# Atsuyo64/RayTracingC

Measured on AMD Instinct MI355X. Metric: Mrays/sec + frame time, 1920x1080x64spp ultracomplex.obj, 1/2/4/8 GPUs, higher is better.
Workload: dtype f32; 1 GPU; ultracomplex_1080p64; scene=ultracomplex.obj, width=1920, height=1080, spp=64, max_bounce=10, triangles=120, row_band=1, chain_wgs_per_cu=3, parallelism=rows mod 1; each rank SDMA-copies its rows into the shared host frame

## Files before the change

include/rtc.h:

```cpp
#ifndef RTC_H
#define RTC_H

#include <stddef.h>
#include <stdint.h>

#ifdef __cplusplus
extern "C" {
#endif

typedef unsigned char uint8;
typedef struct vec3 { float x, y, z; } vec3;
typedef struct Scene {
    vec3 normalizedSunDirection, skyColorHorizon, skyColorZenith, groundColor;
    float sunFocus, sunIntensity;
} Scene;
typedef struct Color { uint8 r, g, b; } Color;
typedef struct Material { vec3 color; float emissionStrength; float smoothness; } Material;
typedef struct Sphere { vec3 pos; float r; Material mat; } Sphere;
typedef struct Triangle { vec3 posA, posB, posC, normal; Material mat; } Triangle;
typedef struct Ray { vec3 pos; vec3 dir; } Ray;

typedef struct RtcCamera { vec3 origin, ex, ey, ez; float fov; } RtcCamera;

typedef struct RtcRenderDesc {
    int width, height;
    int spp;
    int maxBounce;
    int trianglesOnly;
    int rowStart, rowStride;
    int flags;
    int rowBand;
} RtcRenderDesc;

#define RTC_F_HOIST_PRIMARY 0x1
#define RTC_F_DEBUG_BOUNCES 0x2
#define RTC_F_NO_TILE_CULL  0x4
#define RTC_F_NO_REORDER    0x8
#define RTC_F_NO_COOP       0x10
#define RTC_F_NO_CLUSTER_CULL 0x20
#define RTC_F_COOP4         0x40
#define RTC_F_COOP8         0x80
#define RTC_F_PIPE          0x200
#define RTC_F_SPEC          0x100
#define RTC_F_CHAIN_INLINE  0x400
#define RTC_F_HOST_ROWS     0x1000
#define RTC_F_SPLIT_SPHERES 0x2000
#define RTC_F_NO_DRAW_CACHE 0x4000
#define RTC_F_WAVE_PER_RAY  0x20000
#define RTC_F_OVERLAP       0x800

typedef struct RtcStats {
    double renderMs;
    double totalMs;
    unsigned long long segments;
    unsigned long long samples;
    unsigned long long triTests;
    unsigned long long clusterTests;
    unsigned long long discardedTests;
    double frameMs;
} RtcStats;

#define RTC_OK 0
#define RTC_EINVAL (-10001)
#define RTC_ENODEV (-10002)
#define RTC_EIO (-10003)
#define RTC_ENOMEM (-10004)
#define RTC_EFORMAT (-10005)
#define RTC_ETIMEDOUT (-10006)
#define RTC_EBUSY (-10007)

const char *rtc_last_error(void);
const char *rtc_version(void);
int rtc_device_count(int *count);

int rtc_load_obj(const char *path, Triangle **outTris, int *outCount);
int rtc_parse_triangle_file(const char *path, Triangle **outTris, int *outCount);
void rtc_free(void *p);
int rtc_default_spheres(const Sphere **outSpheres, int *outCount);
int rtc_default_scene(Scene *outScene);
int rtc_scene_set_sun(Scene *scene, vec3 sunDirection);
int rtc_camera_basis(vec3 origin, vec3 lookingAt, float fov, RtcCamera *outCam);
int rtc_write_bmp(const char *path, int width, int height, const Color *image);
int rtc_quantize(const float *accum, size_t pixels, Color *out);

int rtc_render(const Triangle *tris, int triCount, const Sphere *spheres, int sphereCount,
               const Scene *scene, const RtcCamera *cam, const RtcRenderDesc *d, int device,
               Color *outImage, float *outAccum, RtcStats *stats);

int rtc_render_multi(const Triangle *tris, int triCount, const Sphere *spheres, int sphereCount,
                     const Scene *scene, const RtcCamera *cam, const RtcRenderDesc *d, int numDevices,
                     Color *outImage, float *outAccum, RtcStats *stats);
int rtc_last_multi_info(int *path, int *devices, int *commRanks, int maxComms);

typedef struct RtcDeviceScene RtcDeviceScene;
int rtc_scene_upload(const Triangle *tris, int triCount, const Sphere *spheres, int sphereCount,
                     int device, RtcDeviceScene **out);
int rtc_scene_release(RtcDeviceScene *s);
int rtc_scene_update_async(RtcDeviceScene *s, const Triangle *dTris, int triCount, const Sphere *dSpheres,
                           int sphereCount, void *stream);
int rtc_scene_update(RtcDeviceScene *s, const Triangle *tris, int triCount, const Sphere *spheres, int sphereCount);
size_t rtc_scene_regroup_scratch_bytes(const RtcDeviceScene *s);
int rtc_scene_regroup_max_tris(void);
int rtc_scene_regroup_async(RtcDeviceScene *s, const Triangle *dTris, int triCount, const Sphere *dSpheres,
                            int sphereCount, void *dScratch, size_t scratchBytes, void *stream);
int rtc_scene_regroup(RtcDeviceScene *s, const Triangle *tris, int triCount, const Sphere *spheres, int sphereCount);
int rtc_regroup_membership_host(const Triangle *tris, int triCount, int *idx);
int rtc_rows_selected(const RtcRenderDesc *d);
#define RTC_SEGMENT_COUNTERS 5
int rtc_scene_set_timing(RtcDeviceScene *s, int enable);
int rtc_scene_set_geometry_event(RtcDeviceScene *s, void *event);
int rtc_scene_set_frame_event(RtcDeviceScene *s, void *event);
int rtc_scene_kernel_times(const RtcDeviceScene *s, float out[2]);
int rtc_bounce_hit_share(const Triangle *tris, int triCount, float *share);
int rtc_scene_chain_wgs(const RtcDeviceScene *s);
typedef struct RtcChainReport {
    int multi, count, hits, general, spheres, resume;
    int chainPrimF, wgsPerCu, chainDyn, clusterCount, chunkCount, launches;
} RtcChainReport;
int rtc_scene_chain_report(const RtcDeviceScene *s, RtcChainReport *out);
int rtc_scene_set_draw_cache(RtcDeviceScene *s, long long blocks);
int rtc_scene_draw_cache_reset(RtcDeviceScene *s);
int rtc_scene_draw_cache_stats(const RtcDeviceScene *s, unsigned long long out[4]);
int rtc_probe_draw_cache(const RtcDeviceScene *s, unsigned int seed, float *out, int *block);
int rtc_bounce_hit_share_all(const Triangle *tris, int triCount, const Sphere *spheres, int sphereCount, float *share);
int rtc_scene_sphere_split(const RtcDeviceScene *s);
int rtc_render_rows_async(const RtcDeviceScene *s, const Scene *scene, const RtcCamera *cam,
                          const RtcRenderDesc *d, void *dColors, float *dAccum,
                          unsigned long long *dSegments, void *stream);
typedef struct RtcSampleRange { int first, count; } RtcSampleRange;
int rtc_render_samples_async(const RtcDeviceScene *s, const Scene *scene, const RtcCamera *cam,
                             const RtcRenderDesc *d, const RtcSampleRange *range,
                             void *dColors, float *dAccum, unsigned int *dRngState,
                             unsigned long long *dSegments, void *stream);
typedef struct RtcHitBuffers {
    int *prim;
    float *depth;
    float *normal;
    float *albedo;
} RtcHitBuffers;
int rtc_render_first_hit_async(const RtcDeviceScene *s, const RtcCamera *cam, const RtcRenderDesc *d,
                               const RtcHitBuffers *out, void *stream);
int rtc_trace_rays_async(const RtcDeviceScene *s, const Ray *dRays, size_t n, int trianglesOnly, int flags,
                         const RtcHitBuffers *out, void *stream);
int rtc_trace_rays(const RtcDeviceScene *s, const Ray *rays, size_t n, int trianglesOnly, int flags, int *prim,
                   float *depth, float *normal, float *albedo);
typedef struct RtcPathDesc {
    int spp;
    int maxBounce;
    int trianglesOnly;
    int flags;
    int sampleFirst, sampleCount;
} RtcPathDesc;
int rtc_trace_paths_async(const RtcDeviceScene *s, const Scene *scene, const Ray *dRays, const unsigned int *dSeeds,
                          size_t n, const RtcPathDesc *d, float *dRadiance, unsigned int *dSeedsOut,
                          unsigned long long *dSegments, void *stream);
int rtc_trace_paths(const RtcDeviceScene *s, const Scene *scene, const Ray *rays, const unsigned int *seeds, size_t n,
                    const RtcPathDesc *d, float *radiance, unsigned int *seedsOut, unsigned long long *segments);
int rtc_occluded_async(const RtcDeviceScene *s, const Ray *dRays, const float *dTMax , size_t n,
                       int trianglesOnly, int flags, unsigned char *dOccluded ,
                       unsigned long long *dCount , void *stream);
int rtc_occluded(const RtcDeviceScene *s, const Ray *rays, const float *tMax, size_t n, int trianglesOnly, int flags,
                 unsigned char *occluded, unsigned long long *count);
int rtc_render_pixels_async(const RtcDeviceScene *s, const Scene *scene, const RtcCamera *cam, const RtcRenderDesc *d,
                            const RtcSampleRange *range, const unsigned int *dPixels, size_t n, int flags,
                            void *dColors , float *dAccum, unsigned int *dRngState,
                            unsigned long long *dSegments , void *stream);
int rtc_render_pixels(const RtcDeviceScene *s, const Scene *scene, const RtcCamera *cam, const RtcRenderDesc *d,
                      const RtcSampleRange *range, const unsigned int *pixels, size_t n, int flags, void *colors,
                      float *accum, unsigned int *rngState, unsigned long long *segments);
int rtc_scene_bounds(const RtcDeviceScene *s, float lo[3], float hi[3]);
size_t rtc_ray_order_scratch_bytes(size_t n);
int rtc_ray_order_shape(int *keysPerGroup, int *scanGroups);
int rtc_ray_order_async(const RtcDeviceScene *s, const Ray *dRays, size_t n, const float *bounds,
                        unsigned *dOrder, unsigned *dKeys, void *dScratch, size_t scratchBytes, void *stream);
int rtc_ray_order(const RtcDeviceScene *s, const Ray *rays, size_t n, const float *bounds, unsigned *order,
                  unsigned *keys);
int rtc_ray_keys_host(const Ray *rays, size_t n, const float lo[3], const float hi[3], unsigned *keys);
int rtc_gather_async(void *dDst, const void *dSrc, const unsigned *dOrder, size_t n, size_t elemBytes, void *stream);
int rtc_scatter_async(void *dDst, const void *dSrc, const unsigned *dOrder, size_t n, size_t elemBytes, void *stream);
int rtc_copy_async(void *dst, const void *src, size_t bytes, int blocks, void *stream);
int rtc_copy_d2h_dma(void *hostDst, const void *devSrc, size_t bytes);
int rtc_dma_pending(const void *p, size_t bytes);
int rtc_dma_debug_inflight(void *p, size_t bytes, int pending);
int rtc_copy_rows_d2h_dma(void *hostDst, size_t hostPitch, const void *devSrc, size_t srcPitch, size_t rowBytes,
                          int rows);
int rtc_host_register(void *p, size_t bytes);
int rtc_host_unregister(void *p);

typedef struct RtcPlanSim RtcPlanSim;
int rtc_plan_sim_create(int triCount, int legacySlotLayout, RtcPlanSim **out);
int rtc_plan_sim_launch(RtcPlanSim *sim, const RtcRenderDesc *d, unsigned long long stream, unsigned long long colors,
                        unsigned long long accum, int segments, const float cam[13], const float env[14], int *ops,
                        int maxOps, unsigned long long *footprint, int maxFootprint);
int rtc_plan_sim_set_spheres(RtcPlanSim *sim, int sphereCount, int gateAllows);
int rtc_plan_sim_set_draw_cache(RtcPlanSim *sim, int on);
int rtc_plan_sim_set_sample_range(RtcPlanSim *sim, int first, int count, unsigned long long rngBuffer);
int rtc_plan_sim_set_first_hit(RtcPlanSim *sim, unsigned long long prim, unsigned long long depth,
                               unsigned long long normal, unsigned long long albedo);
int rtc_plan_sim_update(RtcPlanSim *sim, unsigned long long stream, int *ops, int maxOps, unsigned long long *footprint,
                        int maxFootprint);
int rtc_plan_sim_set_update_fault(RtcPlanSim *sim, int mode);
int rtc_plan_sim_regroup(RtcPlanSim *sim, unsigned long long stream, unsigned long long scratch, int *ops, int maxOps,
                         unsigned long long *footprint, int maxFootprint);
int rtc_plan_sim_trace_rays(RtcPlanSim *sim, unsigned long long stream, unsigned long long rays,
                            const unsigned long long hit[4], int flags, int *ops, int maxOps,
                            unsigned long long *footprint, int maxFootprint);
int rtc_plan_sim_trace_paths(RtcPlanSim *sim, unsigned long long stream, unsigned long long rays,
                             unsigned long long seeds, unsigned long long radiance, unsigned long long seedsOut,
                             unsigned long long segments, int sampleFirst, int flags, int *ops, int maxOps,
                             unsigned long long *footprint, int maxFootprint);
int rtc_plan_sim_occluded(RtcPlanSim *sim, unsigned long long stream, unsigned long long rays, unsigned long long tMax,
                          unsigned long long occluded, unsigned long long count, int flags, int *ops, int maxOps,
                          unsigned long long *footprint, int maxFootprint);
int rtc_plan_sim_render_pixels(RtcPlanSim *sim, unsigned long long stream, unsigned long long pixels,
                               unsigned long long colors, unsigned long long accum, unsigned long long rng,
                               unsigned long long segments, int first, int flags, int *ops, int maxOps,
                               unsigned long long *footprint, int maxFootprint);
int rtc_plan_sim_regions(const RtcPlanSim *sim, unsigned long long *rows, int maxRows);
int rtc_plan_sim_release(RtcPlanSim *sim);

typedef struct RtcLoopStats {
    double wallMs;
    int frames;
    double enqueueMs;
    double copyMsMedian;
    double copyMsMax;
} RtcLoopStats;
int rtc_frame_loop(RtcDeviceScene *s, const Scene *scene, const RtcCamera *cam, const RtcRenderDesc *d,
                   void *const *devRows, void *const *hostRows, size_t hostPitch, int nbuf, int frames, void *stream,
                   RtcLoopStats *stats);
int rtc_frame_loop_cameras(RtcDeviceScene *s, const Scene *scene, const RtcCamera *cams, int ncams,
                           const RtcRenderDesc *d, void *const *devRows, void *const *hostRows, size_t hostPitch,
                           int nbuf, int frames, void *stream, RtcLoopStats *stats);

int rtc_deinterleave_async(const void *dCompact, int parts, int rowsPerPart, int width, int height,
                           void *dOut, void *stream);
int rtc_deinterleave_bands_async(const void *dCompact, int parts, int rowsPerPart, int width, int height, int rowBand,
                                 void *dOut, void *stream);

int rtc_probe_ray_triangle(const Ray *rays, const Triangle *tris, size_t n, int *didHit, float *dst);
int rtc_probe_ray_sphere(const Ray *rays, const Sphere *spheres, size_t n, int *didHit, float *dst,
                         vec3 *normal);
int rtc_probe_environment(const Ray *rays, const Scene *scenes, size_t n, vec3 *out);
int rtc_probe_random(const unsigned int *seeds, size_t n, int draws, float *uniform, float *normal,
                     vec3 *direction);
int rtc_probe_sun_vanish(const Ray *rays, const Scene *scene, size_t n, int spp, int *vanish, vec3 *out, vec3 *sum);
int rtc_env_vanish_limit(const Scene *scene, double *limit);
int rtc_probe_cluster_bound(const Triangle *tris, int triCount, const Ray *rays, size_t n,
                            unsigned long long counts[7]);
int rtc_probe_item_records(const Triangle *tris, int triCount, const Sphere *spheres, int sphereCount, const Scene *scene,
                           const RtcCamera *cam, const RtcRenderDesc *d, int counts[16], int info[4],
                           unsigned int *records, size_t maxRecords, unsigned long long *pixMask, size_t maxTiles);
int rtc_probe_primary_cull(const Triangle *tris, int triCount, const Scene *scene, const RtcCamera *cam,
                           const RtcRenderDesc *d, unsigned char *kept, size_t maxKept, unsigned long long *tileBits,
                           size_t maxWords, unsigned long long *pixMask, size_t maxTiles, int info[4], float *primF,
                           double *cones, unsigned char *pruned);
int rtc_scene_records_host(const Triangle *tris, int triCount, const Triangle *newTris, const Sphere *spheres,
                           int sphereCount, void *outTris, void *outMats, void *outSpheres, void *outClTris,
                           void *outClusters, void *outChunks, size_t bytes[6]);
int rtc_probe_scene_records(const RtcDeviceScene *s, void *outTris, void *outMats, void *outSpheres, void *outClTris,
                            void *outClusters, void *outChunks, size_t bytes[6]);

#ifdef __cplusplus
}
#endif
#endif
```

raytracingc_amd/__init__.py:

```python
from __future__ import annotations

import contextlib
import ctypes as C
from dataclasses import dataclass

import numpy as np

from ._abi import (
    CLI_PATH,
    LIB_PATH,
    RAY_DT,
    RTC_F_DEBUG_BOUNCES,
    RTC_F_HOIST_PRIMARY,
    RTC_F_NO_CLUSTER_CULL,
    RTC_F_NO_COOP,
    RTC_F_CHAIN_INLINE,
    RTC_F_OVERLAP,
    RTC_F_HOST_ROWS,
    RTC_F_SPLIT_SPHERES,
    RTC_F_NO_DRAW_CACHE,
    RTC_F_NO_REORDER,
    RTC_F_NO_TILE_CULL,
    RTC_F_WAVE_PER_RAY,
    RTC_SEGMENT_COUNTERS,
    RTC_EBUSY,
    RTC_EINVAL,
    RTC_ETIMEDOUT,
    SCENE_DT,
    SPHERE_DT,
    TRIANGLE_DT,
    VEC3_DT,
    EXPORTS,
    Ray,
    RtcCamera,
    RtcChainReport,
    RtcError,
    RtcHitBuffers,
    RtcLoopStats,
    RtcPathDesc,
    RtcRenderDesc,
    RtcSampleRange,
    RtcStats,
    Scene,
    Vec3,
    check,
    lib,
)
from ._abi import _ptr

__all__ = [
    "loadOBJTriangles", "parseTriangleFile", "default_spheres", "default_scene", "camera_basis", "RenderConfig",
    "render", "render_multi", "DeviceScene", "vec3ToColor", "write_bmp", "rayTriangle", "raySphere",
    "getEnvironmentLight", "random_sequences", "device_count", "lib", "TRIANGLE_DT", "SPHERE_DT", "RAY_DT",
    "SCENE_DT", "RtcError", "ProgressState", "save_progress", "load_progress", "scene_records_host", "RECORD_ARRAYS",
    "ray_keys_host", "ray_order_scratch_bytes", "gather_async", "scatter_async",
    "regroup_membership_host", "regroup_max_tris", "adaptive_selection",
]

DEFAULT_ORIGIN = (-4.75, -1.5, -4.75)
DEFAULT_LOOKING_AT = (0.9, -1.2, 1.0)
DEFAULT_FOV = 1.0
DEFAULT_SUN = (-30.0, -85.0, 100.0)


def _take_tris(p: C.c_void_p, n: int) -> np.ndarray:
    out = np.empty(n, dtype=TRIANGLE_DT)
    if n:
        C.memmove(out.ctypes.data, p.value, n * TRIANGLE_DT.itemsize)
    lib().rtc_free(p)
    return out


def loadOBJTriangles(path: str) -> np.ndarray:
    p, n = C.c_void_p(), C.c_int()
    check(lib().rtc_load_obj(path.encode(), C.byref(p), C.byref(n)), "rtc_load_obj")
    return _take_tris(p, n.value)


def parseTriangleFile(path: str) -> np.ndarray:
    p, n = C.c_void_p(), C.c_int()
    check(lib().rtc_parse_triangle_file(path.encode(), C.byref(p), C.byref(n)), "rtc_parse_triangle_file")
    return _take_tris(p, n.value)


def default_spheres() -> np.ndarray:
    p, n = C.c_void_p(), C.c_int()
    check(lib().rtc_default_spheres(C.byref(p), C.byref(n)), "rtc_default_spheres")
    out = np.empty(n.value, dtype=SPHERE_DT)
    C.memmove(out.ctypes.data, p.value, n.value * SPHERE_DT.itemsize)
    return out


def default_scene(sun=DEFAULT_SUN, ground=None, horizon=None, zenith=None, focus=None, intensity=None) -> Scene:
    s = Scene()
    check(lib().rtc_default_scene(C.byref(s)), "rtc_default_scene")
    if ground is not None:
        s.groundColor = Vec3(*ground)
    if horizon is not None:
        s.skyColorHorizon = Vec3(*horizon)
    if zenith is not None:
        s.skyColorZenith = Vec3(*zenith)
    if focus is not None:
        s.sunFocus = focus
    if intensity is not None:
        s.sunIntensity = intensity
    check(lib().rtc_scene_set_sun(C.byref(s), Vec3(*sun)), "rtc_scene_set_sun")
    return s


def camera_basis(origin=DEFAULT_ORIGIN, looking_at=DEFAULT_LOOKING_AT, fov=DEFAULT_FOV) -> RtcCamera:
    cam = RtcCamera()
    check(lib().rtc_camera_basis(Vec3(*origin), Vec3(*looking_at), C.c_float(fov), C.byref(cam)), "rtc_camera_basis")
    return cam


@dataclass
class RenderConfig:
    width: int = 128
    height: int = 128
    spp: int = 4000
    max_bounce: int = 10
    triangles_only: bool = True
    hoist: bool = False
    row_start: int = 0
    row_stride: int = 1
    row_band: int = 0
    debug_bounces: bool = False
    tile_cull: bool = True
    reorder: bool = True
    coop: bool = True
    cluster_cull: bool = True
    chain_inline: bool = False
    host_rows: bool = False
    overlap: bool = False
    split_spheres: bool = False
    draw_cache: bool = True

    def flags(self) -> int:
        return ((RTC_F_HOIST_PRIMARY if self.hoist else 0) | (RTC_F_DEBUG_BOUNCES if self.debug_bounces else 0)
                | (0 if self.tile_cull else RTC_F_NO_TILE_CULL) | (0 if self.reorder else RTC_F_NO_REORDER)
                | (0 if self.coop else RTC_F_NO_COOP) | (0 if self.cluster_cull else RTC_F_NO_CLUSTER_CULL)
                | (RTC_F_CHAIN_INLINE if self.chain_inline else 0) | (RTC_F_OVERLAP if self.overlap else 0)
                | (RTC_F_HOST_ROWS if self.host_rows else 0) | (RTC_F_SPLIT_SPHERES if self.split_spheres else 0)
                | (0 if self.draw_cache else RTC_F_NO_DRAW_CACHE))

    def desc(self) -> RtcRenderDesc:
        return RtcRenderDesc(self.width, self.height, self.spp, self.max_bounce, int(self.triangles_only),
                             self.row_start, self.row_stride, self.flags(), self.row_band)

    def rows(self) -> int:
        d = self.desc()
        return lib().rtc_rows_selected(C.byref(d))


def _arr(a, dt):
    if a is None or len(a) == 0:
        return None, 0
    a = np.ascontiguousarray(a, dtype=dt)
    return a, len(a)


def _stats(st: RtcStats) -> dict:
    return {"render_ms": st.renderMs, "frame_ms": st.frameMs, "total_ms": st.totalMs, "segments": st.segments,
            "samples": st.samples, "tri_tests": st.triTests, "cluster_tests": st.clusterTests,
            "discarded_tests": st.discardedTests}


def _vp(p):
    return C.c_void_p(p) if p else None


def _query_rays(who: str, rays):
    if hasattr(rays, "data_ptr"):
        nbytes = rays.numel() * rays.element_size()
        if not rays.is_cuda or not rays.is_contiguous() or nbytes % RAY_DT.itemsize:
            raise ValueError(f"{who}: rays must be a contiguous device tensor of whole 24-byte Rays")
        return True, rays, nbytes // RAY_DT.itemsize
    a = np.asarray(rays)
    if a.dtype != RAY_DT:
        if a.ndim != 2 or a.shape[1] != 6:
            raise ValueError(f"{who}: rays must be RAY_DT [n] or float32 [n, 6]")
        a = np.ascontiguousarray(a, np.float32).view(RAY_DT).reshape(-1)
    a = np.ascontiguousarray(a.reshape(-1))
    return False, a, len(a)


@contextlib.contextmanager
def _current_stream_of(device):
    import torch

    with torch.cuda.device(device):
        st = torch.cuda.current_stream()
        yield st.cuda_stream
        st.synchronize()


def _host_order(who: str, order, n: int) -> np.ndarray:
    if hasattr(order, "data_ptr"):
        order = order.detach().cpu().numpy()
    idx = np.ascontiguousarray(np.asarray(order).reshape(-1)).astype(np.intp)
    if len(idx) != n or (n and (idx.min() < 0 or idx.max() >= n)):
        raise ValueError(f"{who}: order must hold {n} indices below {n}")
    return idx


def _device_order(who: str, order, n: int, device):
    import torch

    if not hasattr(order, "data_ptr"):
        order = torch.from_numpy(_host_order(who, order, n).astype(np.int32))
    order = order.reshape(-1).to(device=device, dtype=torch.int32).contiguous()
    if order.numel() != n or (n and (int(order.min()) < 0 or int(order.max()) >= n)):
        raise ValueError(f"{who}: order must hold {n} indices below {n}")
    return order


def _permuted(scatter: bool, src, order, n: int, elem_bytes: int, stream):
    import torch

    dst = torch.zeros_like(src) if scatter else torch.empty_like(src)
    if n:
        (scatter_async if scatter else gather_async)(dst.data_ptr(), src.data_ptr(), order.data_ptr(), n, elem_bytes,
                                                     stream)
    return dst


RECORD_ARRAYS = ("tris", "mats", "spheres", "clTris", "clusters", "chunks")
# ... 396 lines not shown
                    continue
                if not hasattr(t, "data_ptr") or not t.is_cuda or t.device != dev or not t.is_contiguous() or \
                        t.numel() * t.element_size() != nbytes:
                    raise ValueError(f"{who}: {name} must be a contiguous tensor of {nbytes} bytes on the list's device")
            if pixels.element_size() != 4 or rng.element_size() != 4 or accum.dtype != torch.float32:
                raise ValueError(f"{who}: pixels and rng are 4-byte integers, accum is float32")
            seg = torch.zeros(1, dtype=torch.int64, device=dev)
            if n and npix:
                with _current_stream_of(dev) as st:
                    self.render_pixels_async(scene, cam, cfg, first, count, pixels.data_ptr(), n, accum.data_ptr(),
                                             rng.data_ptr(), colors.data_ptr() if colors is not None else 0,
                                             seg.data_ptr() if segments else None, flags, st)
            res = {"accum": accum, "rng": rng}
            if colors is not None:
                res["colors"] = colors
            if segments:
                res["segments"] = int(seg.cpu().numpy()[0])
            return res
        px = np.asarray(pixels).reshape(-1)
        if px.size and (not np.issubdtype(px.dtype, np.integer) or px.min() < 0 or px.max() > 0xffffffff):
            raise ValueError(f"{who}: pixels must be integers in [0, 2^32)")
        px = np.ascontiguousarray(px, np.uint32)
        acc = np.array(accum, np.float32, order="C")
        state = np.array(rng, np.uint32, order="C")
        col = None if colors is None else np.array(colors, np.uint8, order="C")
        if acc.size != 3 * npix or state.size != npix or (col is not None and col.size != 3 * npix):
            raise ValueError(f"{who}: accum float32 [rows, W, 3], rng uint32 [rows, W] and colors uint8 [rows, W, 3] of "
                             f"the frame's {npix} pixels")
        seg = C.c_ulonglong(0)
        if len(px) and npix:
            d = cfg.desc()
            rg = RtcSampleRange(int(first), int(count))
            check(lib().rtc_render_pixels(self._h, C.byref(scene), C.byref(cam), C.byref(d), C.byref(rg), _ptr(px), len(px),
                                          int(flags), _ptr(col), _ptr(acc), _ptr(state),
                                          C.cast(C.pointer(seg), C.c_void_p) if segments else None), "rtc_render_pixels")
        res = {"accum": acc, "rng": state}
        if col is not None:
            res["colors"] = col
        if segments:
            res["segments"] = int(seg.value)
        return res

    def render_adaptive(self, scene: Scene, cam: RtcCamera, cfg: RenderConfig, passes, select, flags: int = 0):
        import torch

        passes = [int(c) for c in passes]
        if not passes or any(c <= 0 for c in passes) or sum(passes) > cfg.spp:
            raise ValueError(f"render_adaptive: passes {passes} are not positive counts summing to at most spp = {cfg.spp}")
        rows = cfg.rows()
        colors = torch.zeros((rows, cfg.width, 3), dtype=torch.uint8, device="cuda")
        accum = torch.zeros((rows, cfg.width, 3), dtype=torch.float32, device="cuda")
        rng = torch.zeros((rows, cfg.width), dtype=torch.int32, device="cuda")
        samples = np.zeros((rows, cfg.width), np.int32)
        st = torch.cuda.current_stream().cuda_stream
        done, host = 0, None
        for k, count in enumerate(passes):
            if k == 0:
                self.render_samples_async(scene, cam, cfg, 0, count, colors.data_ptr(), accum.data_ptr(), rng.data_ptr(),
                                          None, st)
                samples += count
            else:
                sel = adaptive_selection(select(done, host[0], host[1], samples.copy()), samples, done)
                if len(sel) == 0:
                    return
                pixels = torch.from_numpy(sel.view(np.int32)).cuda()
                self.render_pixels_async(scene, cam, cfg, done, count, pixels.data_ptr(), len(sel), accum.data_ptr(),
                                         rng.data_ptr(), colors.data_ptr(), None, flags, st)
                samples.reshape(-1)[sel] += count
            done += count
            torch.cuda.synchronize()
            host = (colors.cpu().numpy(), accum.cpu().numpy())
            yield done, host[0], host[1], samples.copy()

    @property
    def chain_wgs(self) -> int:
        return lib().rtc_scene_chain_wgs(self._h)

    def chain_report(self) -> dict:
        r = RtcChainReport()
        check(lib().rtc_scene_chain_report(self._h, C.byref(r)), "rtc_scene_chain_report")
        out = {k: bool(getattr(r, k)) for k in ("multi", "count", "hits", "general", "spheres", "resume")}
        out.update(chain_prim_f=bool(r.chainPrimF), wgs_per_cu=r.wgsPerCu, chain_dyn=r.chainDyn,
                   cluster_count=r.clusterCount, chunk_count=r.chunkCount, launches=r.launches)
        return out

    def set_draw_cache(self, blocks: int = -1):
        check(lib().rtc_scene_set_draw_cache(self._h, int(blocks)), "rtc_scene_set_draw_cache")

    def draw_cache_reset(self):
        check(lib().rtc_scene_draw_cache_reset(self._h), "rtc_scene_draw_cache_reset")

    def draw_cache_stats(self) -> dict:
        out = (C.c_ulonglong * 4)()
        check(lib().rtc_scene_draw_cache_stats(self._h, out), "rtc_scene_draw_cache_stats")
        return {"blocks": int(out[0]), "capacity": int(out[1]), "fresh": int(out[2]), "uncached": int(out[3])}

    def draw_cache_block(self, seed: int):
        out = np.zeros((64, 4), np.float32)
        blk = C.c_int(-1)
        check(lib().rtc_probe_draw_cache(self._h, int(seed), _ptr(out), C.byref(blk)), "rtc_probe_draw_cache")
        return out if blk.value >= 0 else None

    @property
    def sphere_split(self) -> bool:
        return bool(lib().rtc_scene_sphere_split(self._h))

    def set_timing(self, enable: bool):
        check(lib().rtc_scene_set_timing(self._h, int(enable)), "rtc_scene_set_timing")

    def set_geometry_event(self, event_handle: int | None):
        check(lib().rtc_scene_set_geometry_event(self._h, C.c_void_p(event_handle) if event_handle else None),
              "rtc_scene_set_geometry_event")

    def set_frame_event(self, event_handle: int | None):
        check(lib().rtc_scene_set_frame_event(self._h, C.c_void_p(event_handle) if event_handle else None),
              "rtc_scene_set_frame_event")

    def frame_loop(self, scene: Scene, cam, cfg: RenderConfig, dev_rows: list, host_rows: list,
                   host_pitch: int, frames: int, stream: int | None = None) -> dict:
        n = len(dev_rows)
        if len(host_rows) != n:
            raise ValueError("frame_loop: one host buffer per device buffer")
        d = cfg.desc()
        dv = (C.c_void_p * n)(*dev_rows)
        hv = (C.c_void_p * n)(*host_rows)
        st = RtcLoopStats()
        strm = C.c_void_p(stream) if stream else None
        if isinstance(cam, RtcCamera):
            check(lib().rtc_frame_loop(self._h, C.byref(scene), C.byref(cam), C.byref(d), dv, hv,
                                       C.c_size_t(host_pitch), n, int(frames), strm, C.byref(st)), "rtc_frame_loop")
        else:
            cams = (RtcCamera * len(cam))(*cam)
            check(lib().rtc_frame_loop_cameras(self._h, C.byref(scene), cams, len(cam), C.byref(d), dv, hv,
                                               C.c_size_t(host_pitch), n, int(frames), strm, C.byref(st)),
                  "rtc_frame_loop_cameras")
        return {"wall_ms": st.wallMs, "frames": st.frames, "enqueue_ms": st.enqueueMs,
                "copy_ms_median": st.copyMsMedian, "copy_ms_max": st.copyMsMax}

    def kernel_times(self):
        out = (C.c_float * 2)()
        check(lib().rtc_scene_kernel_times(self._h, out), "rtc_scene_kernel_times")
        return None if out[0] < 0 else (float(out[0]), float(out[1]))

    def regroup_scratch_bytes(self) -> int:
        return int(lib().rtc_scene_regroup_scratch_bytes(self._h))

    def regroup_async(self, tris_ptr: int, spheres_ptr: int | None, scratch_ptr: int, scratch_bytes: int,
                      stream: int | None = None):
        if not self._h:
            raise RuntimeError("DeviceScene.regroup_async: the scene has been released")
        check(lib().rtc_scene_regroup_async(self._h, _vp(tris_ptr), self.tri_count, _vp(spheres_ptr),
                                            self.sphere_count if spheres_ptr else 0, _vp(scratch_ptr), scratch_bytes,
                                            _vp(stream)), "rtc_scene_regroup_async")

    def update(self, tris=None, spheres=None, stream: int | None = None, regroup: bool = False):
        if not self._h:
            raise RuntimeError("DeviceScene.update: the scene has been released")
        if tris is None and spheres is None:
            raise ValueError("DeviceScene.update: neither triangles nor spheres")
        if regroup and tris is None:
            raise ValueError("DeviceScene.update: regroup=True needs the triangles (the clusters are decided from them)")
        on_device = [hasattr(a, "data_ptr") for a in (tris, spheres) if a is not None]
        if not any(on_device):
            t, nt = _arr(tris, TRIANGLE_DT)
            s, ns = _arr(spheres, SPHERE_DT)
            if regroup:
# ... 304 lines not shown
```

raytracingc_amd/_abi.py:

```python
from __future__ import annotations

import ctypes as C
import os

import numpy as np

HERE = os.path.dirname(os.path.abspath(__file__))
LIB_PATH = os.environ.get("RTC_LIB_PATH") or os.path.join(HERE, "_lib", "librtc.so")
CLI_PATH = os.path.join(HERE, "_lib", "rtc")


class Vec3(C.Structure):
    _fields_ = [("x", C.c_float), ("y", C.c_float), ("z", C.c_float)]


class Scene(C.Structure):
    _fields_ = [
        ("normalizedSunDirection", Vec3),
        ("skyColorHorizon", Vec3),
        ("skyColorZenith", Vec3),
        ("groundColor", Vec3),
        ("sunFocus", C.c_float),
        ("sunIntensity", C.c_float),
    ]
# ... 8 lines not shown


class Triangle(C.Structure):
    _fields_ = [("posA", Vec3), ("posB", Vec3), ("posC", Vec3), ("normal", Vec3), ("mat", Material)]


class Ray(C.Structure):
    _fields_ = [("pos", Vec3), ("dir", Vec3)]


class RtcCamera(C.Structure):
    _fields_ = [("origin", Vec3), ("ex", Vec3), ("ey", Vec3), ("ez", Vec3), ("fov", C.c_float)]


class RtcRenderDesc(C.Structure):
    _fields_ = [
        ("width", C.c_int),
        ("height", C.c_int),
        ("spp", C.c_int),
        ("maxBounce", C.c_int),
        ("trianglesOnly", C.c_int),
        ("rowStart", C.c_int),
        ("rowStride", C.c_int),
        ("flags", C.c_int),
        ("rowBand", C.c_int),
    ]


class RtcSampleRange(C.Structure):
    _fields_ = [("first", C.c_int), ("count", C.c_int)]


class RtcHitBuffers(C.Structure):
    _fields_ = [("prim", C.c_void_p), ("depth", C.c_void_p), ("normal", C.c_void_p), ("albedo", C.c_void_p)]


class RtcPathDesc(C.Structure):
    _fields_ = [(k, C.c_int) for k in ("spp", "maxBounce", "trianglesOnly", "flags", "sampleFirst", "sampleCount")]


class RtcChainReport(C.Structure):
    _fields_ = [(k, C.c_int) for k in ("multi", "count", "hits", "general", "spheres", "resume", "chainPrimF", "wgsPerCu",
                                       "chainDyn", "clusterCount", "chunkCount", "launches")]


class RtcStats(C.Structure):
    _fields_ = [
        ("renderMs", C.c_double),
        ("totalMs", C.c_double),
        ("segments", C.c_ulonglong),
        ("samples", C.c_ulonglong),
        ("triTests", C.c_ulonglong),
        ("clusterTests", C.c_ulonglong),
        ("discardedTests", C.c_ulonglong),
        ("frameMs", C.c_double),
    ]


class RtcLoopStats(C.Structure):
    _fields_ = [
        ("wallMs", C.c_double),
        ("frames", C.c_int),
        ("enqueueMs", C.c_double),
        ("copyMsMedian", C.c_double),
        ("copyMsMax", C.c_double),
    ]


RTC_F_HOIST_PRIMARY = 0x1
RTC_F_DEBUG_BOUNCES = 0x2
RTC_F_NO_TILE_CULL = 0x4
RTC_F_NO_REORDER = 0x8
RTC_F_NO_COOP = 0x10
RTC_F_NO_CLUSTER_CULL = 0x20
RTC_F_COOP4 = 0x40
RTC_F_COOP8 = 0x80
RTC_F_SPEC = 0x100
RTC_F_PIPE = 0x200
RTC_F_CHAIN_INLINE = 0x400
RTC_F_OVERLAP = 0x800
RTC_F_HOST_ROWS = 0x1000
RTC_F_SPLIT_SPHERES = 0x2000
RTC_F_NO_DRAW_CACHE = 0x4000
RTC_F_WAVE_PER_RAY = 0x20000
RAY_ORDER_KEYS_PER_GROUP = 4096
RAY_ORDER_SCAN_GROUPS = 256
RTC_SEGMENT_COUNTERS = 5
RTC_EINVAL, RTC_ENODEV, RTC_EIO, RTC_ENOMEM, RTC_EFORMAT = -10001, -10002, -10003, -10004, -10005
RTC_ETIMEDOUT, RTC_EBUSY = -10006, -10007

assert C.sizeof(Vec3) == 12 and C.sizeof(Scene) == 56 and C.sizeof(Material) == 20
assert C.sizeof(Sphere) == 36 and C.sizeof(Triangle) == 68 and C.sizeof(Ray) == 24

VEC3_DT = np.dtype([("x", "<f4"), ("y", "<f4"), ("z", "<f4")])
MATERIAL_DT = np.dtype([("color", VEC3_DT), ("emissionStrength", "<f4"), ("smoothness", "<f4")])
TRIANGLE_DT = np.dtype(
    [("posA", VEC3_DT), ("posB", VEC3_DT), ("posC", VEC3_DT), ("normal", VEC3_DT), ("mat", MATERIAL_DT)]
)
SPHERE_DT = np.dtype([("pos", VEC3_DT), ("r", "<f4"), ("mat", MATERIAL_DT)])
RAY_DT = np.dtype([("pos", VEC3_DT), ("dir", VEC3_DT)])
SCENE_DT = np.dtype(
    [
        ("normalizedSunDirection", VEC3_DT),
        ("skyColorHorizon", VEC3_DT),
        ("skyColorZenith", VEC3_DT),
        ("groundColor", VEC3_DT),
        ("sunFocus", "<f4"),
        ("sunIntensity", "<f4"),
    ]
)
assert TRIANGLE_DT.itemsize == 68 and SPHERE_DT.itemsize == 36 and RAY_DT.itemsize == 24
assert SCENE_DT.itemsize == 56

EXPORTS = [
    "rtc_last_error", "rtc_version", "rtc_device_count",
    "rtc_load_obj", "rtc_parse_triangle_file", "rtc_free", "rtc_default_spheres", "rtc_default_scene",
    "rtc_scene_set_sun", "rtc_camera_basis", "rtc_write_bmp", "rtc_quantize",
    "rtc_render", "rtc_render_multi", "rtc_last_multi_info",
    "rtc_scene_upload", "rtc_scene_release", "rtc_rows_selected", "rtc_render_rows_async", "rtc_scene_set_timing", "rtc_scene_kernel_times",
    "rtc_bounce_hit_share", "rtc_scene_chain_wgs", "rtc_bounce_hit_share_all", "rtc_scene_sphere_split",
    "rtc_plan_sim_set_spheres", "rtc_plan_sim_regions", "rtc_render_samples_async", "rtc_plan_sim_set_sample_range",
    "rtc_scene_set_geometry_event", "rtc_scene_set_frame_event",
    "rtc_deinterleave_async", "rtc_deinterleave_bands_async", "rtc_copy_async", "rtc_copy_d2h_dma", "rtc_copy_rows_d2h_dma", "rtc_host_register",
    "rtc_host_unregister", "rtc_plan_sim_create", "rtc_plan_sim_launch", "rtc_plan_sim_release", "rtc_frame_loop", "rtc_frame_loop_cameras", "rtc_dma_pending", "rtc_dma_debug_inflight",
    "rtc_probe_ray_triangle", "rtc_probe_ray_sphere", "rtc_probe_environment", "rtc_probe_random",
    "rtc_probe_cluster_bound", "rtc_probe_sun_vanish", "rtc_env_vanish_limit", "rtc_probe_item_records",
    "rtc_probe_primary_cull",
    "rtc_scene_update_async", "rtc_scene_update", "rtc_plan_sim_update", "rtc_plan_sim_set_update_fault",
    "rtc_scene_records_host", "rtc_probe_scene_records",
    "rtc_scene_chain_report",
    "rtc_render_first_hit_async", "rtc_plan_sim_set_first_hit",
    "rtc_trace_rays_async", "rtc_trace_rays", "rtc_plan_sim_trace_rays",
    "rtc_scene_set_draw_cache", "rtc_scene_draw_cache_reset", "rtc_scene_draw_cache_stats", "rtc_probe_draw_cache",
    "rtc_plan_sim_set_draw_cache",
    "rtc_trace_paths_async", "rtc_trace_paths", "rtc_plan_sim_trace_paths",
    "rtc_occluded_async", "rtc_occluded", "rtc_plan_sim_occluded",
    "rtc_scene_bounds", "rtc_ray_order_shape", "rtc_ray_order_scratch_bytes", "rtc_ray_order_async", "rtc_ray_order", "rtc_ray_keys_host",
    "rtc_gather_async", "rtc_scatter_async",
    "rtc_scene_regroup_scratch_bytes", "rtc_scene_regroup_max_tris", "rtc_scene_regroup_async", "rtc_scene_regroup",
    "rtc_regroup_membership_host", "rtc_plan_sim_regroup",
    "rtc_render_pixels_async", "rtc_render_pixels", "rtc_plan_sim_render_pixels",
]

_lib = None


def _ptr(a: np.ndarray | None):
    return None if a is None else a.ctypes.data_as(C.c_void_p)


def lib() -> C.CDLL:
    global _lib
    if _lib is not None:
        return _lib
    if not os.path.exists(LIB_PATH):
        raise RuntimeError(f"librtc.so not built ({LIB_PATH}); run `make` or __graft_entry__.build()")
    try:
        import torch
    except Exception:
        pass
    L = C.CDLL(LIB_PATH)
    vp, ip, sz = C.c_void_p, C.c_int, C.c_size_t
    L.rtc_last_error.restype = C.c_char_p
    L.rtc_version.restype = C.c_char_p
    L.rtc_device_count.argtypes = [C.POINTER(C.c_int)]
    L.rtc_load_obj.argtypes = [C.c_char_p, C.POINTER(vp), C.POINTER(C.c_int)]
    L.rtc_parse_triangle_file.argtypes = [C.c_char_p, C.POINTER(vp), C.POINTER(C.c_int)]
    L.rtc_free.argtypes = [vp]
    L.rtc_free.restype = None
    L.rtc_default_spheres.argtypes = [C.POINTER(vp), C.POINTER(C.c_int)]
    L.rtc_default_scene.argtypes = [C.POINTER(Scene)]
    L.rtc_scene_set_sun.argtypes = [C.POINTER(Scene), Vec3]
    L.rtc_camera_basis.argtypes = [Vec3, Vec3, C.c_float, C.POINTER(RtcCamera)]
    L.rtc_write_bmp.argtypes = [C.c_char_p, ip, ip, vp]
    L.rtc_quantize.argtypes = [vp, sz, vp]
    L.rtc_render.argtypes = [vp, ip, vp, ip, C.POINTER(Scene), C.POINTER(RtcCamera), C.POINTER(RtcRenderDesc), ip,
                             vp, vp, C.POINTER(RtcStats)]
    L.rtc_render_multi.argtypes = [vp, ip, vp, ip, C.POINTER(Scene), C.POINTER(RtcCamera),
                                   C.POINTER(RtcRenderDesc), ip, vp, vp, C.POINTER(RtcStats)]
    L.rtc_last_multi_info.argtypes = [C.POINTER(C.c_int), C.POINTER(C.c_int), C.POINTER(C.c_int), ip]
    L.rtc_scene_upload.argtypes = [vp, ip, vp, ip, ip, C.POINTER(vp)]
    L.rtc_scene_release.argtypes = [vp]
    L.rtc_scene_kernel_times.argtypes = [vp, vp]
    L.rtc_bounce_hit_share.argtypes = [vp, C.c_int, C.POINTER(C.c_float)]
    L.rtc_scene_chain_wgs.argtypes = [vp]
    if hasattr(L, "rtc_scene_sphere_split"):
        L.rtc_bounce_hit_share_all.argtypes = [vp, C.c_int, vp, C.c_int, C.POINTER(C.c_float)]
        L.rtc_scene_sphere_split.argtypes = [vp]
        L.rtc_plan_sim_set_spheres.argtypes = [vp, ip, ip]
    L.rtc_scene_set_timing.argtypes = [vp, C.c_int]
    L.rtc_scene_set_geometry_event.argtypes = [vp, vp]
    L.rtc_scene_set_frame_event.argtypes = [vp, vp]
    L.rtc_copy_async.argtypes = [vp, vp, sz, C.c_int, vp]
    L.rtc_copy_d2h_dma.argtypes = [vp, vp, sz]
    L.rtc_copy_rows_d2h_dma.argtypes = [vp, sz, vp, sz, sz, ip]
    L.rtc_host_register.argtypes = [vp, sz]
    L.rtc_host_unregister.argtypes = [vp]
    L.rtc_frame_loop.argtypes = [vp, C.POINTER(Scene), C.POINTER(RtcCamera), C.POINTER(RtcRenderDesc), vp, vp, sz, ip,
                                 ip, vp, C.POINTER(RtcLoopStats)]
    L.rtc_frame_loop_cameras.argtypes = [vp, C.POINTER(Scene), vp, ip, C.POINTER(RtcRenderDesc), vp, vp, sz, ip, ip,
                                         vp, C.POINTER(RtcLoopStats)]
    L.rtc_plan_sim_create.argtypes = [ip, ip, C.POINTER(vp)]
    L.rtc_plan_sim_launch.argtypes = [vp, C.POINTER(RtcRenderDesc), C.c_ulonglong, C.c_ulonglong, C.c_ulonglong, ip, vp,
                                      vp, vp, ip, vp, ip]
    L.rtc_plan_sim_release.argtypes = [vp]
    if hasattr(L, "rtc_plan_sim_regions"):
        L.rtc_plan_sim_regions.argtypes = [vp, vp, ip]
    L.rtc_dma_pending.argtypes = [vp, sz]
    L.rtc_dma_debug_inflight.argtypes = [vp, sz, ip]
    L.rtc_rows_selected.argtypes = [C.POINTER(RtcRenderDesc)]
    L.rtc_render_rows_async.argtypes = [vp, C.POINTER(Scene), C.POINTER(RtcCamera), C.POINTER(RtcRenderDesc), vp, vp,
                                        vp, vp]
    if hasattr(L, "rtc_render_samples_async"):
        L.rtc_render_samples_async.argtypes = [vp, C.POINTER(Scene), C.POINTER(RtcCamera), C.POINTER(RtcRenderDesc),
                                               C.POINTER(RtcSampleRange), vp, vp, vp, vp, vp]
        L.rtc_plan_sim_set_sample_range.argtypes = [vp, ip, ip, C.c_ulonglong]
    L.rtc_deinterleave_async.argtypes = [vp, ip, ip, ip, ip, vp, vp]
    if hasattr(L, "rtc_deinterleave_bands_async"):
        L.rtc_deinterleave_bands_async.argtypes = [vp, ip, ip, ip, ip, ip, vp, vp]
    L.rtc_probe_ray_triangle.argtypes = [vp, vp, sz, vp, vp]
    L.rtc_probe_ray_sphere.argtypes = [vp, vp, sz, vp, vp, vp]
    L.rtc_probe_environment.argtypes = [vp, vp, sz, vp]
    L.rtc_probe_random.argtypes = [vp, sz, ip, vp, vp, vp]
    L.rtc_probe_cluster_bound.argtypes = [vp, ip, vp, sz, vp]
    if hasattr(L, "rtc_probe_sun_vanish"):
        L.rtc_probe_sun_vanish.argtypes = [vp, vp, sz, ip, vp, vp, vp]
        L.rtc_env_vanish_limit.argtypes = [vp, vp]
    if hasattr(L, "rtc_probe_item_records"):
        L.rtc_probe_item_records.argtypes = [vp, ip, vp, ip, C.POINTER(Scene), C.POINTER(RtcCamera),
                                             C.POINTER(RtcRenderDesc), vp, vp, vp, sz, vp, sz]
    if hasattr(L, "rtc_probe_primary_cull"):
        L.rtc_probe_primary_cull.argtypes = [vp, ip, C.POINTER(Scene), C.POINTER(RtcCamera), C.POINTER(RtcRenderDesc),
                                             vp, sz, vp, sz, vp, sz, vp, vp, vp, vp]
    if hasattr(L, "rtc_scene_update_async"):
        L.rtc_scene_update_async.argtypes = [vp, vp, ip, vp, ip, vp]
        L.rtc_scene_update.argtypes = [vp, vp, ip, vp, ip]
        L.rtc_plan_sim_update.argtypes = [vp, C.c_ulonglong, vp, ip, vp, ip]
        L.rtc_plan_sim_set_update_fault.argtypes = [vp, ip]
        L.rtc_scene_records_host.argtypes = [vp, ip, vp, vp, ip, vp, vp, vp, vp, vp, vp, vp]
        L.rtc_probe_scene_records.argtypes = [vp, vp, vp, vp, vp, vp, vp, vp]
    if hasattr(L, "rtc_scene_chain_report"):
        L.rtc_scene_chain_report.argtypes = [vp, C.POINTER(RtcChainReport)]
    if hasattr(L, "rtc_render_first_hit_async"):
        L.rtc_render_first_hit_async.argtypes = [vp, C.POINTER(RtcCamera), C.POINTER(RtcRenderDesc),
                                                 C.POINTER(RtcHitBuffers), vp]
        L.rtc_plan_sim_set_first_hit.argtypes = [vp, C.c_ulonglong, C.c_ulonglong, C.c_ulonglong, C.c_ulonglong]
    if hasattr(L, "rtc_trace_rays_async"):
        L.rtc_trace_rays_async.argtypes = [vp, vp, sz, ip, ip, C.POINTER(RtcHitBuffers), vp]
        L.rtc_trace_rays.argtypes = [vp, vp, sz, ip, ip, vp, vp, vp, vp]
        L.rtc_plan_sim_trace_rays.argtypes = [vp, C.c_ulonglong, C.c_ulonglong, vp, ip, vp, ip, vp, ip]
    if hasattr(L, "rtc_scene_set_draw_cache"):
        L.rtc_scene_set_draw_cache.argtypes = [vp, C.c_longlong]
        L.rtc_scene_draw_cache_reset.argtypes = [vp]
        L.rtc_scene_draw_cache_stats.argtypes = [vp, vp]
        L.rtc_probe_draw_cache.argtypes = [vp, C.c_uint, vp, C.POINTER(C.c_int)]
        L.rtc_plan_sim_set_draw_cache.argtypes = [vp, ip]
    if hasattr(L, "rtc_trace_paths_async"):
        L.rtc_trace_paths_async.argtypes = [vp, C.POINTER(Scene), vp, vp, sz, C.POINTER(RtcPathDesc), vp, vp, vp, vp]
        L.rtc_trace_paths.argtypes = [vp, C.POINTER(Scene), vp, vp, sz, C.POINTER(RtcPathDesc), vp, vp, vp]
        L.rtc_plan_sim_trace_paths.argtypes = [vp, C.c_ulonglong, C.c_ulonglong, C.c_ulonglong, C.c_ulonglong,
                                               C.c_ulonglong, C.c_ulonglong, ip, ip, vp, ip, vp, ip]
    if hasattr(L, "rtc_occluded_async"):
        L.rtc_occluded_async.argtypes = [vp, vp, vp, sz, ip, ip, vp, vp, vp]
        L.rtc_occluded.argtypes = [vp, vp, vp, sz, ip, ip, vp, vp]
        L.rtc_plan_sim_occluded.argtypes = [vp, C.c_ulonglong, C.c_ulonglong, C.c_ulonglong, C.c_ulonglong,
                                            C.c_ulonglong, ip, vp, ip, vp, ip]
    if hasattr(L, "rtc_ray_order_async"):
        L.rtc_scene_bounds.argtypes = [vp, vp, vp]
        L.rtc_ray_order_shape.argtypes = [C.POINTER(C.c_int), C.POINTER(C.c_int)]
        L.rtc_ray_order_scratch_bytes.argtypes = [sz]
        L.rtc_ray_order_scratch_bytes.restype = sz
        L.rtc_ray_order_async.argtypes = [vp, vp, sz, vp, vp, vp, vp, sz, vp]
        L.rtc_ray_order.argtypes = [vp, vp, sz, vp, vp, vp]
        L.rtc_ray_keys_host.argtypes = [vp, sz, vp, vp, vp]
        L.rtc_gather_async.argtypes = [vp, vp, vp, sz, sz, vp]
        L.rtc_scatter_async.argtypes = [vp, vp, vp, sz, sz, vp]
    if hasattr(L, "rtc_scene_regroup_async"):
        L.rtc_scene_regroup_scratch_bytes.argtypes = [vp]
        L.rtc_scene_regroup_scratch_bytes.restype = sz
        L.rtc_scene_regroup_max_tris.argtypes = []
        L.rtc_scene_regroup_async.argtypes = [vp, vp, ip, vp, ip, vp, sz, vp]
        L.rtc_scene_regroup.argtypes = [vp, vp, ip, vp, ip]
        L.rtc_regroup_membership_host.argtypes = [vp, ip, vp]
        L.rtc_plan_sim_regroup.argtypes = [vp, C.c_ulonglong, C.c_ulonglong, vp, ip, vp, ip]
    if hasattr(L, "rtc_render_pixels_async"):
        L.rtc_render_pixels_async.argtypes = [vp, C.POINTER(Scene), C.POINTER(RtcCamera), C.POINTER(RtcRenderDesc),
                                              C.POINTER(RtcSampleRange), vp, sz, ip, vp, vp, vp, vp, vp]
        L.rtc_render_pixels.argtypes = [vp, C.POINTER(Scene), C.POINTER(RtcCamera), C.POINTER(RtcRenderDesc),
                                        C.POINTER(RtcSampleRange), vp, sz, ip, vp, vp, vp, vp]
        L.rtc_plan_sim_render_pixels.argtypes = [vp, C.c_ulonglong, C.c_ulonglong, C.c_ulonglong, C.c_ulonglong,
                                                 C.c_ulonglong, C.c_ulonglong, ip, ip, vp, ip, vp, ip]
    _lib = L
    return L


class RtcError(RuntimeError):
    def __init__(self, code: int, where: str):
        msg = lib().rtc_last_error().decode(errors="replace")
        super().__init__(f"{where} failed ({code}): {msg}")
        self.code = code


def check(rc: int, where: str) -> None:
    if rc != 0:
        raise RtcError(rc, where)
```

raytracingc_amd/csrc/rtc_chain.h:

```cpp
#pragma once

static_assert(sizeof(SampleSlot) == rtcplan::kSampleSlotBytes, "the planner sizes the deferred sample slots");
#ifndef RTC_SKY_MERGE
#define RTC_SKY_MERGE 1
#endif
constexpr int kChainBlock = 256;
#ifndef RTC_CHAIN_WGS_SHARE
#define RTC_CHAIN_WGS_SHARE 3
#endif
#ifndef RTC_CHAIN_WAVES
#define RTC_CHAIN_WAVES 4
#endif

typedef float f2 __attribute__((ext_vector_type(2)));
constexpr int kChainPairs = 1024;
struct ChainWaveLds {
    float4 cl[kChunkClusters][2];
    unsigned long long key[64];
    unsigned short pair[kChainPairs];
    float4 draw[64];
};
constexpr unsigned long long kNoHitKey = ((unsigned long long)0x497423F0u << 32) | 0xFFFFFFFFull;
static_assert(kChunkClusters <= 32, "cluster masks are 32-bit");
static_assert(kChainPairs >= 64 * kClusterSize, "one cluster's pairs of a full wave fit the list");
// ... 322 lines not shown
        }
        const size_t o = (size_t)P.itemPix[it];
        P.colors[3 * o] = float_to_u8(accxy.x);
        P.colors[3 * o + 1] = float_to_u8(accxy.y);
        P.colors[3 * o + 2] = float_to_u8(accz);
        if (P.accum) {
            P.accum[3 * o] = accxy.x;
            P.accum[3 * o + 1] = accxy.y;
            P.accum[3 * o + 2] = accz;
        }
    }
}

__device__ __forceinline__ void closest_primary_listed_lds(const RenderParams &P, V3 dir, Closest &c, const unsigned long long *__restrict__ mask,
                                                           unsigned long long m0, unsigned long long m1,
                                                           const DevPrimF *__restrict__ sF, bool staged)
{
    const int maskWords = KARG(maskWords);
    const DevPrimF *const primF = KARG(primF);
    const DevPrimX *const primX = KARG(primX);
    for (int w = 0; w < maskWords; ++w) {
        unsigned long long m = w == 0 ? m0 : w == 1 ? m1 : KCONST(mask)[w];
        while (m) {
            const int t = w * 64 + __builtin_ctzll(m);
            m &= m - 1;
            const DevPrimF F = staged ? sF[t] : KLOAD(primF, t);
            if (!prim_backfacing(dir, F) && prim_pass(dir, F) && !(dot(dir, V3{F.nx, F.ny, F.nz}) >= 0.f)) {
                const DevPrimX X = KLOAD(primX, t);
                const V3 h = cross(dir, V3{X.acx, X.acy, X.acz});
                const float det = dot(V3{X.abx, X.aby, X.abz}, h);
                if (!(-kEps < det && det < kEps)) {
                    const float invDet = rcp_cr(det);
                    const float u = dot(V3{X.s0x, X.s0y, X.s0z}, h) * invDet;
                    const float v = dot(dir, V3{X.q0x, X.q0y, X.q0z}) * invDet;
                    const float dst = X.dac0 * invDet;
                    if (!(u < 0.f || u > 1.f) && !(v < 0.f || u + v > 1.f) && !(dst < kEps) && dst < c.dst) {
                        c.dst = dst;
                        c.idx = t;
                    }
                }
            }
        }
    }
}

constexpr int kChainSphereBase = 1 << 30;
__device__ __forceinline__ void closest_spheres(const RenderParams &P, V3 pos, V3 dir, Closest &c)
{
    const DevSphere *const spheres = KARG(spheres);
    const int n = KARG(sphereCount);
    for (int i = 0; i < n; ++i) {
        const DevSphere sp = KLOAD(spheres, i);
        float d;
        if (ray_sphere(pos, dir, V3{sp.cx, sp.cy, sp.cz}, sp.radius, d) && d < c.dst) {
            c.dst = d;
            c.idx = kChainSphereBase + i;
        }
    }
}

struct ChainStage {
    float4 *rec;
    DevPrimF *primF;
};
template <bool MULTI>
__device__ __forceinline__ ChainStage chain_stage(const RenderParams &P, unsigned char *sDyn)
{
    ChainStage S{nullptr, nullptr};
    if (!MULTI)
        S.rec = (float4 *)sDyn;
    if (P.chainPrimF)
        S.primF = (DevPrimF *)(sDyn + (MULTI ? 0 : (size_t)soa_slots(P.clusterCount * kClusterSize) * sizeof(DevTri)));
    const int nRec = P.clusterCount * kClusterSize, slots = soa_slots(nRec);
    for (int i = threadIdx.x; S.rec && i < nRec; i += kChainBlock) {
        const float4 *g = (const float4 *)(P.clTris + i);
        for (int k = 0; k < 4; ++k)
            S.rec[k * slots + i] = g[k];
    }
    for (int i = threadIdx.x; S.primF && i < P.triPadded; i += kChainBlock)
        S.primF[i] = P.primF[i];
    return S;
}

template <bool MULTI, bool COUNT, bool HITS, bool GENERAL, bool SPHERES = false, bool RESUME = false, bool DRAWS = false>
__global__ __launch_bounds__(kChainBlock) __attribute__((amdgpu_waves_per_eu(RTC_CHAIN_WAVES))) void rtc_render_chain(
    RenderParams P)
{
    if (RTC_CHAIN_PRIO > 0)
        __builtin_amdgcn_s_setprio(RTC_CHAIN_PRIO);
    DSECT_BEGIN(dtot);
    DMARK_INIT(dcur);
#ifdef RTC_DIAG
    const unsigned long long dWaveT0 = __builtin_amdgcn_s_memrealtime();
    unsigned dWaveItems = 0;
    unsigned long long dItemEnd[5] = {0, 0, 0, 0, 0};
#endif
    extern __shared__ __attribute__((aligned(64))) unsigned char sDyn[];
    __shared__ PowTablesLds sPow;
    __shared__ ChainWaveLds sWave[kChainBlock / 64];
    __shared__ int sWork;
    __shared__ DevCluster sCl[kChunkClusters];
    if (!MULTI && threadIdx.x < P.clusterCount && threadIdx.x < kChunkClusters)
        sCl[threadIdx.x] = P.clusters[threadIdx.x];
    if (threadIdx.x == 0)
        sWork = 0;
    sPow.fill(threadIdx.x);
    const ChainStage S = chain_stage<MULTI>(P, sDyn);
    const float4 *sRec = S.rec;
    const DevPrimF *sPF = (const DevPrimF *)(sDyn + (MULTI ? 0 : (size_t)soa_slots(P.clusterCount * kClusterSize) * sizeof(DevTri)));
    const bool pfStaged = !GENERAL || P.chainPrimF != 0;
#ifdef RTC_DIAG
    if ((threadIdx.x & 63) < kDiagSects)
        s_rtc_sect[threadIdx.x >> 6][threadIdx.x & 63] = 0;
    static_assert(kChainBlock / 64 <= 4, "s_rtc_sect holds four waves");
#endif
    __syncthreads();
    sPow.attach(P.env);
    const int lane = threadIdx.x & 63;
    ChainWaveLds &W = sWave[threadIdx.x >> 6];
    const RngJump laneJump = rng_jump_by(7u * (unsigned)lane);
    int nextIt = 0;
    const auto next_item = [&]() { return (int)blockIdx.x + atomicAdd(&sWork, 1) * (int)gridDim.x; };
    if (lane == 0)
        nextIt = next_item();
#ifdef RTC_DIAG_COUNT
    constexpr bool counting = true;
#else
    constexpr bool counting = COUNT;
#endif
    unsigned segCalls = 0, segTraced = 0, segClusters = 0;
    unsigned long long segTests = 0, segSpec = 0;
#ifdef RTC_DIAG
    unsigned long long dIters = 0, dAlive = 0, dAct = 0, dWindows = 0, dUsed = 0, dIters2 = 0, dAlive2 = 0;
#endif
    int incl = lane < kGeoLists ? min(P.geoCount[lane * kGeoCountStride], P.geoCap) : 0;
#pragma unroll
    for (int d = 1; d < kGeoLists; d <<= 1) {
        const int v = __shfl_up(incl, d);
        if (lane >= d)
            incl += v;
    }
    const int nItems = __builtin_amdgcn_readlane(incl, kGeoLists - 1);
    const auto entry_of = [&](int it2) -> size_t {
        const int l = (int)__popcll(__ballot(lane < kGeoLists && incl <= it2));
        const int base = l ? __builtin_amdgcn_readlane(incl, l - 1) : 0;
        return (size_t)l * KARG(geoCap) + (size_t)(it2 - base);
    };
    static_assert(!DRAWS || (!GENERAL && !RESUME && !SPHERES && !MULTI && !COUNT), "the draw cache: the kernels without GENERAL");
    const auto record_dwords = [&](int it2) -> unsigned {
        if constexpr (DRAWS) {
            const size_t e = entry_of(it2);
            const unsigned *const rec = KARG(geoList) + e * (size_t)kItemRecDwords + (size_t)(lane & (kItemRecDwords - 1));
            const unsigned *const blk = KARG(itemDraw) + e;
            return gload((lane & kItemRecDwords) ? blk : rec, 0);
        }
        return gload(KARG(geoList), entry_of(it2) * (size_t)kItemRecDwords + (size_t)(lane & (kItemRecDwords - 1)));
    };
    const auto record_tile = [&](unsigned d0) -> int {
        return KARG(wideItems) ? (int)(d0 >> 6) : (int)(d0 >> 19) * (KARG(blocksX) * 2) + (int)((d0 & 0xffffu) >> 3);
    };
    const auto mask_dwords = [&](unsigned d0) -> unsigned {
        const unsigned *mw = (const unsigned *)(KARG(tileMask) + (size_t)record_tile(d0) * P.maskWords);
        return lane < 2 * P.maskWords && lane < 4 ? gload(mw, (size_t)lane) : 0u;
    };
    int it = __builtin_amdgcn_readfirstlane(nextIt);
    unsigned vc = 0, vm = 0;
    if (it < nItems) {
        vc = record_dwords(it);
        vm = mask_dwords((unsigned)__builtin_amdgcn_readfirstlane((int)vc));
    }
    if (lane == 0)
        nextIt = next_item();
    DMARK(dcur, 19);
    for (;;) {
        if (it >= nItems)
            break;
#ifdef RTC_DIAG
        const unsigned long long dItemT0 = __builtin_amdgcn_s_memrealtime();
        unsigned dItemWindows = 0;
        const unsigned long long dItemIters0 = dIters;
        const unsigned dBm0 = __atomic_load_n(&g_rtc_bmfall[(blockIdx.x * (kChainBlock / 64) + (threadIdx.x >> 6)) & 65535u],
                                              __ATOMIC_RELAXED);
        const unsigned long long dSect = lane < kItemSects ? s_rtc_sect[threadIdx.x >> 6][item_sect_id(lane)] : 0ull;
        unsigned long long dItemTests = 0;
#endif
        const unsigned d0 = (unsigned)__builtin_amdgcn_readfirstlane((int)vc);
        const V3 pdir{__uint_as_float((unsigned)__builtin_amdgcn_readlane((int)vc, 1)),
                      __uint_as_float((unsigned)__builtin_amdgcn_readlane((int)vc, 2)),
                      __uint_as_float((unsigned)__builtin_amdgcn_readlane((int)vc, 3))};
        const unsigned long long m0 = (unsigned long long)(unsigned)__builtin_amdgcn_readlane((int)vm, 0) |
                                      (unsigned long long)(unsigned)__builtin_amdgcn_readlane((int)vm, 1) << 32;
        const unsigned long long m1 = (unsigned long long)(unsigned)__builtin_amdgcn_readlane((int)vm, 2) |
                                      (unsigned long long)(unsigned)__builtin_amdgcn_readlane((int)vm, 3) << 32;
        float4 cachedDraw = make_float4(0.f, 0.f, 0.f, 0.f);
        unsigned drawBlock = 0;
        if constexpr (DRAWS) {
            drawBlock = (unsigned)__builtin_amdgcn_readlane((int)vc, kItemRecDwords);
            if (drawBlock)
                cachedDraw = gload4(KARG(drawPool), (size_t)(drawBlock - 1u) * kDrawEntries + (size_t)lane);
        }
        const int itNext = __builtin_amdgcn_readfirstlane(nextIt);
        if (itNext < nItems)
            vc = record_dwords(itNext);
        bool maskNext = itNext >= nItems;
        if (lane == 0)
            nextIt = next_item();
        const int tile = record_tile(d0);
        int x = (int)(d0 & 0xffffu), r = (int)(d0 >> 16);
        if (KARG(wideItems)) {
            const int tilesX = KARG(blocksX) * 2, bit = (int)(d0 & 63u);
            x = (tile % tilesX) * 8 + (bit & 7), r = (tile / tilesX) * 8 + (bit >> 3);
        }
        const int sh = KARG(rowBandShift);
        const int y = KARG(rowStart) + ((r >> sh) * KARG(rowStride) << sh) + (r & ((1 << sh) - 1));
        const unsigned long long *mask = KARG(tileMask) + (size_t)tile * P.maskWords;
        unsigned L = 0;
        if (counting)
            for (int w = 0; w < P.maskWords; ++w)
                L += (unsigned)__popcll(mask[w]);
        unsigned seedOf = (unsigned)(x + y * KARG(width));
        if constexpr (RESUME) {
            if (KARG(sampleFirst) > 0)
                seedOf = (unsigned)__builtin_amdgcn_readfirstlane(
                    (int)gload(KARG(rngState), (size_t)r * (size_t)KARG(width) + (size_t)x));
        }
        const unsigned seed = seedOf;
        const bool deferred = GENERAL && it < P.sampleCap;
        Closest prim{999999.f, -1};
        if (GENERAL && P.hoist && P.spp > 0 && P.maxBounce > 0) {
            if constexpr (SPHERES)
                closest_spheres(P, KARG(origin), pdir, prim);
            closest_primary_listed_lds(P, pdir, prim, mask, m0, m1, sPF, pfStaged);
            if (counting && lane == 0) {
                segTraced++;
                segTests += L;
            }
        }
        DMARK(dcur, 15);
        float acc = 0.f;
        if constexpr (RESUME) {
            if (KARG(sampleFirst) > 0 && !deferred && lane < 3)
                acc = __uint_as_float(gload(KARG(accum), 3 * ((size_t)r * (size_t)KARG(width) + (size_t)x) + (size_t)lane));
        }
        int k = 0;
        unsigned jn = 0;
        while (k < P.spp && P.maxBounce > 0) {
            const int need = P.spp - k;
            const int est = k > 0 ? (int)(((unsigned long long)need * jn + (unsigned)k - 1u) / (unsigned)k) : need;
            const int nAct = min(64, est + (est >> 3) + 1);
            const bool act = lane < nAct;
            const unsigned s0 = (unsigned)__builtin_amdgcn_readfirstlane((int)rng_advance(seed, 7u * jn));
            unsigned rng = s0 * laneJump.a + laneJump.c;
            DMARK(dcur, 0);
            V3 pos = KARG(origin), dir = pdir, rayColor{1.f, 1.f, 1.f}, light{0.f, 0.f, 0.f};
            int bounce = 0;
            unsigned hits = 0, calls = 0, tests = 0, clTests = 0;
            bool alive = act;
            for (int iter = 0; __any(alive); ++iter) {
                const bool first = iter == 0, bounce1 = iter == 1;
#ifdef RTC_DIAG
                dIters++;
                dAlive += (unsigned long long)__popcll(__ballot(alive));
                if (iter >= 2) {
                    dIters2++;
                    dAlive2 += (unsigned long long)__popcll(__ballot(alive));
                }
#endif
                Closest c{999999.f, -1};
                if (first) {
                    if (alive) {
                        if (GENERAL && P.hoist) {
                            c = prim;
                        } else {
                            if constexpr (SPHERES)
                                closest_spheres(P, pos, dir, c);
                            closest_primary_listed_lds(P, dir, c, mask, m0, m1, sPF, pfStaged);
                            if (counting)
                                tests += L;
                        }
                    }
                    DMARK(dcur, 1);
                } else {
                    if (!maskNext) {
                        vm = mask_dwords((unsigned)__builtin_amdgcn_readfirstlane((int)vc));
                        maskNext = true;
                    }
                    unsigned t = 0;
                    if constexpr (SPHERES) {
// ... 351 lines not shown
```

raytracingc_amd/csrc/rtc_closest.h:

```cpp
#pragma once

__global__ __launch_bounds__(64) void rtc_prep_primary(const DevTri *__restrict__ tris, DevPrimF *__restrict__ pf,
                                                        DevPrimX *__restrict__ px, int triCount, V3 origin,
                                                        int *__restrict__ geoCount)
{
    const int t = blockIdx.x * 64 + threadIdx.x;
    if (geoCount && blockIdx.x == 0 && threadIdx.x < kGeoLists)
        geoCount[threadIdx.x * kGeoCountStride] = 0;
    if (t >= triCount)
        return;
    const DevTri T = tris[t];
    const V3 AB{T.abx, T.aby, T.abz}, AC{T.acx, T.acy, T.acz}, N{T.nx, T.ny, T.nz};
    const V3 s0 = sub(origin, V3{T.ax, T.ay, T.az});
    const V3 q0 = cross(s0, AB);
    const float dac0 = dot(AC, q0);
    DevPrimX x;
    x.abx = AB.x, x.aby = AB.y, x.abz = AB.z;
    x.acx = AC.x, x.acy = AC.y, x.acz = AC.z;
    x.s0x = s0.x, x.s0y = s0.y, x.s0z = s0.z;
    x.q0x = q0.x, x.q0y = q0.y, x.q0z = q0.z;
    x.dac0 = dac0;
    x.pad[0] = x.pad[1] = x.pad[2] = 0.f;
    px[t] = x;

    const double abx = AB.x, aby = AB.y, abz = AB.z, acx = AC.x, acy = AC.y, acz = AC.z;
    const double sx = s0.x, sy = s0.y, sz = s0.z;
    const double gdx = acy * abz - acz * aby, gdy = acz * abx - acx * abz, gdz = acx * aby - acy * abx;
    const double gux = acy * sz - acz * sy, guy = acz * sx - acx * sz, guz = acx * sy - acy * sx;
    auto n1 = [](double a, double b, double c) { return fabs(a) + fabs(b) + fabs(c); };
    const double u = 5.9604644775390625e-08;
    const double nAB = n1(abx, aby, abz), nAC = n1(acx, acy, acz), nS = n1(sx, sy, sz);
    const double nQ = n1(q0.x, q0.y, q0.z), nN = n1(N.x, N.y, N.z);
    const double eD = 9.006 * u * nAB * nAC;
    const double eU = 9.006 * u * nS * nAC;
    const double eV = 6.002 * u * nQ;
    const double eW = eD + eU + eV + 2.0002 * u * (nAB * nAC + nS * nAC + nQ) + 4.8e-7 * nAB * nAC;
    const double tiny = 8.673617379884035e-19;
    const double m = fmax(fmax(eU, eV), eW) * 4.0 + tiny;
    const double ed = eD * 4.0;
    const double mnd = 6.002 * u * nN * 4.0;
    const bool sane = ed < 2.5e-4 && nAB * nAC < 1e30 && nS * nAC < 1e30 && nQ < 1e30 && m < 1e30 && mnd < 1e30;
    const bool never = !(dac0 < 0.f || dac0 > 0.f);
    const float sg = dac0 < 0.f ? -1.f : 1.f;
    DevPrimF f;
    f.nx = N.x, f.ny = N.y, f.nz = N.z;
    f.gdx = sane ? sg * (float)gdx : 0.f, f.gdy = sane ? sg * (float)gdy : 0.f, f.gdz = sane ? sg * (float)gdz : 0.f;
    f.gux = sane ? sg * (float)gux : 0.f, f.guy = sane ? sg * (float)guy : 0.f, f.guz = sane ? sg * (float)guz : 0.f;
    f.q0x = sane ? sg * q0.x : 0.f, f.q0y = sane ? sg * q0.y : 0.f, f.q0z = sane ? sg * q0.z : 0.f;
    f.pad0 = 0.f;
    f.mnd = never ? -__builtin_inff() : (sane ? __double2float_ru(mnd) : __builtin_inff());
    f.c = sane ? __double2float_rd((double)0.001f - ed) : -__builtin_inff();
    f.negm = sane ? -__double2float_ru(m) : -__builtin_inff();
    pf[t] = f;
}

struct Closest {
    float dst;
    int idx;
};

constexpr float kTiny = 8.67361738e-19f;





__device__ __forceinline__ void primary_test(const RenderParams &P, V3 dir, const DevPrimF &F, int t, int base,
                                             Closest &c)
{
    if (!prim_backfacing(dir, F)) {
        if (prim_pass(dir, F)) {
            const DevPrimX X = P.primX[t];
            if (!(dot(dir, V3{F.nx, F.ny, F.nz}) >= 0.f)) {
                const V3 h = cross(dir, V3{X.acx, X.acy, X.acz});
                const float det = dot(V3{X.abx, X.aby, X.abz}, h);
                if (!(-kEps < det && det < kEps)) {
                    const float invDet = rcp_cr(det);
                    const float u = dot(V3{X.s0x, X.s0y, X.s0z}, h) * invDet;
                    const float v = dot(dir, V3{X.q0x, X.q0y, X.q0z}) * invDet;
                    const float dst = X.dac0 * invDet;
                    if (!(u < 0.f || u > 1.f) && !(v < 0.f || u + v > 1.f) && !(dst < kEps) && dst < c.dst) {
                        c.dst = dst;
                        c.idx = base + t;
                    }
                }
            }
        }
    }
}

__device__ __forceinline__ void closest_primary(const RenderParams &P, V3 dir, Closest &c, int base)
// ... 157 lines not shown
```

raytracingc_amd/csrc/rtc_cull.h:

```cpp
#pragma once


constexpr int kSuperBlocks = 4;
__global__ __launch_bounds__(64) void rtc_super_cull(RenderParams P, unsigned long long *__restrict__ superMask)
{
    const int sx = blockIdx.x, sy = blockIdx.y, lane = threadIdx.x;
    const int x0 = sx * kSuperBlocks * kTileW, r0 = sy * kSuperBlocks * kTileH;
    const TileCone K = rect_cone(P, x0, x0 + kSuperBlocks * kTileW - 1, r0, r0 + kSuperBlocks * kTileH - 1);
    unsigned long long *out = superMask + (size_t)(sy * P.superX + sx) * P.maskWords;
    for (int w = 0; w < P.maskWords; ++w) {
        const int ti = w * 64 + lane;
        const bool maybe = ti < P.triPadded && (!K.ok || !tile_prunes(K, P.primF[ti]));
        const unsigned long long m = __ballot(maybe);
        if (lane == 0)
            out[w] = m;
    }
}

template <bool SPH, bool DRAWS = false>
__device__ __forceinline__ void tile_cull_body(const RenderParams &P, unsigned long long *__restrict__ mask,
                                               unsigned *__restrict__ weight, unsigned long long *__restrict__ pixMask,
                                               const DrawCache &C = DrawCache{})
{
    const bool split = P.geoList != nullptr;
    if (KARG(cullPrio))
        __builtin_amdgcn_s_setprio(3);
    __shared__ unsigned wgWeight, wgAny;
    extern __shared__ unsigned long long sBlockCand[];
    CSTAMP(c0);
    if (threadIdx.x == 0) {
        wgWeight = 0;
        wgAny = 0;
    }
    const int bx = blockIdx.x, by = blockIdx.y;
    const int lane = threadIdx.x & 63, wave = threadIdx.x >> 6;
    if (P.geoCountNext && bx == 0 && by == 0 && threadIdx.x < kGeoLists)
        P.geoCountNext[threadIdx.x * kGeoCountStride] = 0;
    __syncthreads();
    const unsigned long long *sup =
        P.superMask ? P.superMask + (size_t)((by / kSuperBlocks) * P.superX + bx / kSuperBlocks) * P.maskWords : nullptr;
    bool supAny = !sup;
    for (int w = 0; sup && w < P.maskWords && !supAny; ++w)
        supAny = KCONST(sup)[w] != 0ull;
    if (wave < P.maskWords && supAny) {
        const TileCone KB = rect_cone(P, bx * kTileW, bx * kTileW + kTileW - 1, by * kTileH, by * kTileH + kTileH - 1);
        for (int w = wave; w < P.maskWords; w += kBlock / 64) {
            const int ti = w * 64 + lane;
            const unsigned long long sw = sup ? KCONST(sup)[w] : ~0ull;
            const bool maybe = ((sw >> lane) & 1ull) && ti < P.triPadded &&
                               (!KB.ok || !tile_prunes(KB, P.primF[ti]));
            const unsigned long long m = __ballot(maybe);
            if (lane == 0) {
                sBlockCand[w] = m;
                if (m)
                    wgAny = 1;
            }
        }
    }
    bool sphHit = false;
    if (SPH) {
        const PixelRay ps = pixel_ray(P, bx, by);
        if (ps.valid) {
            for (int i = 0; i < P.sphereCount; ++i) {
                const DevSphere sp = KLOAD(P.spheres, i);
                float d;
                if (ray_sphere(P.origin, ps.dir, V3{sp.cx, sp.cy, sp.cz}, sp.radius, d) && d < 999999.f)
                    sphHit = true;
            }
        }
        if (!supAny)
            for (int w = threadIdx.x; w < P.maskWords; w += kBlock)
                sBlockCand[w] = 0ull;
        if (__ballot(sphHit) != 0ull && lane == 0)
            wgAny = 1;
    }
    __syncthreads();
    CSTAMP(c1);
    const int tile = wave_tile(bx, by);
    unsigned long long *out = mask + (size_t)tile * P.maskWords;
    if (!wgAny) {
        for (int w = lane; !split && w < P.maskWords; w += 64)
            out[w] = 0ull;
        if (lane == 0)
            pixMask[tile] = 0ull;
        if (threadIdx.x == 0 && !split)
            weight[blockIdx.y * gridDim.x + blockIdx.x] = 0u;
        CSTAMP(c9);
        CREC(blockIdx.y * gridDim.x + blockIdx.x, c0, c1, c9, 0, 0, 0, 0);
        return;
    }
#ifdef RTC_DIAG
    unsigned long long dPre = 0, dLoop = 0, dCand = 0;
#endif
    const PixelRay px = pixel_ray(P, bx, by);
    bool anyCand = SPH && sphHit;
    const TileCone K = tile_cone(P, tile % (int)(gridDim.x * 2), tile / (int)(gridDim.x * 2));
    for (int w = 0; w < P.maskWords; ++w) {
        const int ti = w * 64 + lane;
        const unsigned long long bc = sBlockCand[w];
        CSTAMP(c2);
        const bool maybe = ((bc >> lane) & 1ull) && (!K.ok || !tile_prunes(K, P.primF[ti]));
        unsigned long long todo = bc ? __ballot(maybe) : 0ull;
        unsigned long long bits = 0;
        CSTAMP(c3);
#ifdef RTC_DIAG
        dPre += c3 - c2;
        dCand += (unsigned long long)__popcll(todo);
#endif
        while (todo) {
            const int j = __builtin_ctzll(todo);
            todo &= todo - 1;
            const DevPrimF F = KLOAD(P.primF, w * 64 + j);
            const bool keep = (int)px.valid & (int)!prim_backfacing(px.dir, F) & (int)prim_pass(px.dir, F);
            anyCand |= keep;
            if (__ballot(keep))
                bits |= 1ull << j;
        }
        CSTAMP(c4);
#ifdef RTC_DIAG
        dLoop += c4 - c3;
// ... 181 lines not shown
```

raytracingc_amd/csrc/rtc_layout.h:

```cpp
#pragma once
#include <hip/hip_runtime.h>

#include <cstddef>

#include "../../include/rtc.h"
#include "rtc_device.h"
#include "rtc_plan.h"

using namespace rtcdev;

struct __attribute__((aligned(64))) DevTri {
    float ax, ay, az, abx, aby, abz, acx, acy, acz, nx, ny, nz, pad0, pad1, pad2, pad3;
};
struct __attribute__((aligned(32))) DevMat {
    float r, g, b, emission, smoothness, pad0, pad1, pad2;
};
struct __attribute__((aligned(16))) DevSphere {
    float cx, cy, cz, radius, r, g, b, emission, smoothness, pad0, pad1, pad2;
};
struct __attribute__((aligned(64))) DevPrimF {
    float nx, ny, nz, mnd;
    float gdx, gdy, gdz, c;
    float gux, guy, guz, negm;
    float q0x, q0y, q0z, pad0;
// ... 75 lines not shown
    K.vmin = vmin * (1.0 - 1e-12);
    K.vmax = vmax * (1.0 + 1e-12);
    K.eDir = 16.0 * u * S / K.vmin + 4.0 * u;
    K.ivmin = 1.0 / K.vmin;
    K.ivmax = 1.0 / K.vmax;
    const bool unitBasis = fabs(P.ex.x) <= 1.0001f && fabs(P.ex.y) <= 1.0001f && fabs(P.ex.z) <= 1.0001f &&
                           fabs(P.ey.x) <= 1.0001f && fabs(P.ey.y) <= 1.0001f && fabs(P.ey.z) <= 1.0001f &&
                           fabs(P.ez.x) <= 1.0001f && fabs(P.ez.y) <= 1.0001f && fabs(P.ez.z) <= 1.0001f;
    K.ok = finite && unitBasis && K.vmin > 1e-6 && K.eDir < 1e-3 && S - S == 0.0;
    return K;
}

template <typename PT> __device__ TileCone tile_cone(const PT &P, int tx, int ty)
{
    return rect_cone(P, tx * 8, tx * 8 + 7, ty * 8, ty * 8 + 7);
}

__device__ __forceinline__ void cone_range(const TileCone &K, double gx, double gy, double gz, double &lb, double &ub)
{
    double mx = -1e300, mn = 1e300;
#pragma unroll
    for (int k = 0; k < 4; ++k) {
        const double a = gx * K.c[k][0] + gy * K.c[k][1] + gz * K.c[k][2];
        mx = fmax(mx, a);
        mn = fmin(mn, a);
    }
    ub = mx * (mx >= 0.0 ? K.ivmin : K.ivmax);
    lb = mn * (mn >= 0.0 ? K.ivmax : K.ivmin);
    ub += fabs(ub) * 0x1p-50;
    lb -= fabs(lb) * 0x1p-50;
}

__device__ bool tile_prunes(const TileCone &K, const DevPrimF &F)
{
    const double u = 5.9604644775390625e-08;
    const double e = K.eDir + 3.01 * u;
    auto n1 = [](double a, double b, double c) { return fabs(a) + fabs(b) + fabs(c); };
    double lb, ub;
    cone_range(K, F.nx, F.ny, F.nz, lb, ub);
    if (lb - n1(F.nx, F.ny, F.nz) * e > (double)F.mnd)
        return true;
    const double nd = n1(F.gdx, F.gdy, F.gdz), nu = n1(F.gux, F.guy, F.guz), nv = n1(F.q0x, F.q0y, F.q0z);
    cone_range(K, F.gdx, F.gdy, F.gdz, lb, ub);
    if (ub + nd * e < (double)F.c)
        return true;
    cone_range(K, F.gux, F.guy, F.guz, lb, ub);
    if (ub + nu * e < (double)F.negm)
        return true;
    cone_range(K, F.q0x, F.q0y, F.q0z, lb, ub);
    if (ub + nv * e < (double)F.negm)
        return true;
    cone_range(K, (double)F.gdx - F.gux - F.q0x, (double)F.gdy - F.guy - F.q0y, (double)F.gdz - F.guz - F.q0z, lb,
               ub);
    if (ub + (nd + nu + nv) * (e + 2.01 * u * 1.0001) < (double)F.negm)
        return true;
    return false;
}

constexpr int kClusterSize = 8;
constexpr int kChunkClusters = 32;
constexpr float kClusterRhoMax = 4.f;
constexpr float kClusterGamma = 2e-5f;
struct __attribute__((aligned(32))) DevCluster {
    float cx, cy, cz, r;
    float alpha, beta, gammaE, e;
};

constexpr unsigned kOrderEventFlags = hipEventDisableTiming | hipEventDisableSystemFence;
constexpr int kSkySlots = 8;
#ifndef RTC_CHAIN_WGS_FULL
#define RTC_CHAIN_WGS_FULL 3
#endif
constexpr size_t kCullPrioMinPixels = 400000;
#ifndef RTC_CHAIN_PRIO
#define RTC_CHAIN_PRIO 3
#endif
#ifndef RTC_CHAIN_WGS_HIT
#define RTC_CHAIN_WGS_HIT 4
#endif
constexpr double kWgsHitShare = 0.15;

constexpr int kGeoLists = 16, kGeoCountStride = 32;
constexpr int kItemRecDwords = 4;
constexpr int kGeoRing = 16, kGeoSetInts = kGeoLists * kGeoCountStride;
static_assert(kGeoSetInts >= kGeoLists * kGeoCountStride, "a counter set holds every sub-list counter");
static_assert(kSkySlots == rtcplan::kSlots && kGeoRing == rtcplan::kGeoRing && kGeoLists == rtcplan::kGeoLists &&
                  kGeoCountStride == rtcplan::kGeoCountStride && kItemRecDwords * 4 == rtcplan::kItemRecordBytes,
              "the planner's slot and counter-set layout is the device's");
constexpr int kDrawEntries = 64;
constexpr size_t kDrawBlockBytes = kDrawEntries * 16;
enum DrawCtr : int {
    kDcTaken = 0,
    kDcFilled0 = 1,
    kDcFilled1 = 2,
    kDcUncachedAcc = 3,
    kDcFresh = 4, kDcUncached = 5,
    kDcWords = 8
};
struct SceneRecords {
    DevTri *tris;
    DevMat *mats;
    DevSphere *spheres;
    DevTri *clTris;
    DevCluster *clusters;
    DevCluster *chunks;
};
enum SceneArrayId : int { kArrTris, kArrMats, kArrSpheres, kArrClTris, kArrClusters, kArrChunks, kSceneArrayCount };
struct SceneArray {
    const char *name;
    size_t elem;
    size_t at;
};
constexpr SceneArray kSceneArrays[kSceneArrayCount] = {
    {"tris", sizeof(DevTri), offsetof(SceneRecords, tris)},
    {"mats", sizeof(DevMat), offsetof(SceneRecords, mats)},
    {"spheres", sizeof(DevSphere), offsetof(SceneRecords, spheres)},
    {"clTris", sizeof(DevTri), offsetof(SceneRecords, clTris)},
    {"clusters", sizeof(DevCluster), offsetof(SceneRecords, clusters)},
    {"chunks", sizeof(DevCluster), offsetof(SceneRecords, chunks)},
};
static_assert(sizeof(SceneRecords) == kSceneArrayCount * sizeof(void *), "every pointer of a SceneRecords is in the table");
inline void *&scene_array(SceneRecords &g, int k)
{
    return *reinterpret_cast<void **>(reinterpret_cast<unsigned char *>(&g) + kSceneArrays[k].at);
}
inline void *scene_array(const SceneRecords &g, int k) { return scene_array(const_cast<SceneRecords &>(g), k); }
struct RtcDeviceScene {
    int device;
    int cuCount;
    int triCount, triPadded, sphereCount;
    int clusterCount;
    int chunkCount;
    float boundsLo[3], boundsHi[3];
    SceneRecords gen[2];
    const SceneRecords &current() const { return gen[plan.gen]; }
    int *clIndex;
    size_t recBytes[kSceneArrayCount];
    DevPrimF *primF;
    DevPrimX *primX;
    size_t primStride;
    unsigned char *scratch;
    int *geoCounts;
    double hitShare;
    int chainWgsFull;
    double hitShareAll;
    bool sphereSplitGate;
    rtcplan::State plan;
    hipStream_t cst;
    hipStream_t cst2;
    hipStream_t side;
    hipEvent_t evCullSync, evFork, evJoin;
    hipEvent_t evSkyDone[kSkySlots], evGeoDone[kSkySlots];
    hipEvent_t frameEvent;
    hipEvent_t geoEvent;
    unsigned char *samples;
    int maskWords;
    unsigned long long *segSlots;
    hipEvent_t evHeavy0, evHeavy1, evSky0, evSky1;
    bool timing;
    bool timed;
    RtcChainReport chainReport;
    struct Draws {
        long long blocks;
        unsigned *table;
        size_t tablePixels;
        unsigned *ctr;
        unsigned *blockSeed;
        void *pool;
        size_t capacity;
        unsigned char *itemDraw;
        int parity;
    } draws;
};
constexpr long long kDrawCacheDefaultBytes = 1ll << 30;

struct RtcCullItems {
    const int *geoCount;
    const unsigned *geoList;
    const unsigned long long *pixMask;
    int geoCap, tilesX;
    size_t tiles;
    int wide;
    const unsigned long long *tileMask;
    int maskWords;
    const DevPrimF *primF;
    int triPadded;
    int level0;
};
int rtc_cull_items(const RtcDeviceScene *s, const Scene *scene, const RtcCamera *cam, const RtcRenderDesc *d,
                   void *dColors, RtcCullItems *items);
int rtc_draws_prepare(RtcDeviceScene *s, int width, int height, bool reset, size_t growBytes);
void rtc_draws_free(RtcDeviceScene *s);

struct ClusterTerms {
    V3 w;
    float w2, A, B;
};
__device__ __forceinline__ ClusterTerms cluster_terms(V3 pos, const DevCluster &K)
{
    ClusterTerms t;
    t.w = sub(V3{K.cx, K.cy, K.cz}, pos);
    const float S = fabsf(t.w.x) + fabsf(t.w.y) + fabsf(t.w.z) + K.r;
    t.w2 = fmaf(t.w.z, t.w.z, fmaf(t.w.y, t.w.y, t.w.x * t.w.x));
    t.A = (K.r + kClusterGamma * S) + K.gammaE;
    t.B = fmaf(K.beta, S, K.alpha);
    return t;
}
__device__ __forceinline__ bool culled_by(const ClusterTerms &t, V3 dir, float rho, float dd)
{
    const float T = fmaf(rho, t.B, t.A) * 1.00001f;
    const float T2 = T * T;
    const float b = fmaf(t.w.z, dir.z, fmaf(t.w.y, dir.y, t.w.x * dir.x));
    const float wd = t.w2 * dd;
    const float x2 = fmaf(-b, b, wd);
    return b > 0.f ? (x2 - 1.5e-6f * wd > T2 * dd) : (t.w2 > T2);
}
__device__ __forceinline__ float dir_dd(V3 dir) { return fmaf(dir.z, dir.z, fmaf(dir.y, dir.y, dir.x * dir.x)); }
__device__ __forceinline__ bool cluster_culled(V3 pos, V3 dir, float rho, float dd, const DevCluster &K)
{
    return culled_by(cluster_terms(pos, K), dir, rho, dd);
}

__host__ __device__ static inline V3 v3(vec3 v) { return V3{v.x, v.y, v.z}; }

#ifndef RTC_SUN_VANISH
#define RTC_SUN_VANISH 1
#endif
static inline EnvParams env_of(const Scene &s)
{
    EnvParams e{};
    e.sun = v3(s.normalizedSunDirection);
    e.horizon = v3(s.skyColorHorizon);
    e.zenith = v3(s.skyColorZenith);
    e.ground = v3(s.groundColor);
    e.focus = s.sunFocus;
    e.intensity = s.sunIntensity;
    e.sunSkip = env_sun_skippable(e.focus, e.intensity);
    const float col[9] = {e.ground.x, e.ground.y, e.ground.z, e.horizon.x, e.horizon.y, e.horizon.z,
                          e.zenith.x, e.zenith.y, e.zenith.z};
    e.vanishLim = RTC_SUN_VANISH && e.sunSkip ? env_vanish_limit(e.focus, e.intensity, col) : -__builtin_inf();
    return e;
}

constexpr int kMaxCullMaskWords = 6144;
// ... 1 lines not shown
```

raytracingc_amd/csrc/rtc_plan.cpp:

```cpp
#include "rtc_plan.h"
#include "rtc_regroup.h"

#include <algorithm>
#include <cstring>
#include <initializer_list>

namespace rtcplan {

void init(State &s)
{
    memset(&s, 0, sizeof s);
}

namespace {
size_t align_up(size_t v, size_t a) { return (v + a - 1) / a * a; }

struct Emitter {
    Plan &p;
    void op(int kind, int stream, int event, int kernel)
    {
        if (p.nOps < (int)(sizeof p.ops / sizeof p.ops[0]))
            p.ops[p.nOps++] = Op{kind, stream, event, kernel};
    }
    void record(int st, int ev) { op(kOpRecord, st, ev, -1); }
    void wait(int st, int ev) { op(kOpWait, st, ev, -1); }
    void kernel(int st, int k, int stopEv = kEvNone) { op(kOpKernel, st, stopEv, k); }
};

void layout_slot(Plan &p, size_t maskWords)
{
    const size_t entries = (size_t)kGeoLists * p.geoCap, counters = (size_t)kGeoLists * kGeoCountStride * 4;
    const struct { size_t used, align, padAfter; } rows[kScratchRegions] = {
         {p.tiles * maskWords * 8, 1, 0},
         {p.tiles * 8, 1, 0},
         {p.blocks * 4, 1, 0},
         {(p.blocks + 4) * 4, 1, counters},
         {entries * kItemRecordBytes, kItemRecordBytes, 0},
         {(size_t)p.superX * p.superY * maskWords * 8, 8, 0},
         {p.tiles * 64 * 4, 256, 0},
         {entries * 4, 1, p.tiles * 4},
    };
    size_t off = 0, budget = 0;
    for (int b = 0; b < kScratchRegions; ++b) {
        p.reg[b] = Region{align_up(off, rows[b].align), rows[b].used};
        off = p.reg[b].offset + rows[b].used + rows[b].padAfter;
        budget += rows[b].used + rows[b].padAfter + (rows[b].align > 1 ? rows[b].align : 0);
    }
    p.slotBytes = align_up(budget, 256);
}

uint64_t stream_id(int st, uint64_t caller)
{
    return st == kStCull0 ? kIdCull0 : st == kStCull1 ? kIdCull1 : caller;
}
}

bool sphere_split(int sphereCount, bool gateAllows, int flags)
{
    return sphereCount > 0 && sphereCount <= kSplitSpheresMax && (gateAllows || (flags & RTC_F_SPLIT_SPHERES)) &&
           !(flags & (RTC_F_NO_COOP | RTC_F_NO_REORDER | RTC_F_NO_TILE_CULL | RTC_F_DEBUG_BOUNCES));
}

Request make_request(const RtcRenderDesc &d, int rows, const SceneShape &sc, uint64_t stream, uint64_t colors,
                     uint64_t accum, bool segments, const float cam[13], const float env[14])
{
    Request r;
    memset(&r, 0, sizeof r);
    r.stream = stream;
    r.flags = d.flags;
    r.width = d.width;
    r.rows = rows;
    r.rowStride = d.rowStride;
    r.spp = d.spp;
    r.sphereCount = d.trianglesOnly ? 0 : sc.sphereCount;
    r.sphereSplit = sphere_split(r.sphereCount, sc.splitGate, d.flags);
    r.triPadded = sc.triPadded;
    r.maskWords = sc.maskWords;
    r.segments = segments;
    r.key.colors = colors;
    r.key.accum = accum;
    memcpy(r.key.cam, cam, sizeof r.key.cam);
    memcpy(r.key.env, env, sizeof r.key.env);
    const int dims[9] = {d.width, d.height, rows, d.rowStart, d.rowStride, d.spp, d.maxBounce,
                         (d.flags & RTC_F_HOIST_PRIMARY) ? 1 : 0, d.rowBand > 1 ? __builtin_ctz((unsigned)d.rowBand) : 0};
    memcpy(r.key.dims, dims, sizeof dims);
    memcpy(r.origin, cam, sizeof r.origin);
    r.height = d.height;
    return r;
}

void set_draw_cache(Request &r, int eligible)
{
    r.drawCache = eligible & 3;
}

void set_sample_range(Request &r, int first, int count, uint64_t rngState)
{
    r.resume = true;
    r.sampleFirst = first;
    r.sampleCount = count;
    r.rngState = rngState;
    r.flags &= ~RTC_F_OVERLAP;
}

void set_first_hit(Request &r, const uint64_t ids[4])
{
    r.firstHit = true;
    memcpy(r.hit, ids, sizeof r.hit);
    r.flags &= RTC_F_NO_TILE_CULL;
    r.segments = false;
    r.key.colors = r.key.accum = 0;
}

int geometry_error(const RtcRenderDesc &d)
{
    if (d.width <= 0 || d.height <= 0 || d.rowStride <= 0 || d.rowStart < 0 || d.rowBand < 0 || d.rowBand > 64 ||
        (d.rowBand & (d.rowBand - 1)) != 0)
        return 1;
    return (long long)d.width * d.height > (1ll << 31) / 4 ? 2 : 0;
}

void plan_launch(const State &s, const Request &r, Plan &p)
{
    memset(&p, 0, sizeof p);
    p.after = s;
    State &n = p.after;
    Emitter E{p};
    if (r.rows <= 0) {
        p.empty = true;
        if (!r.firstHit) {
            E.record(kStCaller, kEvGeometry);
            E.record(kStCaller, kEvFrame);
        }
        return;
    }
    const size_t px = (size_t)r.width * (size_t)r.rows;
    p.debug = (r.flags & RTC_F_DEBUG_BOUNCES) != 0;
    p.resume = r.resume;
    p.resumeRead = r.resume && r.sampleFirst > 0;
    p.cull = !(r.flags & RTC_F_NO_TILE_CULL) && r.maskWords <= 6144;
    p.fused = p.cull && !p.debug && (r.sphereCount == 0 || r.sphereSplit) &&
              !(r.flags & (RTC_F_NO_COOP | RTC_F_NO_REORDER)) && !r.firstHit;
    p.chain = p.fused;
    p.gridX = (unsigned)((r.width + 15) / 16);
    p.gridY = (unsigned)((r.rows + 15) / 16);
    p.blocks = (size_t)p.gridX * p.gridY;
    p.tiles = 4 * p.blocks;
    p.superX = (p.gridX + 3) / 4;
    p.superY = (p.gridY + 3) / 4;
    p.superCull = p.cull && px > kSuperCullPixels && r.maskWords > 0;
    p.geoCap = (int)((p.tiles + kGeoLists - 1) / kGeoLists * 64);
    p.wideItems = r.width > kItemCoordMax || r.rows > kItemCoordMax;
    p.overlap = (r.flags & RTC_F_OVERLAP) && p.fused && !r.segments && !r.resume;
    p.half = p.overlap ? s.flip : 0;
    p.gen = s.gen;
    if (p.overlap)
        n.slotGens[p.half] |= (unsigned char)(1u << s.gen);
    p.smallShare = r.rowStride > 1 && px <= kInlineSumPixels;
    p.chainOnCs = p.overlap && (p.smallShare || px > kInlineSumPixels);
    p.merge = p.chainOnCs && p.smallShare && !r.noMerge;
    p.needCst2 = p.chainOnCs && !s.cst2;
    if (p.needCst2)
        n.cst2 = true;
    p.cs = p.chainOnCs ? ((p.half & 1) ? kStCull1 : kStCull0) : kStCaller;
    p.gs = p.chainOnCs ? p.cs : kStCaller;
    const uint64_t csId = stream_id(p.cs, r.stream);

    const bool waitAll = !p.overlap && !r.firstHit;
    int waitSky = -1;
    for (int h = 0; h < kSlots; ++h)
        if (s.skyPending[h] &&
            (waitAll || (h == p.half && p.cs == kStCaller) ||
             (!r.firstHit &&
              (s.skyKey[h].colors == r.key.colors || (r.key.accum && s.skyKey[h].accum == r.key.accum)) &&
              memcmp(&s.skyKey[h], &r.key, sizeof r.key) != 0)) &&
            (waitSky < 0 || s.skySeq[h] > s.skySeq[waitSky]))
            waitSky = h;
    if (waitSky >= 0) {
        E.wait(kStCaller, kEvSkyDone0 + waitSky);
        const unsigned long long upTo = s.skySeq[waitSky];
        for (int h = 0; h < kSlots; ++h)
            if (s.skySeq[h] <= upTo)
                n.skyPending[h] = false;
    }

    if (p.cull) {
        layout_slot(p, (size_t)r.maskWords);
        p.scratchNeed = kSlots * p.slotBytes;
        p.scratchGrow = p.scratchNeed > s.scratchCap;
        if (p.scratchGrow)
            n.scratchCap = p.scratchNeed;
        const size_t slotStride = r.legacySlotLayout ? p.slotBytes : n.scratchCap / kSlots;
        p.slotOffset = (size_t)p.half * slotStride;
    }
    if (p.chain) {
        p.geoSet = s.geoSeq % kGeoRing;
        p.geoSetNext = (s.geoSeq + 1) % kGeoRing;
        p.cullPrio = p.smallShare && px > 400000;
        if (r.spp > 0 && !(r.flags & RTC_F_CHAIN_INLINE) && !p.smallShare && !p.chainOnCs) {
            const size_t per = (size_t)(r.resume ? r.sampleCount : r.spp) * kSampleSlotBytes + sizeof(int);
            const size_t cap = std::min<size_t>(px, kSampleBufBudget / per);
            p.samplesNeed = cap * per + 256;
            p.samplesGrow = p.samplesNeed > s.samplesCap;
            if (p.samplesGrow)
                n.samplesCap = p.samplesNeed;
            p.sampleCap = (int)cap;
        }
        p.draws = ((r.drawCache >> (p.smallShare ? 1 : 0)) & 1) && r.spp > 0 && p.sampleCap == 0 && !r.segments &&
                  !r.resume && r.sphereCount == 0 && !(r.flags & (RTC_F_HOIST_PRIMARY | RTC_F_NO_DRAW_CACHE));
        if (p.draws) {
            p.drawReset = s.drawWidth != r.width || s.drawHeight != r.height;
            n.drawWidth = r.width, n.drawHeight = r.height;
            const size_t slotItemDraw = align_up((size_t)kGeoLists * p.geoCap * 4, 256);
            p.itemDrawNeed = kSlots * slotItemDraw;
            p.itemDrawGrow = p.itemDrawNeed > s.itemDrawCap;
            if (p.itemDrawGrow)
                n.itemDrawCap = p.itemDrawNeed;
            p.itemDrawOffset = (size_t)p.half * (n.itemDrawCap / kSlots);
        }
    }
    const auto bind = [&p](bool on, std::initializer_list<int> bufs) { for (int b : bufs) p.bound |= (unsigned)on << b; };
    bind(true, {kBufPrim, kBufSceneGen});
    bind(!r.firstHit, {kBufColors});
    bind(r.firstHit, {kBufHit});
    bind(p.cull, {kBufMask, kBufPixMask, kBufWeight});
    bind(p.cull && !p.fused && !r.firstHit, {kBufOrder});
    bind(p.superCull, {kBufSuperMask});
    bind(p.chain, {kBufGeoList, kBufGeoSet, kBufGeoSetNext});
    bind(p.merge, {kBufPixItem, kBufGeoColor});
    bind(p.sampleCap > 0, {kBufSamples});
    bind(r.key.accum != 0, {kBufAccum});
    bind(r.segments, {kBufSegSlots, kBufCallerSegments});
    bind(r.resume, {kBufRngState});
    bind(p.draws, {kBufDrawTable, kBufItemDraw});

    if (p.cs != kStCaller) {
        E.record(kStCaller, kEvCullSync);
        E.wait(p.cs, kEvCullSync);
        if (s.slotUsed[p.half]) {
            E.wait(p.cs, kEvSkyDone0 + p.half);
            E.wait(p.cs, kEvGeoDone0 + p.half);
        }
    }
    const bool waitPrevCull = p.chain && s.cullValid && s.cullStream != csId;
    if (waitPrevCull)
        E.wait(p.cs, kEvFork);
    const bool prepCurrent = s.prepValid[p.half] && s.prepStream[p.half] == csId &&
                             memcmp(s.prepOrigin[p.half], r.origin, sizeof r.origin) == 0;
    const bool countsZeroed = !p.chain || (s.cullValid && (s.cullStream == csId || waitPrevCull));
    if (p.chain)
        n.cullValid = false;
    if ((r.triPadded > 0 || p.chain) && !(prepCurrent && countsZeroed)) {
        p.prep = true;
        p.prepCounts = p.chain;
        E.kernel(p.cs, kKPrep);
        n.prepValid[p.half] = true;
        n.prepStream[p.half] = csId;
        memcpy(n.prepOrigin[p.half], r.origin, sizeof r.origin);
    }
    if (p.superCull)
        E.kernel(p.cs, kKSuperCull);
    if (r.firstHit) {
        if (p.cull)
            E.kernel(kStCaller, kKTileCull);
        E.kernel(kStCaller, kKFirstHit);
        return;
    }
    if (!p.cull) {
        E.kernel(kStCaller, kKRender);
    } else {
        E.kernel(p.cs, kKTileCull, p.fused ? kEvFork : kEvNone);
        if (p.chain) {
            n.geoSeq = s.geoSeq + 1;
            n.cullValid = true;
            n.cullStream = csId;
        }
        if (p.cs != kStCaller && !p.chainOnCs)
            E.wait(kStCaller, kEvFork);
        if (!p.fused) {
            E.kernel(kStCaller, kKOrder);
            E.kernel(kStCaller, kKRender);
        } else {
            if (p.merge) {
                E.kernel(p.gs, kKChain, kEvGeoDone0 + p.half);
                E.record(p.gs, kEvGeometry);
                E.wait(kStSide, kEvGeoDone0 + p.half);
                E.kernel(kStSide, kKSky);
                n.skyPending[p.half] = true;
                n.skyKey[p.half] = r.key;
                n.skySeq[p.half] = ++n.skyCount;
                E.record(kStSide, kEvSkyDone0 + p.half);
                E.record(kStSide, kEvFrame);
                n.slotUsed[p.half] = true;
                n.flip = (s.flip + 1) % kSlots;
                return;
            }
            if (p.resume) {
                E.kernel(kStCaller, kKSky);
                E.kernel(kStCaller, kKChain);
                if (p.sampleCap > 0)
                    E.kernel(kStCaller, kKAccum);
                E.record(kStCaller, kEvGeometry);
                if (r.segments)
                    E.kernel(kStCaller, kKReduce);
                E.record(kStCaller, kEvFrame);
                return;
            }
            E.wait(kStSide, kEvFork);
            E.kernel(kStSide, kKSky);
            E.record(kStSide, kEvJoin);
            if (p.overlap) {
                n.skyPending[p.half] = true;
                n.skyKey[p.half] = r.key;
                n.skySeq[p.half] = ++n.skyCount;
            }
            const bool accum = p.sampleCap > 0;
            E.kernel(p.gs, kKChain, p.overlap && !accum ? kEvGeoDone0 + p.half : kEvNone);
            if (accum)
                E.kernel(p.gs, kKAccum, p.overlap ? kEvGeoDone0 + p.half : kEvNone);
            E.record(p.gs, kEvGeometry);
            if (p.overlap) {
                E.wait(kStSide, kEvGeoDone0 + p.half);
                E.record(kStSide, kEvSkyDone0 + p.half);
                E.record(kStSide, kEvFrame);
                n.slotUsed[p.half] = true;
                n.flip = (s.flip + 1) % kSlots;
                return;
            }
            E.wait(kStCaller, kEvJoin);
            if (r.segments)
                E.kernel(kStCaller, kKReduce);
            E.record(kStCaller, kEvFrame);
            return;
        }
    }
    E.record(kStCaller, kEvGeometry);
    if (r.segments)
        E.kernel(kStCaller, kKReduce);
    E.record(kStCaller, kEvFrame);
}

namespace {
enum When : int { kAlways, kIfMerge, kIfNotMerge, kIfPrepCounts, kIfResumeRead };
struct Touch {
    int kernel, buf, access, when;
};
const Touch kTouches[] = {
    {kKPrep, kBufPrim, kWrite, kAlways},          {kKPrep, kBufGeoSet, kWrite, kIfPrepCounts},
    {kKSuperCull, kBufPrim, kRead, kAlways},      {kKSuperCull, kBufSuperMask, kWrite, kAlways},
    {kKTileCull, kBufPrim, kRead, kAlways},       {kKTileCull, kBufSuperMask, kRead, kAlways},
    {kKTileCull, kBufMask, kWrite, kAlways},      {kKTileCull, kBufPixMask, kWrite, kAlways},
    {kKTileCull, kBufWeight, kWrite, kAlways},    {kKTileCull, kBufGeoList, kWrite, kAlways},
    {kKTileCull, kBufPixItem, kWrite, kAlways},   {kKTileCull, kBufGeoSet, kAtomic, kAlways},
    {kKTileCull, kBufGeoSetNext, kWrite, kAlways},
    {kKSky, kBufPixMask, kRead, kAlways},         {kKSky, kBufPixItem, kRead, kAlways},
    {kKSky, kBufGeoColor, kRead, kAlways},        {kKSky, kBufGeoSet, kRead, kIfMerge},
    {kKSky, kBufColors, kKeyedWrite, kAlways},    {kKSky, kBufAccum, kKeyedWrite, kAlways},
    {kKSky, kBufSegSlots, kAtomic, kAlways},
    {kKChain, kBufPrim, kRead, kAlways},          {kKChain, kBufMask, kRead, kAlways},
    {kKChain, kBufGeoList, kRead, kAlways},       {kKChain, kBufGeoSet, kRead, kAlways},
    {kKChain, kBufSamples, kWrite, kAlways},      {kKChain, kBufGeoColor, kWrite, kAlways},
    {kKChain, kBufColors, kKeyedWrite, kIfNotMerge}, {kKChain, kBufAccum, kKeyedWrite, kAlways},
    {kKChain, kBufSegSlots, kAtomic, kAlways},
    {kKAccum, kBufGeoSet, kRead, kAlways},        {kKAccum, kBufSamples, kRead, kAlways},
    {kKAccum, kBufColors, kKeyedWrite, kAlways},  {kKAccum, kBufAccum, kKeyedWrite, kAlways},
    {kKOrder, kBufWeight, kRead, kAlways},        {kKOrder, kBufOrder, kWrite, kAlways},
    {kKRender, kBufPrim, kRead, kAlways},         {kKRender, kBufMask, kRead, kAlways},
    {kKRender, kBufOrder, kRead, kAlways},        {kKRender, kBufColors, kKeyedWrite, kAlways},
    {kKRender, kBufAccum, kKeyedWrite, kAlways},  {kKRender, kBufSegSlots, kAtomic, kAlways},
    {kKReduce, kBufSegSlots, kWrite, kAlways},    {kKReduce, kBufCallerSegments, kWrite, kAlways},
    {kKSky, kBufRngState, kKeyedWrite, kAlways},   {kKChain, kBufRngState, kKeyedWrite, kAlways},
    {kKAccum, kBufRngState, kKeyedWrite, kAlways}, {kKRender, kBufRngState, kKeyedWrite, kAlways},
    {kKSky, kBufRngState, kRead, kIfResumeRead},   {kKChain, kBufRngState, kRead, kIfResumeRead},
    {kKAccum, kBufRngState, kRead, kIfResumeRead}, {kKRender, kBufRngState, kRead, kIfResumeRead},
    {kKSky, kBufAccum, kRead, kIfResumeRead},      {kKChain, kBufAccum, kRead, kIfResumeRead},
    {kKAccum, kBufAccum, kRead, kIfResumeRead},    {kKRender, kBufAccum, kRead, kIfResumeRead},
    {kKPrep, kBufSceneGen, kRead, kAlways},        {kKSuperCull, kBufSceneGen, kRead, kAlways},
    {kKTileCull, kBufSceneGen, kRead, kAlways},    {kKSky, kBufSceneGen, kRead, kAlways},
    {kKChain, kBufSceneGen, kRead, kAlways},       {kKRender, kBufSceneGen, kRead, kAlways},
    {kKFirstHit, kBufMask, kRead, kAlways},        {kKFirstHit, kBufPrim, kRead, kAlways},
    {kKFirstHit, kBufSceneGen, kRead, kAlways},    {kKFirstHit, kBufHit, kWrite, kAlways},
    {kKTileCull, kBufDrawTable, kWrite, kAlways},  {kKTileCull, kBufItemDraw, kWrite, kAlways},
    {kKChain, kBufItemDraw, kRead, kAlways},
};
}

int kernel_footprint(const Plan &p, const Request &r, int kernel, Footprint *out, int max)
{
    const struct { int res; unsigned long long id; } outside[kBufs - kScratchRegions] = {
        {kResPrim, (unsigned long long)p.half}, {kResGeoSet, p.geoSet}, {kResGeoSet, p.geoSetNext}, {kResSamples, 0},
        {kResSegSlots, 0}, {kResColors, r.key.colors}, {kResAccum, r.key.accum}, {kResCallerSegments, 0},
        {kResRngState, r.rngState}, {kResSceneGen, (unsigned long long)p.gen}, {kResHit, 0},
        {kResDrawTable, 0}, {kResItemDraw, (unsigned long long)p.half}};
    int k = 0;
    for (const Touch &t : kTouches) {
        const bool when = t.when == kAlways || (t.when == kIfResumeRead ? p.resumeRead
                                                : t.when == kIfPrepCounts ? p.prepCounts
                                                                          : p.merge == (t.when == kIfMerge));
        if (t.kernel != kernel || !p.binds(t.buf) || !when)
            continue;
        if (t.buf == kBufHit) {
            for (const uint64_t id : r.hit)
                if (id) {
                    if (k < max)
                        out[k] = Footprint{kResHit, t.access, id, 0, 1};
                    ++k;
                }
            continue;
        }
        if (k < max && t.buf < kScratchRegions)
            out[k] = Footprint{kResScratch, t.access, 0, p.slotOffset + p.reg[t.buf].offset,
                               p.slotOffset + p.reg[t.buf].offset + p.reg[t.buf].size};
        else if (k < max)
            out[k] = Footprint{outside[t.buf - kScratchRegions].res, t.access, outside[t.buf - kScratchRegions].id, 0, 1};
        ++k;
    }
    return k;
}

void plan_update(const State &s, int fault, UpdatePlan &u)
{
    memset(&u, 0, sizeof u);
    u.after = s;
    State &n = u.after;
    const int other = s.gen ^ 1;
    u.reads = s.gen;
    u.writes = fault == 3 ? s.gen : other;
    for (int h = 0; h < kSlots; ++h)
        if (s.slotGens[h] >> other & 1) {
            if (fault != 1)
                u.ops[u.nOps++] = Op{kOpWait, kStCaller, kEvSkyDone0 + h, -1};
            n.slotGens[h] = 0;
        }
    u.ops[u.nOps++] = Op{kOpKernel, kStCaller, kEvNone, kKRefit};
    n.gen = u.writes;
    if (fault != 2)
        for (int h = 0; h < kSlots; ++h)
            n.prepValid[h] = false;
}

int update_footprint(const UpdatePlan &u, Footprint *out, int max)
{
    const Footprint f[2] = {{kResSceneGen, kWrite, (unsigned long long)u.writes, 0, 1},
                            {kResSceneGen, kRead, (unsigned long long)u.reads, 0, 1}};
    for (int k = 0; k < 2 && k < max; ++k)
        out[k] = f[k];
    return 2;
}

void plan_regroup(const State &s, int levels, RegroupPlan &g)
{
    memset(&g, 0, sizeof g);
    UpdatePlan u;
    plan_update(s, 0, u);
    g.reads = u.reads, g.writes = u.writes;
    g.levels = levels < 0 ? 0 : levels > kRegroupMaxLevels ? kRegroupMaxLevels : levels;
    for (int i = 0; i + 1 < u.nOps; ++i)
        g.ops[g.nOps++] = u.ops[i];
    g.ops[g.nOps++] = Op{kOpKernel, kStCaller, kEvNone, kKRegroupCentroids};
    for (int l = 0; l < g.levels; ++l)
        g.ops[g.nOps++] = Op{kOpKernel, kStCaller, kEvNone, kKRegroupLevel};
    g.ops[g.nOps++] = Op{kOpKernel, kStCaller, kEvNone, kKRegroupIndex};
    g.ops[g.nOps++] = u.ops[u.nOps - 1];
    g.after = u.after;
}

int regroup_footprint(const RegroupPlan &g, int kernel, uint64_t scratch, Footprint *out, int max)
{
    const Footprint sr{kResRegroupScratch, kRead, scratch, 0, 1}, sw{kResRegroupScratch, kWrite, scratch, 0, 1};
    const Footprint mr{kResMembership, kRead, 0, 0, 1}, mw{kResMembership, kWrite, 0, 0, 1};
    Footprint f[3];
    int k = 0;
    if (kernel == kKRegroupCentroids) {
        f[k++] = sw;
    } else if (kernel == kKRegroupLevel) {
        f[k++] = sr, f[k++] = sw;
    } else if (kernel == kKRegroupIndex) {
        f[k++] = sr, f[k++] = mw;
    } else if (kernel == kKRefit) {
        UpdatePlan u{};
        u.reads = g.reads, u.writes = g.writes;
        k = update_footprint(u, f, 2);
        f[k++] = mr;
    }
    for (int j = 0; j < k && j < max; ++j)
        out[j] = f[j];
    return k;
}

void plan_query(const State &s, int kernel, TracePlan &t)
{
    memset(&t, 0, sizeof t);
    t.after = s;
    t.gen = s.gen;
    t.ops[t.nOps++] = Op{kOpKernel, kStCaller, kEvNone, kernel};
}

int query_footprint(const TracePlan &t, std::initializer_list<QueryRow> rows, Footprint *out, int max)
{
    int k = 0;
    const auto row = [&](const QueryRow &r) {
        if (!r.present)
            return;
        if (k < max)
            out[k] = Footprint{r.res, r.access, r.id, 0, 1};
        ++k;
    };
    row({kResSceneGen, kRead, (unsigned long long)t.gen, true});
    for (const QueryRow &r : rows)
        row(r);
    return k;
}

int trace_footprint(const TracePlan &t, uint64_t rays, const uint64_t hit[4], Footprint *out, int max)
{
    return query_footprint(t,
                           {{kResRays, kRead, rays, true},
                            {kResHit, kWrite, hit[0], hit[0] != 0},
                            {kResHit, kWrite, hit[1], hit[1] != 0},
                            {kResHit, kWrite, hit[2], hit[2] != 0},
                            {kResHit, kWrite, hit[3], hit[3] != 0}},
                           out, max);
}

int paths_footprint(const TracePlan &t, uint64_t rays, uint64_t seeds, uint64_t radiance, uint64_t seedsOut, bool segments,
                    bool readRadiance, Footprint *out, int max)
{
    return query_footprint(t,
                           {{kResRays, kRead, rays, true},
                            {kResSeeds, kRead, seeds, true},
                            {kResRadiance, kRead, radiance, readRadiance},
                            {kResRadiance, kWrite, radiance, true},
                            {kResSeeds, kWrite, seedsOut, seedsOut != 0},
                            {kResCallerSegments, kAtomic, 0, segments}},
                           out, max);
}

int occluded_footprint(const TracePlan &t, uint64_t rays, uint64_t tMax, uint64_t occluded, bool count, Footprint *out,
                       int max)
{
    return query_footprint(t,
                           {{kResRays, kRead, rays, true},
                            {kResTMax, kRead, tMax, tMax != 0},
                            {kResOccluded, kWrite, occluded, occluded != 0},
                            {kResCallerSegments, kAtomic, 0, count}},
                           out, max);
}

int pixels_footprint(const TracePlan &t, uint64_t pixels, uint64_t colors, uint64_t accum, uint64_t rngState, bool segments,
                     bool readState, Footprint *out, int max)
{
    return query_footprint(t,
                           {{kResPixelList, kRead, pixels, true},
                            {kResAccum, kRead, accum, readState},
                            {kResRngState, kRead, rngState, readState},
                            {kResAccum, kWrite, accum, true},
                            {kResRngState, kWrite, rngState, true},
                            {kResColors, kWrite, colors, colors != 0},
                            {kResCallerSegments, kAtomic, 0, segments}},
                           out, max);
}

}

struct RtcPlanSim {
    rtcplan::State st;
    rtcplan::SceneShape shape;
    int legacy;
    rtcplan::Plan last;
    bool ranged;
    int first, count;
    unsigned long long rngBuffer;
    int updateFault;
    bool hitNext;
    uint64_t hit[4];
    bool drawCache;
};

namespace {
template <class FootprintOf>
int serialise(const rtcplan::Op *o, int nOps, int *ops, int maxOps, unsigned long long *fp, int maxFp,
              const unsigned long long (&trailer)[5], FootprintOf footprint)
{
    int nf = 0;
    for (int i = 0; i < nOps && i < maxOps; ++i) {
        ops[4 * i] = o[i].kind, ops[4 * i + 1] = o[i].stream, ops[4 * i + 2] = o[i].event, ops[4 * i + 3] = o[i].kernel;
        if (o[i].kind != rtcplan::kOpKernel)
            continue;
        rtcplan::Footprint f[24];
        const int k = std::min(footprint(o[i], f, 24), 24);
        for (int j = 0; j < k; ++j, ++nf)
            if (fp && nf < maxFp) {
                unsigned long long *q = fp + 6 * (size_t)nf;
                q[0] = (unsigned long long)i, q[1] = (unsigned long long)f[j].res, q[2] = (unsigned long long)f[j].access;
                q[3] = f[j].id, q[4] = f[j].lo, q[5] = f[j].hi;
            }
    }
    if (fp && nf < maxFp) {
        unsigned long long *q = fp + 6 * (size_t)nf;
        q[0] = ~0ull;
        std::copy(trailer, trailer + 5, q + 1);
    }
    return nOps | ((nf + 1) << 8);
}

template <class FootprintOf>
int sim_query(RtcPlanSim *s, int kernel, int *ops, int maxOps, unsigned long long *fp, int maxFp, FootprintOf footprint)
{
    rtcplan::TracePlan t;
    rtcplan::plan_query(s->st, kernel, t);
    s->st = t.after;
    return serialise(t.ops, t.nOps, ops, maxOps, fp, maxFp, {0, (unsigned long long)t.gen, 0, 0, 0},
                     [&](const rtcplan::Op &, rtcplan::Footprint *f, int max) { return footprint(t, f, max); });
}
}

extern "C" int rtc_plan_sim_create(int triCount, int legacySlotLayout, RtcPlanSim **out)
{
    if (!out || triCount < 0)
        return RTC_EINVAL;
    RtcPlanSim *s = new RtcPlanSim();
    rtcplan::init(s->st);
    s->shape.triPadded = (triCount + 7) / 8 * 8;
    s->shape.maskWords = (s->shape.triPadded + 63) / 64;
    s->legacy = legacySlotLayout;
    *out = s;
    return 0;
}

extern "C" int rtc_plan_sim_set_spheres(RtcPlanSim *s, int sphereCount, int gateAllows)
{
    if (!s || sphereCount < 0)
        return RTC_EINVAL;
    s->shape.sphereCount = sphereCount;
    s->shape.splitGate = gateAllows != 0;
    return 0;
}

extern "C" int rtc_plan_sim_set_draw_cache(RtcPlanSim *s, int on)
{
    if (!s)
        return RTC_EINVAL;
    s->drawCache = on != 0;
    return 0;
}

extern "C" int rtc_plan_sim_set_sample_range(RtcPlanSim *s, int first, int count, unsigned long long rngBuffer)
{
    if (!s)
        return RTC_EINVAL;
    s->ranged = true;
    s->first = first, s->count = count, s->rngBuffer = rngBuffer;
    return 0;
}

extern "C" int rtc_plan_sim_set_first_hit(RtcPlanSim *s, unsigned long long prim, unsigned long long depth,
                                          unsigned long long normal, unsigned long long albedo)
{
    if (!s)
        return RTC_EINVAL;
    s->hitNext = true;
    s->hit[0] = prim, s->hit[1] = depth, s->hit[2] = normal, s->hit[3] = albedo;
    return 0;
}

extern "C" int rtc_plan_sim_release(RtcPlanSim *s)
{
    delete s;
    return 0;
}

extern "C" int rtc_plan_sim_launch(RtcPlanSim *s, const RtcRenderDesc *d, unsigned long long stream,
                                   unsigned long long colors, unsigned long long accum, int segments, const float cam[13],
                                   const float env[14], int *ops, int maxOps, unsigned long long *fp, int maxFp)
{
    if (!s || !d || !cam || !env)
        return RTC_EINVAL;
    rtcplan::Request r = rtcplan::make_request(*d, rtc_rows_selected(d), s->shape, stream, colors, accum, segments != 0,
                                               cam, env);
    r.legacySlotLayout = s->legacy != 0;
    if (s->hitNext) {
        s->hitNext = false;
        s->ranged = false;
        if (!(s->hit[0] | s->hit[1] | s->hit[2] | s->hit[3]) || (d->flags & ~RTC_F_NO_TILE_CULL) ||
            rtcplan::geometry_error(*d))
            return RTC_EINVAL;
        rtcplan::set_first_hit(r, s->hit);
    }
    if (s->ranged) {
        s->ranged = false;
        if (s->first < 0 || s->count <= 0 || s->first > d->spp - s->count || (d->flags & RTC_F_OVERLAP) || !accum ||
            !s->rngBuffer)
            return RTC_EINVAL;
        rtcplan::set_sample_range(r, s->first, s->count, s->rngBuffer);
    }
    if (s->drawCache)
        rtcplan::set_draw_cache(r, 3);
    rtcplan::Plan &p = s->last;
    rtcplan::plan_launch(s->st, r, p);
    s->st = p.after;
    return serialise(p.ops, p.nOps, ops, maxOps, fp, maxFp,
                     {p.scratchGrow || p.samplesGrow || p.drawReset || p.itemDrawGrow, (unsigned long long)p.half,
                      p.chainOnCs, p.overlap, p.slotOffset},
                     [&](const rtcplan::Op &o, rtcplan::Footprint *f, int max) {
                         return rtcplan::kernel_footprint(p, r, o.kernel, f, max);
                     });
}

extern "C" int rtc_plan_sim_set_update_fault(RtcPlanSim *s, int mode)
{
    if (!s || mode < 0 || mode > 3)
        return RTC_EINVAL;
    s->updateFault = mode;
    return 0;
}

extern "C" int rtc_plan_sim_update(RtcPlanSim *s, unsigned long long stream, int *ops, int maxOps, unsigned long long *fp,
                                   int maxFp)
{
    if (!s || !ops)
        return RTC_EINVAL;
    (void)stream;
    rtcplan::UpdatePlan u;
    rtcplan::plan_update(s->st, s->updateFault, u);
    s->st = u.after;
    return serialise(u.ops, u.nOps, ops, maxOps, fp, maxFp, {0, (unsigned long long)u.writes, 0, 0, 0},
                     [&](const rtcplan::Op &, rtcplan::Footprint *f, int max) {
                         return rtcplan::update_footprint(u, f, max);
                     });
}

extern "C" int rtc_plan_sim_regroup(RtcPlanSim *s, unsigned long long stream, unsigned long long scratch, int *ops,
                                    int maxOps, unsigned long long *fp, int maxFp)
{
    if (!s || !ops || !scratch || scratch % 16 || s->shape.triPadded <= 0 || s->shape.triPadded > kRegroupMaxTris)
        return RTC_EINVAL;
    (void)stream;
    rtcplan::RegroupPlan g;
    rtcplan::plan_regroup(s->st, regroup_levels(s->shape.triPadded), g);
    s->st = g.after;
    return serialise(g.ops, g.nOps, ops, maxOps, fp, maxFp, {0, (unsigned long long)g.writes, (unsigned long long)g.levels, 0, 0},
                     [&](const rtcplan::Op &o, rtcplan::Footprint *f, int max) {
                         return rtcplan::regroup_footprint(g, o.kernel, scratch, f, max);
                     });
}

extern "C" int rtc_plan_sim_trace_rays(RtcPlanSim *s, unsigned long long stream, unsigned long long rays,
                                       const unsigned long long hit[4], int flags, int *ops, int maxOps,
                                       unsigned long long *fp, int maxFp)
{
    if (!s || !ops || !rays || !hit || !(hit[0] | hit[1] | hit[2] | hit[3]) || (flags & ~RTC_F_NO_CLUSTER_CULL))
        return RTC_EINVAL;
    (void)stream;
    const uint64_t ids[4] = {hit[0], hit[1], hit[2], hit[3]};
    return sim_query(s, rtcplan::kKTraceRays, ops, maxOps, fp, maxFp,
                     [&](const rtcplan::TracePlan &t, rtcplan::Footprint *f, int max) {
                         return rtcplan::trace_footprint(t, rays, ids, f, max);
                     });
}

extern "C" int rtc_plan_sim_trace_paths(RtcPlanSim *s, unsigned long long stream, unsigned long long rays,
                                        unsigned long long seeds, unsigned long long radiance,
                                        unsigned long long seedsOut, unsigned long long segments, int sampleFirst,
                                        int flags, int *ops, int maxOps, unsigned long long *fp, int maxFp)
{
    if (!s || !ops || !rays || !seeds || !radiance || sampleFirst < 0 ||
        (flags & ~(RTC_F_NO_CLUSTER_CULL | RTC_F_WAVE_PER_RAY)))
        return RTC_EINVAL;
    (void)stream;
    return sim_query(s, rtcplan::kKTracePaths, ops, maxOps, fp, maxFp,
                     [&](const rtcplan::TracePlan &t, rtcplan::Footprint *f, int max) {
                         return rtcplan::paths_footprint(t, rays, seeds, radiance, seedsOut, segments != 0, sampleFirst > 0,
                                                         f, max);
                     });
}

extern "C" int rtc_plan_sim_occluded(RtcPlanSim *s, unsigned long long stream, unsigned long long rays,
                                     unsigned long long tMax, unsigned long long occluded, unsigned long long count,
                                     int flags, int *ops, int maxOps, unsigned long long *fp, int maxFp)
{
// ... 37 lines not shown
```

raytracingc_amd/csrc/rtc_plan.h:

```cpp
#pragma once
#include <cstddef>
#include <cstdint>
#include <initializer_list>

#include "../../include/rtc.h"

namespace rtcplan {

constexpr int kSlots = 8;
constexpr int kGeoRing = 16;
constexpr int kGeoLists = 16;
constexpr int kGeoCountStride = 32;
constexpr size_t kItemRecordBytes = 16;
constexpr int kItemCoordMax = 65535;
constexpr size_t kInlineSumPixels = 600000;
constexpr size_t kSuperCullPixels = 400000;
constexpr size_t kSampleBufBudget = (size_t)2 << 30;
constexpr size_t kSampleSlotBytes = 12;
constexpr int kSplitSpheresMax = 32;
constexpr double kSplitMaxHitShare = 0.5;

enum Stream : int { kStCaller = 0, kStCull0 = 1, kStCull1 = 2, kStSide = 3, kStreams = 4 };
enum Event : int {
    kEvNone = -1,
    kEvCullSync = 0,
    kEvFork = 1,
    kEvJoin = 2,
    kEvSkyDone0 = 3,
    kEvGeoDone0 = 3 + kSlots,
    kEvFrame = 3 + 2 * kSlots,
    kEvGeometry = 4 + 2 * kSlots,
    kEvents = 5 + 2 * kSlots
};
enum Kernel : int { kKPrep, kKSuperCull, kKTileCull, kKSky, kKChain, kKAccum, kKOrder, kKRender, kKReduce,
                    kKRefit ,
                    kKFirstHit ,
                    kKTraceRays ,
                    kKTracePaths ,
                    kKOccluded ,
                    kKRegroupCentroids, kKRegroupLevel, kKRegroupIndex,
                    kKRenderPixels  };
static_assert(kKRefit == 9 && kKFirstHit == 10 && kKTraceRays == 11 && kKTracePaths == 12 && kKOccluded == 13 &&
                  kKRegroupCentroids == 14 && kKRegroupLevel == 15 && kKRegroupIndex == 16 && kKRenderPixels == 17,
              "the kernels' numbers are the test hooks' encoding");
enum OpKind : int { kOpKernel = 0, kOpRecord = 1, kOpWait = 2 };
struct Op {
    int kind;
    int stream;
    int event;
    int kernel;
};

constexpr uint64_t kIdCull0 = ~0ull - 1, kIdCull1 = ~0ull - 2;

struct Key {
    uint64_t colors, accum;
    float cam[13], env[14];
    int dims[9];
};

struct State {
    int flip;
    bool slotUsed[kSlots];
    bool skyPending[kSlots];
    Key skyKey[kSlots];
    unsigned long long skySeq[kSlots], skyCount;
    unsigned long long geoSeq;
    bool cullValid;
    uint64_t cullStream;
    bool prepValid[kSlots];
    uint64_t prepStream[kSlots];
    float prepOrigin[kSlots][3];
    size_t scratchCap, samplesCap;
    bool cst2;
    int gen;
    unsigned char slotGens[kSlots];
    int drawWidth, drawHeight;
    size_t itemDrawCap;
};
void init(State &s);

struct Request {
    uint64_t stream;
    int flags;
    int width, rows, rowStride;
    int spp;
    int sphereCount;
    bool sphereSplit;
    int triPadded, maskWords;
    bool segments;
    Key key;
    float origin[3];
    bool legacySlotLayout;
    bool noMerge;
    bool resume;
    int sampleFirst, sampleCount;
    uint64_t rngState;
    bool firstHit;
    uint64_t hit[4];
    int drawCache;
    int height;
};

struct SceneShape {
    int triPadded, maskWords, sphereCount;
    bool splitGate;
};
Request make_request(const RtcRenderDesc &d, int rows, const SceneShape &sc, uint64_t stream, uint64_t colors,
                     uint64_t accum, bool segments, const float cam[13], const float env[14]);

void set_sample_range(Request &r, int first, int count, uint64_t rngState);

void set_first_hit(Request &r, const uint64_t ids[4]);

void set_draw_cache(Request &r, int eligible);

int geometry_error(const RtcRenderDesc &d);

enum Buf : int {
    kBufMask,
    kBufPixMask,
    kBufWeight,
    kBufOrder,
    kBufGeoList,
    kBufSuperMask,
    kBufPixItem,
    kBufGeoColor,
    kScratchRegions,
    kBufPrim = kScratchRegions,
    kBufGeoSet, kBufGeoSetNext,
    kBufSamples,
    kBufSegSlots,
    kBufColors, kBufAccum, kBufCallerSegments,
    kBufRngState,
    kBufSceneGen,
    kBufHit,
    kBufDrawTable, kBufItemDraw,
    kBufs
};
struct Region {
    size_t offset, size;
};

struct Plan {
    bool empty;
    bool cull, fused, chain, overlap, smallShare, chainOnCs, superCull, debug;
    bool resume;
    bool resumeRead;
    bool merge;
    int half;
    int gen;
    int cs, gs;
    unsigned gridX, gridY, superX, superY;
    size_t blocks, tiles;
    int geoCap;
    bool wideItems;
    size_t slotBytes;
    size_t slotOffset;
    Region reg[kScratchRegions];
    unsigned bound;
    bool binds(int b) const { return (bound >> b & 1u) != 0; }
    size_t scratchNeed;
    bool scratchGrow, samplesGrow, needCst2;
    size_t samplesNeed;
    int sampleCap;
    unsigned long long geoSet, geoSetNext;
    bool prep, prepCounts;
    bool cullPrio;
    bool draws, drawReset, itemDrawGrow;
    size_t itemDrawNeed, itemDrawOffset;
    int nOps;
    Op ops[40];
    State after;
};

bool sphere_split(int sphereCount, bool gateAllows, int flags);

void plan_launch(const State &s, const Request &r, Plan &p);

enum Res : int { kResScratch = 0, kResPrim = 1, kResGeoSet = 2, kResSamples = 3, kResSegSlots = 4, kResColors = 5,
                 kResAccum = 6, kResCallerSegments = 7, kResRngState = 8, kResSceneGen = 9 ,
                 kResHit = 10 , kResRays = 11 ,
                 kResDrawTable = 12, kResItemDraw = 13 ,
                 kResSeeds = 14 , kResRadiance = 15 ,
                 kResTMax = 16 , kResOccluded = 17 ,
                 kResMembership = 18 ,
                 kResRegroupScratch = 19 ,
                 kResPixelList = 20  };
enum Access : int { kRead = 0, kWrite = 1, kAtomic = 2, kKeyedWrite = 3  };
struct Footprint {
    int res, access;
    unsigned long long id;
    unsigned long long lo, hi;
};
int kernel_footprint(const Plan &p, const Request &r, int kernel, Footprint *out, int max);

struct UpdatePlan {
    int reads, writes;
    int nOps;
    Op ops[kSlots + 1];
    State after;
};
void plan_update(const State &s, int fault, UpdatePlan &u);
int update_footprint(const UpdatePlan &u, Footprint *out, int max);

constexpr int kRegroupMaxLevels = 32;
struct RegroupPlan {
    int reads, writes;
    int levels;
    int nOps;
    Op ops[kSlots + 3 + kRegroupMaxLevels];
    State after;
};
void plan_regroup(const State &s, int levels, RegroupPlan &g);
int regroup_footprint(const RegroupPlan &g, int kernel, uint64_t scratch, Footprint *out, int max);

struct TracePlan {
    int gen;
    int nOps;
    Op ops[1];
    State after;
};
void plan_query(const State &s, int kernel, TracePlan &t);
struct QueryRow {
    int res, access;
    unsigned long long id;
    bool present;
};
int query_footprint(const TracePlan &t, std::initializer_list<QueryRow> rows, Footprint *out, int max);

int trace_footprint(const TracePlan &t, uint64_t rays, const uint64_t hit[4], Footprint *out, int max);
int paths_footprint(const TracePlan &t, uint64_t rays, uint64_t seeds, uint64_t radiance, uint64_t seedsOut, bool segments,
                    bool readRadiance, Footprint *out, int max);
int occluded_footprint(const TracePlan &t, uint64_t rays, uint64_t tMax, uint64_t occluded, bool count, Footprint *out,
                       int max);
int pixels_footprint(const TracePlan &t, uint64_t pixels, uint64_t colors, uint64_t accum, uint64_t rngState, bool segments,
                     bool readState, Footprint *out, int max);

}
```

raytracingc_amd/csrc/rtc_probe.hip:

```cpp
#include <hip/hip_runtime.h>

#include <cstring>
#include <vector>

#include "rtc_layout.h"
#include "rtc_internal.h"
#include "rtc_hip_util.h"

__global__ void probe_tri_kernel(const Ray *rays, const Triangle *tris, size_t n, int *didHit, float *dst)
{
    size_t i = blockIdx.x * (size_t)blockDim.x + threadIdx.x;
    if (i >= n)
        return;
    const Ray R = rays[i];
    const Triangle T = tris[i];
    const V3 A = v3(T.posA);
    float d = 0.f;
    bool h = ray_triangle(v3(R.pos), v3(R.dir), A, sub(v3(T.posB), A), sub(v3(T.posC), A), v3(T.normal), d);
    didHit[i] = h ? 1 : 0;
    dst[i] = h ? d : 0.f;
}

__global__ void probe_sphere_kernel(const Ray *rays, const Sphere *sph, size_t n, int *didHit, float *dst,
                                    vec3 *normal)
// ... 263 lines not shown
    Scratch sc;
    unsigned *dsd;
    float *du, *dn;
    vec3 *dd;
    const size_t m = n * (size_t)draws;
    ALLOC_IN(dsd, seeds, n * sizeof(unsigned));
    ALLOC_OUT(du, m * sizeof(float));
    ALLOC_OUT(dn, m * sizeof(float));
    ALLOC_OUT(dd, m * sizeof(vec3));
    hipLaunchKernelGGL(probe_random_kernel, dim3(probe_blocks(n)), dim3(256), 0, nullptr, dsd, n, draws, du, dn, dd);
    HIP_TRY(hipGetLastError());
    HIP_TRY(hipMemcpy(uniform, du, m * sizeof(float), hipMemcpyDeviceToHost));
    HIP_TRY(hipMemcpy(normal, dn, m * sizeof(float), hipMemcpyDeviceToHost));
    HIP_TRY(hipMemcpy(direction, dd, m * sizeof(vec3), hipMemcpyDeviceToHost));
    return 0;
}

extern "C" int rtc_probe_cluster_bound(const Triangle *tris, int triCount, const Ray *rays, size_t n,
                                       unsigned long long counts[7])
{
    if (!counts || triCount < 0 || (triCount > 0 && !tris) || (n > 0 && !rays))
        return rtc_fail(RTC_EINVAL, "rtc_probe_cluster_bound: bad argument");
    memset(counts, 0, 7 * sizeof(unsigned long long));
    if (int rc = probe_prelude())
        return rc;
    if (n == 0 || triCount == 0)
        return 0;
    RtcDeviceScene *s = nullptr;
    if (int rc = rtc_scene_upload(tris, triCount, nullptr, 0, -1, &s))
        return rc;
    Scratch sc;
    Ray *dr = nullptr;
    unsigned long long *dc = nullptr;
    int rc = 0;
    hipError_t e = sc.alloc((void **)&dr, n * sizeof(Ray));
    if (e == hipSuccess)
        e = hipMemcpy(dr, rays, n * sizeof(Ray), hipMemcpyHostToDevice);
    if (e == hipSuccess)
        e = sc.alloc((void **)&dc, 7 * sizeof(unsigned long long));
    if (e == hipSuccess)
        e = hipMemset(dc, 0, 7 * sizeof(unsigned long long));
    if (e == hipSuccess) {
        const SceneRecords &g = s->current();
        hipLaunchKernelGGL(probe_cluster_kernel, dim3(probe_blocks(n)), dim3(256), 0, nullptr, g.clTris, g.clusters,
                           s->clusterCount, kClusterSize, s->clusterCount * kClusterSize, true, dr, n, dc);
        e = hipGetLastError();
        if (e == hipSuccess && s->chunkCount > 1) {
            hipLaunchKernelGGL(probe_cluster_kernel, dim3(probe_blocks(n)), dim3(256), 0, nullptr, g.clTris, g.chunks,
                               s->chunkCount, kClusterSize * kChunkClusters, s->clusterCount * kClusterSize, false, dr, n,
                               dc);
            e = hipGetLastError();
        }
    }
    if (e == hipSuccess)
        e = hipMemcpy(counts, dc, 7 * sizeof(unsigned long long), hipMemcpyDeviceToHost);
    if (e != hipSuccess)
        rc = rtc_fail(-(int)e, "rtc_probe_cluster_bound: %s", hipGetErrorString(e));
    rtc_scene_release(s);
    return rc;
}

extern "C" int rtc_probe_item_records(const Triangle *tris, int triCount, const Sphere *spheres, int sphereCount,
                                      const Scene *scene, const RtcCamera *cam, const RtcRenderDesc *d, int counts[16],
                                      int info[4], unsigned *records, size_t maxRecords, unsigned long long *pixMask,
                                      size_t maxTiles)
{
    static_assert(kGeoLists == 16, "counts[16]: one per sub-list");
    if (!scene || !cam || !d || !counts || !info || !records || !pixMask || triCount < 0 || sphereCount < 0)
        return rtc_fail(RTC_EINVAL, "rtc_probe_item_records: bad argument");
    if (int rc = probe_prelude())
        return rc;
    RtcDeviceScene *s = nullptr;
    if (int rc = rtc_scene_upload(tris, triCount, spheres, sphereCount, -1, &s))
        return rc;
    Scratch sc;
    int rc = 0;
    const auto run = [&]() -> int {
        unsigned char *dColors = nullptr;
        HIP_TRY(sc.alloc((void **)&dColors, (size_t)d->width * (size_t)(rtc_rows_selected(d) > 0 ? rtc_rows_selected(d) : 1) * 3));
        RtcCullItems it{};
        if (const int r = rtc_cull_items(s, scene, cam, d, dColors, &it))
            return r;
        HIP_TRY(hipDeviceSynchronize());
        int raw[kGeoSetInts];
        HIP_TRY(hipMemcpy(raw, it.geoCount, sizeof raw, hipMemcpyDeviceToHost));
        size_t total = 0;
        for (int l = 0; l < kGeoLists; ++l) {
            counts[l] = raw[l * kGeoCountStride] < it.geoCap ? raw[l * kGeoCountStride] : it.geoCap;
            total += (size_t)counts[l];
        }
        info[0] = it.geoCap, info[1] = it.tilesX, info[2] = (int)it.tiles, info[3] = it.wide;
        if (total > maxRecords || it.tiles > maxTiles)
            return rtc_fail(RTC_EINVAL, "rtc_probe_item_records: %zu records, %zu tiles: the outputs are smaller", total,
                            it.tiles);
        size_t at = 0;
        for (int l = 0; l < kGeoLists; ++l) {
            HIP_TRY(hipMemcpy(records + at * kItemRecDwords, it.geoList + (size_t)l * it.geoCap * kItemRecDwords,
                              (size_t)counts[l] * kItemRecDwords * 4, hipMemcpyDeviceToHost));
            at += (size_t)counts[l];
        }
        HIP_TRY(hipMemcpy(pixMask, it.pixMask, it.tiles * 8, hipMemcpyDeviceToHost));
        return 0;
    };
    rc = run();
    rtc_scene_release(s);
    return rc;
}

__global__ void probe_primary_kernel(PrimaryView V, int rows, const DevPrimF *primF, int triCount, unsigned char *kept)
{
    const size_t i = blockIdx.x * (size_t)blockDim.x + threadIdx.x;
    if (i >= (size_t)rows * (size_t)V.width)
        return;
    const int x = (int)(i % (size_t)V.width), r = (int)(i / (size_t)V.width);
    const V3 dir = primary_dir(V, x, launch_row_y(V, r));
    for (int t = 0; t < triCount; ++t) {
        const DevPrimF F = primF[t];
        kept[i * (size_t)triCount + t] = !prim_backfacing(dir, F) && prim_pass(dir, F) ? 1 : 0;
    }
}

__global__ void probe_cone_kernel(PrimaryView V, int tilesX, int tiles, const DevPrimF *primF, int triCount, double *cones,
                                  unsigned char *pruned)
{
    const int tile = blockIdx.x * blockDim.x + threadIdx.x;
    if (tile >= tiles)
        return;
    const TileCone K = tile_cone(V, tile % tilesX, tile / tilesX);
    cones[tile * 4 + 0] = K.eDir, cones[tile * 4 + 1] = K.vmin, cones[tile * 4 + 2] = K.vmax, cones[tile * 4 + 3] = K.ok ? 1.0 : 0.0;
    for (int t = 0; t < triCount; ++t)
        pruned[(size_t)tile * (size_t)triCount + t] = K.ok && tile_prunes(K, primF[t]) ? 1 : 0;
}

extern "C" int rtc_probe_primary_cull(const Triangle *tris, int triCount, const Scene *scene, const RtcCamera *cam,
                                      const RtcRenderDesc *d, unsigned char *kept, size_t maxKept,
                                      unsigned long long *tileBits, size_t maxWords, unsigned long long *pixMask,
                                      size_t maxTiles, int info[4], float *primF, double *cones, unsigned char *pruned)
{
    if (!tris || triCount <= 0 || !scene || !cam || !d || !kept || !tileBits || !pixMask || !info)
        return rtc_fail(RTC_EINVAL, "rtc_probe_primary_cull: bad argument");
    if (int rc = probe_prelude())
        return rc;
    RtcDeviceScene *s = nullptr;
    if (int rc = rtc_scene_upload(tris, triCount, nullptr, 0, -1, &s))
        return rc;
    Scratch sc;
    const auto run = [&]() -> int {
        const int rows = rtc_rows_selected(d);
        if (rows <= 0)
            return rtc_fail(RTC_EINVAL, "rtc_probe_primary_cull: the launch has no rows");
        unsigned char *dColors = nullptr;
        HIP_TRY(sc.alloc((void **)&dColors, (size_t)d->width * (size_t)rows * 3));
        RtcCullItems it{};
        if (const int r = rtc_cull_items(s, scene, cam, d, dColors, &it))
            return r;
        HIP_TRY(hipDeviceSynchronize());
        const size_t pixels = (size_t)rows * (size_t)d->width, words = it.tiles * (size_t)it.maskWords;
        info[0] = (int)it.tiles, info[1] = it.tilesX, info[2] = it.maskWords, info[3] = it.level0;
        if (pixels * (size_t)triCount > maxKept || words > maxWords || it.tiles > maxTiles || triCount > it.triPadded)
            return rtc_fail(RTC_EINVAL, "rtc_probe_primary_cull: %zu verdicts, %zu words, %zu tiles: the outputs are smaller",
                            pixels * (size_t)triCount, words, it.tiles);
        unsigned char *dk = nullptr;
        HIP_TRY(sc.alloc((void **)&dk, pixels * (size_t)triCount));
        PrimaryView V{};
        V.width = d->width, V.height = d->height, V.rows = rows, V.rowStart = d->rowStart, V.rowStride = d->rowStride;
        V.rowBandShift = d->rowBand > 1 ? __builtin_ctz((unsigned)d->rowBand) : 0;
        V.ex = v3(cam->ex), V.ey = v3(cam->ey), V.ez = v3(cam->ez), V.fov = cam->fov;
// ... 29 lines not shown
```

raytracingc_amd/csrc/rtc_render.hip:

```cpp
#include <hip/hip_runtime.h>
#include <hip/hip_ext.h>

#include <algorithm>
#include <chrono>
#include <cmath>
#include <cstdarg>
#include <cstdio>
#include <cstdlib>
#include <cstring>
#include <vector>
#ifdef RTC_DIAG
__device__ unsigned g_rtc_bmfall[65536];
#endif

#include "../../include/rtc.h"
#include "rtc_layout.h"
#include "rtc_internal.h"
#include "rtc_hip_util.h"
#include "rtc_staged.h"

static_assert(sizeof(vec3) == 12, "vec3 layout");
static_assert(sizeof(Material) == 20, "Material layout");
static_assert(sizeof(Sphere) == 36, "Sphere layout");
static_assert(sizeof(Triangle) == 68, "Triangle layout");
static_assert(sizeof(Scene) == 56, "Scene layout");
static_assert(sizeof(Color) == 3, "Color layout");
static_assert(sizeof(Ray) == 24, "Ray layout");
static_assert(sizeof(RtcRenderDesc) == 36, "RtcRenderDesc layout (ctypes mirror: raytracingc_amd/_abi.py)");

using namespace rtcdev;

static thread_local char g_err[1024] = "";

extern "C" int rtc_fail(int code, const char *fmt, ...)
{
    va_list ap;
    va_start(ap, fmt);
    vsnprintf(g_err, sizeof g_err, fmt, ap);
    va_end(ap);
    return code;
}

extern "C" void rtc_log(int level, const char *fmt, ...)
{
    const char *v = getenv("RTC_VERBOSE");
    if (!v || atoi(v) < level)
        return;
    va_list ap;
    va_start(ap, fmt);
    vfprintf(stderr, fmt, ap);
    va_end(ap);
}

extern "C" const char *rtc_last_error(void) { return g_err; }
extern "C" const char *rtc_version(void) { return "rtc-mi355x 0.1 (gfx950)"; }


extern "C" int rtc_device_count(int *count)
{
    if (!count)
        return rtc_fail(RTC_EINVAL, "null count");
    *count = 0;
    int n = 0;
    hipError_t e = hipGetDeviceCount(&n);
    if (e != hipSuccess || n <= 0)
        return rtc_fail(RTC_ENODEV, "no HIP device: %s", hipGetErrorString(e));
    *count = n;
    return 0;
}

#include "rtc_params.h"
#include "rtc_closest.h"
#include "rtc_diag.h"
#include "rtc_cull.h"
#include "rtc_lane.h"
#include "rtc_sky.h"
#include "rtc_chain.h"
#include "rtc_first_hit.h"
#include "rtc_trace_rays.h"
#include "rtc_trace_paths.h"
#include "rtc_occluded.h"
#include "rtc_render_pixels.h"

template <typename... K, typename... A>
static hipError_t launch_stop(void (*k)(K...), dim3 g, dim3 b, size_t sh, hipStream_t st, hipEvent_t stop, A... args)
{
    if (stop) {
        hipExtLaunchKernelGGL(k, g, b, (std::uint32_t)sh, st, nullptr, stop, 0u, args...);
        return hipGetLastError();
    }
    hipLaunchKernelGGL(k, g, b, sh, st, args...);
    return hipGetLastError();
}

struct ChainFlags {
    bool multi, count, hits, general, spheres, resume, draws;
    constexpr bool operator==(const ChainFlags &o) const
    {
        return multi == o.multi && count == o.count && hits == o.hits && general == o.general && spheres == o.spheres &&
               resume == o.resume && draws == o.draws;
    }
};

constexpr ChainFlags chain_flags(bool multi, bool count, bool defer, bool hits, bool spheres, bool resume,
                                 bool draws = false)
{
    const bool general = multi || count || defer || spheres || resume;
    return ChainFlags{multi, count, hits && !general, general, spheres, resume, draws && !general};
}

struct ChainVariant {
    ChainFlags flags;
    void (*kernel)(RenderParams);
};
#define CHAIN_ROW(...) ChainVariant{ChainFlags{__VA_ARGS__}, rtc_render_chain<__VA_ARGS__>}

template <int n> constexpr int chain_variant(const ChainVariant (&table)[n], ChainFlags f)
{
    for (int i = 0; i < n; ++i)
        if (table[i].flags == f)
            return i;
    return n;
}

constexpr int kInMulti = 1, kInCount = 2, kInDefer = 4, kInHits = 8, kInSpheres = 16, kInResume = 32, kInDraws = 64;
template <typename Rule> constexpr bool every_chain_launch(Rule rule)
{
    for (int in = 0; in < 128; ++in)
        if (!rule(in, chain_flags(in & kInMulti, in & kInCount, in & kInDefer, in & kInHits, in & kInSpheres,
                                  in & kInResume, in & kInDraws)))
            return false;
    return true;
}
static_assert(every_chain_launch([](int in, ChainFlags f) { return f.general == ((in & ~(kInHits | kInDraws)) != 0); }),
              "GENERAL whenever the launch is multi-chunk, counting, deferring, with spheres or a pass");
static_assert(every_chain_launch([](int in, ChainFlags f) { return f.hits == ((in & ~kInDraws) == kInHits); }),
              "HITS only when none of them holds and the scene is hit-heavy");
static_assert(every_chain_launch([](int in, ChainFlags f) { return f.draws == (!!(in & kInDraws) && !f.general); }),
              "DRAWS only in the two kernels without GENERAL");
static_assert(every_chain_launch([](int in, ChainFlags f) {
                  return f.multi == !!(in & kInMulti) && f.count == !!(in & kInCount) &&
                         f.spheres == !!(in & kInSpheres) && f.resume == !!(in & kInResume);
              }),
              "MULTI, COUNT, SPHERES and RESUME are the launch's own");
static_assert(every_chain_launch([](int, ChainFlags f) { return !((f.hits || !f.general) && (f.spheres || f.resume)); }),
              "SPHERES and RESUME kernels are GENERAL ones without HITS");

#ifdef RTC_AB_NO_SLOTS
constexpr bool kAbNoSlots = true;
#else
constexpr bool kAbNoSlots = false;
#endif
struct Launch {
    const RtcDeviceScene *s;
    const rtcplan::Plan &pl;
    RenderParams P;
    int wgsPerCu;
    size_t chainDyn;
    bool resume;
    const RtcHitBuffers *hit = nullptr;
    DrawCache dc{};
    dim3 grid() const { return dim3(pl.gridX, pl.gridY); }
    template <typename T> T *region(int buf) const
    {
        return pl.binds(buf) ? (T *)(s->scratch + pl.slotOffset + pl.reg[buf].offset) : nullptr;
    }
};

static int check_arguments(const char *who, const Scene *scene, const RtcCamera *cam, const RtcRenderDesc *d,
                           const void *dColors, const RtcHitBuffers *hit)
{
    if ((!scene && !hit) || !cam || !d || (!dColors && !hit))
        return rtc_fail(RTC_EINVAL, "%s: null argument", who);
    if (hit && !hit->prim && !hit->depth && !hit->normal && !hit->albedo)
        return rtc_fail(RTC_EINVAL, "%s: no buffer asked for (prim, depth, normal and albedo are all null)", who);
    const int geometry = rtcplan::geometry_error(*d);
    if (geometry == 1)
        return rtc_fail(RTC_EINVAL, "%s: bad geometry %dx%d rows %d+k*%d", who, d->width, d->height, d->rowStart,
                        d->rowStride);
    if (geometry)
        return rtc_fail(RTC_EINVAL, "frame too large");
    if (hit && (d->flags & ~RTC_F_NO_TILE_CULL))
        return rtc_fail(RTC_EINVAL, "%s: flags 0x%x (a first-hit launch takes RTC_F_NO_TILE_CULL and no other flag)", who,
                        d->flags);
    if (d->flags & (RTC_F_COOP4 | RTC_F_COOP8 | RTC_F_PIPE | RTC_F_SPEC))
        return rtc_fail(RTC_EINVAL, "%s: RTC_F_COOP4 / COOP8 / PIPE / SPEC name kernels that were "
                                    "removed (rtc_render_chain renders every geometry pixel)", who);
    return 0;
}

static RenderParams render_params(const RtcDeviceScene *s, const Scene *scene, const RtcCamera &cam,
                                  const RtcRenderDesc &d, int rows, void *dColors, float *dAccum,
                                  unsigned long long *dSegments, const RtcSampleRange *range)
{
    RenderParams P;
    memset(&P, 0, sizeof P);
    P.triCount = s->triCount, P.triPadded = s->triPadded, P.maskWords = s->maskWords;
    P.sphereCount = d.trianglesOnly ? 0 : s->sphereCount;
    P.clusterCount = s->clusterCount;
    P.chunkCount = s->chunkCount, P.clusterCull = !(d.flags & RTC_F_NO_CLUSTER_CULL);
    P.colors = (unsigned char *)dColors, P.accum = dAccum;
    P.segments = dSegments, P.segSlots = s->segSlots;
    P.width = d.width, P.height = d.height;
    P.rows = rows, P.rowStart = d.rowStart, P.rowStride = d.rowStride;
    P.rowBandShift = d.rowBand > 1 ? __builtin_ctz((unsigned)d.rowBand) : 0;
    P.spp = range ? range->count : d.spp, P.maxBounce = d.maxBounce;
    P.sampleFirst = range ? range->first : 0;
    P.hoist = (d.flags & RTC_F_HOIST_PRIMARY) ? 1 : 0;
    P.invSpp = d.spp > 0 ? (float)(1. / (double)d.spp) : 0.f;
    P.origin = v3(cam.origin), P.ex = v3(cam.ex), P.ey = v3(cam.ey), P.ez = v3(cam.ez), P.fov = cam.fov;
    if (scene)
        P.env = env_of(*scene);
    return P;
}

static int regrow(unsigned char *&buf, size_t &cap, size_t need)
{
    if (buf)
        HIP_TRY(hipFree(buf));
    buf = nullptr;
    cap = 0;
    HIP_TRY(hipMalloc(&buf, need));
    cap = need;
    return 0;
}

static int grow_capacity(RtcDeviceScene *ms, const rtcplan::Plan &pl)
{
    if (pl.needCst2) {
        int leastPrio = 0, greatestPrio = 0;
        HIP_TRY(hipDeviceGetStreamPriorityRange(&leastPrio, &greatestPrio));
        HIP_TRY(hipStreamCreateWithPriority(&ms->cst2, hipStreamNonBlocking, greatestPrio));
        ms->plan.cst2 = true;
    }
    if (const int rc = pl.scratchGrow ? regrow(ms->scratch, ms->plan.scratchCap, pl.scratchNeed) : 0)
        return rc;
    return pl.samplesGrow ? regrow(ms->samples, ms->plan.samplesCap, pl.samplesNeed) : 0;
}

static void bind_plan(Launch &L, int flags)
{
    const RtcDeviceScene *s = L.s;
    const rtcplan::Plan &pl = L.pl;
    RenderParams &P = L.P;
    const SceneRecords &g = s->gen[pl.gen];
    P.tris = g.tris, P.mats = g.mats, P.spheres = g.spheres;
    P.clTris = g.clTris, P.clusters = g.clusters, P.chunks = g.chunks;
    P.primF = s->primF + (size_t)pl.half * s->primStride;
    P.primX = s->primX + (size_t)pl.half * s->primStride;
    P.blocksX = (int)pl.gridX;
    P.tileMask = L.region<unsigned long long>(rtcplan::kBufMask);
    P.pixMask = L.region<unsigned long long>(rtcplan::kBufPixMask);
    P.order = (flags & RTC_F_NO_REORDER) ? nullptr : L.region<int>(rtcplan::kBufOrder);
    P.superMask = L.region<unsigned long long>(rtcplan::kBufSuperMask);
    P.superX = P.superMask ? (int)pl.superX : 0;
    P.geoList = L.region<unsigned>(rtcplan::kBufGeoList);
    P.pixItem = L.region<unsigned>(rtcplan::kBufPixItem);
    P.geoColor = L.region<unsigned>(rtcplan::kBufGeoColor);
    if (pl.binds(rtcplan::kBufGeoSet)) {
        P.geoCount = s->geoCounts + (size_t)pl.geoSet * kGeoSetInts;
        P.geoCountNext = s->geoCounts + (size_t)pl.geoSetNext * kGeoSetInts;
        P.geoCap = pl.geoCap;
        P.wideItems = pl.wideItems;
        P.cullPrio = pl.cullPrio;
    }
    if (pl.binds(rtcplan::kBufDrawTable) && pl.binds(rtcplan::kBufItemDraw)) {
        const RtcDeviceScene::Draws &D = s->draws;
        L.dc.table = D.table, L.dc.ctr = D.ctr, L.dc.blockSeed = D.blockSeed, L.dc.pool = (float4 *)D.pool;
        L.dc.itemDraw = (unsigned *)(D.itemDraw + pl.itemDrawOffset);
        L.dc.capacity = (unsigned)D.capacity;
        L.dc.tablePixels = (unsigned)((size_t)P.width * (size_t)P.height);
        L.dc.parity = D.parity;
        P.drawPool = L.dc.pool;
        P.itemDraw = L.dc.itemDraw;
    }
    if (pl.binds(rtcplan::kBufSamples)) {
        P.sampleBuf = (SampleSlot *)s->samples;
        P.itemPix = (int *)(s->samples + (size_t)pl.sampleCap * (size_t)P.spp * sizeof(SampleSlot));
        P.sampleCap = pl.sampleCap;
    }
}

static bool chain_prim_f_staged(const RtcDeviceScene *s, int wgsPerCu)
{
    const size_t recLds = s->chunkCount <= 1 ? (size_t)soa_slots(s->clusterCount * kClusterSize) * sizeof(DevTri) : 0;
    const size_t pfLds = (size_t)s->triPadded * sizeof(DevPrimF);
    return s->chunkCount <= 1 && kChainStaticLds + recLds + pfLds <= kCuLds / (size_t)wgsPerCu;
}

static int draw_cache_eligible(const RtcDeviceScene *s)
{
    if (s->draws.blocks == 0 || s->triCount == 0)
        return 0;
    return (chain_prim_f_staged(s, s->chainWgsFull) ? 1 : 0) | (chain_prim_f_staged(s, RTC_CHAIN_WGS_SHARE) ? 2 : 0);
}

static void size_chain_lds(Launch &L)
{
    const RtcDeviceScene *s = L.s;
    L.wgsPerCu = L.pl.smallShare ? RTC_CHAIN_WGS_SHARE : s->chainWgsFull;
    const size_t recLds = s->chunkCount <= 1 ? (size_t)soa_slots(s->clusterCount * kClusterSize) * sizeof(DevTri) : 0;
    const size_t pfLds = (size_t)s->triPadded * sizeof(DevPrimF);
    L.P.chainPrimF = chain_prim_f_staged(s, L.wgsPerCu);
    const size_t floorLds = chain_lds_floor(L.wgsPerCu);
    L.chainDyn = std::max<size_t>(recLds + (L.P.chainPrimF ? pfLds : 0),
                                  floorLds > kChainStaticLds ? floorLds - kChainStaticLds : 0);
}

static int run_prep(const Launch &L, hipStream_t os, hipEvent_t)
{
    const int n = L.s->triPadded;
    HIP_TRY(launch_stop(rtc_prep_primary, dim3((n + 8 + 63) / 64), dim3(64), 0, os, nullptr, L.P.tris,
                        const_cast<DevPrimF *>(L.P.primF), const_cast<DevPrimX *>(L.P.primX), n > 0 ? n + 8 : 0,
                        L.P.origin, L.pl.prepCounts ? L.P.geoCount : nullptr));
    return 0;
}

static int run_super_cull(const Launch &L, hipStream_t os, hipEvent_t)
{
    HIP_TRY(launch_stop(rtc_super_cull, dim3(L.pl.superX, L.pl.superY), dim3(64), 0, os, nullptr, L.P,
                        L.region<unsigned long long>(rtcplan::kBufSuperMask)));
    return 0;
}

static int run_tile_cull(const Launch &L, hipStream_t os, hipEvent_t ev)
{
    unsigned long long *const mask = L.region<unsigned long long>(rtcplan::kBufMask);
    unsigned long long *const pixMask = L.region<unsigned long long>(rtcplan::kBufPixMask);
    unsigned *const weight = L.region<unsigned>(rtcplan::kBufWeight);
    const size_t lds = (size_t)L.s->maskWords * sizeof(unsigned long long);
    const bool spheres = L.P.geoList && L.P.sphereCount > 0;
    static void (*const kCull[2])(RenderParams, unsigned long long *, unsigned *, unsigned long long *) = {
        rtc_tile_cull, rtc_tile_cull_sph<true>};
    if (L.pl.draws) {
        HIP_TRY(launch_stop(rtc_tile_cull_draws<true>, L.grid(), dim3(kBlock), lds, os, nullptr, L.P, mask, weight, pixMask,
                            L.dc));
        HIP_TRY(launch_stop(rtc_fill_draws<true>, dim3(kFillBlocks), dim3(256), 0, os, ev, L.dc));
        const_cast<RtcDeviceScene *>(L.s)->draws.parity ^= 1;
        return 0;
    }
    HIP_TRY(launch_stop(kCull[spheres], L.grid(), dim3(kBlock), lds, os, ev, L.P, mask, weight, pixMask));
    return 0;
}

static int run_sky(const Launch &L, hipStream_t os, hipEvent_t)
{
    const RenderParams &P = L.P;
    const bool wide = L.pl.smallShare && (size_t)P.width * (size_t)P.rows > 400000;
    const bool general = P.geoColor || P.hoist || P.accum || P.segments;
    static void (*const kSky[2][3])(RenderParams) = {
        {rtc_render_sky_rows<1, false>, rtc_render_sky_rows<1, true>, rtc_render_sky_rows<1, true, true>},
        {rtc_render_sky_rows<4, false>, rtc_render_sky_rows<4, true>, rtc_render_sky_rows<4, true, true>}};
    if (L.s->timing)
        HIP_TRY(hipEventRecord(L.s->evSky0, os));
    const dim3 grid((P.width + 63) / 64, wide ? (P.rows + 3) / 4 : P.rows);
    HIP_TRY(launch_stop(kSky[wide][L.resume ? 2 : general], grid, dim3(wide ? 256 : 64), 0, os, nullptr, P));
    if (L.s->timing)
        HIP_TRY(hipEventRecord(L.s->evSky1, os));
    return 0;
}

static int run_chain(const Launch &L, hipStream_t os, hipEvent_t ev)
{
    const RtcDeviceScene *s = L.s;
    const RenderParams &P = L.P;
    const dim3 cg((unsigned)(L.wgsPerCu * s->cuCount)), cb(kChainBlock);
    const bool multi = s->chunkCount > 1, count = P.segments != nullptr;
    const bool defer = P.sampleCap > 0 || P.hoist || !P.chainPrimF;
    const bool hits = s->chainWgsFull == RTC_CHAIN_WGS_HIT && RTC_CHAIN_WGS_HIT != RTC_CHAIN_WGS_FULL;
    static constexpr ChainVariant kChain[] = {
        CHAIN_ROW(false, false, false, false, false, false), CHAIN_ROW(false, false, true, false, false, false),
        CHAIN_ROW(false, false, false, true, false, false),  CHAIN_ROW(false, true, false, true, false, false),
        CHAIN_ROW(true, false, false, true, false, false),   CHAIN_ROW(true, true, false, true, false, false),
        CHAIN_ROW(false, false, false, true, true, false),   CHAIN_ROW(false, true, false, true, true, false),
        CHAIN_ROW(true, false, false, true, true, false),    CHAIN_ROW(true, true, false, true, true, false),
        CHAIN_ROW(false, false, false, true, false, true),   CHAIN_ROW(false, true, false, true, false, true),
        CHAIN_ROW(true, false, false, true, false, true),    CHAIN_ROW(true, true, false, true, false, true),
        CHAIN_ROW(false, false, false, true, true, true),    CHAIN_ROW(false, true, false, true, true, true),
        CHAIN_ROW(true, false, false, true, true, true),     CHAIN_ROW(true, true, false, true, true, true),
        CHAIN_ROW(false, false, false, false, false, false, true), CHAIN_ROW(false, false, true, false, false, false, true)};
    constexpr int kVariants = (int)(sizeof kChain / sizeof kChain[0]);
    static_assert(every_chain_launch([](int, ChainFlags f) { return chain_variant(kChain, f) < kVariants; }),
                  "every launch selects an instantiated kernel");
    const int variant =
        chain_variant(kChain, chain_flags(multi, count, defer, hits, P.sphereCount > 0, L.resume, L.pl.draws));
    if (kChain[variant].flags.draws != L.pl.draws)
        return rtc_fail(RTC_EINVAL, "rtc_render_chain: the launch was planned with the draw cache but runs a GENERAL kernel");
    {
        const ChainFlags &f = kChain[variant].flags;
        RtcChainReport &r = const_cast<RtcDeviceScene *>(s)->chainReport;
        r = RtcChainReport{f.multi,      f.count,    f.hits,          f.general,       f.spheres,     f.resume,
                           P.chainPrimF, L.wgsPerCu, (int)L.chainDyn, s->clusterCount, s->chunkCount, r.launches + 1};
    }
    if (s->timing)
        HIP_TRY(hipEventRecord(s->evHeavy0, os));
    HIP_TRY(launch_stop(kChain[variant].kernel, cg, cb, L.chainDyn, os, ev, P));
    if (s->timing)
        HIP_TRY(hipEventRecord(s->evHeavy1, os));
    return 0;
}

static int run_accumulate(const Launch &L, hipStream_t os, hipEvent_t ev)
{
    const unsigned g = (unsigned)std::min<size_t>(((size_t)L.P.sampleCap + 255) / 256, 1024);
    if (L.resume)
        HIP_TRY(launch_stop(rtc_accumulate_samples_resume<true>, dim3(g), dim3(256), 0, os, ev, L.P));
    else if (!kAbNoSlots)
        HIP_TRY(launch_stop(rtc_accumulate_samples, dim3(g), dim3(256), 0, os, ev, L.P));
    else if (ev)
        HIP_TRY(hipEventRecord(ev, os));
    return 0;
}

static int run_order(const Launch &L, hipStream_t os, hipEvent_t)
{
    HIP_TRY(launch_stop(rtc_order_blocks, dim3(1), dim3(1024), 0, os, nullptr, L.region<unsigned>(rtcplan::kBufWeight),
                        (int)L.pl.blocks, L.region<int>(rtcplan::kBufOrder)));
    return 0;
}

static int run_render(const Launch &L, hipStream_t os, hipEvent_t)
{
    static void (*const kRender[2][2][2])(RenderParams) = {
        {{rtc_render_kernel<false, false>, rtc_render_kernel<false, false, true>},
         {rtc_render_kernel<false, true>, rtc_render_kernel<false, true, true>}},
        {{rtc_render_kernel<true, false>, rtc_render_kernel<true, false, true>},
         {rtc_render_kernel<true, true>, rtc_render_kernel<true, true, true>}}};
    HIP_TRY(launch_stop(kRender[L.P.sphereCount > 0][L.pl.debug][L.resume], L.grid(), dim3(kBlock), 0, os, nullptr,
                        L.P));
    return 0;
}

static int run_reduce(const Launch &L, hipStream_t os, hipEvent_t)
{
    HIP_TRY(launch_stop(rtc_reduce_segments, dim3(1), dim3(kSegSlots), 0, os, nullptr, L.P.segSlots, L.P.segments));
    return 0;
}

static int run_first_hit(const Launch &L, hipStream_t os, hipEvent_t)
{
    static void (*const kFirstHit[2])(RenderParams, int *, float *, float *, float *) = {rtc_first_hit<false>,
                                                                                         rtc_first_hit<true>};
    const RtcHitBuffers &h = *L.hit;
    HIP_TRY(launch_stop(kFirstHit[L.P.sphereCount > 0], L.grid(), dim3(kBlock), 0, os, nullptr, L.P, h.prim, h.depth,
                        h.normal, h.albedo));
    return 0;
}

static int (*const kPlanned[])(const Launch &, hipStream_t, hipEvent_t) = {
    run_prep,  run_super_cull, run_tile_cull, run_sky, run_chain,    run_accumulate,
    run_order, run_render,     run_reduce,    nullptr, run_first_hit};
static_assert(sizeof kPlanned / sizeof kPlanned[0] == rtcplan::kKFirstHit + 1 && rtcplan::kKRefit == rtcplan::kKReduce + 1,
              "one function per planned kernel");

static int render_rows(const RtcDeviceScene *s, const Scene *scene, const RtcCamera *cam, const RtcRenderDesc *d,
                       void *dColors, float *dAccum, unsigned long long *dSegments, void *stream, RtcCullItems *items,
                       const RtcSampleRange *range = nullptr, unsigned *dRngState = nullptr,
                       const RtcHitBuffers *hit = nullptr)
{
    const char *const who = hit ? "rtc_render_first_hit_async" : "rtc_render_rows_async";
    if (!s)
        return rtc_fail(RTC_EINVAL, "%s: null scene", who);
    RtcDeviceScene *const ms = const_cast<RtcDeviceScene *>(s);
    const hipEvent_t geoEvent = hit ? nullptr : s->geoEvent, frameEvent = hit ? nullptr : s->frameEvent;
    if (!hit)
        ms->geoEvent = ms->frameEvent = nullptr;
    if (const int rc = check_arguments(who, scene, cam, d, dColors, hit))
        return rc;
    if (range) {
        if (!dAccum || !dRngState)
            return rtc_fail(RTC_EINVAL, "rtc_render_samples_async: the accumulator and the RNG-state buffer are required");
        if (range->first < 0 || range->count <= 0 || range->first > d->spp - range->count)
            return rtc_fail(RTC_EINVAL, "rtc_render_samples_async: samples [%d, %d + %d) are not within the frame's %d",
                            range->first, range->first, range->count, d->spp);
        if (d->flags & RTC_F_OVERLAP)
            return rtc_fail(RTC_EINVAL, "rtc_render_samples_async: RTC_F_OVERLAP (an unjoined sky pass would race the next "
                                        "pass's read of the accumulator)");
    }
    const int rows = rtc_rows_selected(d);
    RtcDeviceGuard guard(s->device);
    if (!guard.ok())
        return rtc_fail(RTC_ENODEV, "%s: cannot select the scene's device %d", who, s->device);
    const hipStream_t st = (hipStream_t)stream;
    if (rows == 0) {
        for (hipEvent_t ev : {geoEvent, frameEvent})
            if (ev)
                HIP_TRY(hipEventRecord(ev, st));
        return 0;
    }
    static thread_local rtcplan::Plan pl;
    Launch L{s, pl, render_params(s, scene, *cam, *d, rows, dColors, dAccum, dSegments, range), 0, 0, range != nullptr,
             hit};
    const RenderParams &P = L.P;
    const EnvParams &E = P.env;
    const float camKey[13] = {P.origin.x, P.origin.y, P.origin.z, P.ex.x, P.ex.y, P.ex.z, P.ey.x,
                              P.ey.y,     P.ey.z,     P.ez.x,     P.ez.y, P.ez.z, P.fov};
    const float envKey[14] = {E.sun.x,    E.sun.y,    E.sun.z,    E.horizon.x, E.horizon.y, E.horizon.z, E.zenith.x,
                              E.zenith.y, E.zenith.z, E.ground.x, E.ground.y,  E.ground.z,  E.focus,     E.intensity};
    rtcplan::Request rq = rtcplan::make_request(
        *d, rows, rtcplan::SceneShape{s->triPadded, s->maskWords, s->sphereCount, s->sphereSplitGate},
        (uint64_t)(uintptr_t)st, (uint64_t)(uintptr_t)dColors, (uint64_t)(uintptr_t)dAccum, dSegments != nullptr, camKey,
        envKey);
    rq.noMerge = !RTC_SKY_MERGE;
    if (range)
        rtcplan::set_sample_range(rq, range->first, range->count, (uint64_t)(uintptr_t)dRngState);
    if (hit) {
        const uint64_t ids[4] = {(uint64_t)(uintptr_t)hit->prim, (uint64_t)(uintptr_t)hit->depth,
                                 (uint64_t)(uintptr_t)hit->normal, (uint64_t)(uintptr_t)hit->albedo};
        rtcplan::set_first_hit(rq, ids);
    }
    if (!hit && !items)
        rtcplan::set_draw_cache(rq, draw_cache_eligible(s));
    rtcplan::plan_launch(s->plan, rq, pl);
    ms->plan.prepValid[pl.half] = false;
    if (!hit)
        ms->plan.cullValid = false;
    if (const int rc = grow_capacity(ms, pl))
        return rc;
    if (pl.draws)
        if (const int rc = rtc_draws_prepare(ms, d->width, d->height, pl.drawReset, pl.itemDrawGrow ? pl.itemDrawNeed : 0))
            return rc;
    bind_plan(L, d->flags);
    if (range)
        L.P.rngState = dRngState;
    size_chain_lds(L);
    const hipStream_t streams[rtcplan::kStreams] = {st, s->cst, ms->cst2, s->side};
    hipEvent_t events[rtcplan::kEvents] = {};
    events[rtcplan::kEvCullSync] = s->evCullSync, events[rtcplan::kEvFork] = s->evFork, events[rtcplan::kEvJoin] = s->evJoin;
    events[rtcplan::kEvFrame] = frameEvent, events[rtcplan::kEvGeometry] = geoEvent;
    for (int h = 0; h < kSkySlots; ++h)
        events[rtcplan::kEvSkyDone0 + h] = s->evSkyDone[h], events[rtcplan::kEvGeoDone0 + h] = s->evGeoDone[h];
    for (int i = 0; i < pl.nOps; ++i) {
        const rtcplan::Op &op = pl.ops[i];
        const hipStream_t os = streams[op.stream];
        const hipEvent_t ev = op.event >= 0 && op.event < rtcplan::kEvents ? events[op.event] : nullptr;
        if (op.kind == rtcplan::kOpRecord) {
            if (ev)
                HIP_TRY(hipEventRecord(ev, os));
        } else if (op.kind == rtcplan::kOpWait) {
            HIP_TRY(hipStreamWaitEvent(os, ev, 0));
        } else if (op.kernel < 0 || op.kernel > rtcplan::kKFirstHit || !kPlanned[op.kernel]) {
            return rtc_fail(RTC_EINVAL, "%s: unknown planned kernel %d", who, op.kernel);
        } else if (items && op.kernel > rtcplan::kKTileCull) {
            if (ev)
                HIP_TRY(hipEventRecord(ev, os));
        } else if (const int rc = kPlanned[op.kernel](L, os, ev)) {
            return rc;
        }
    }
    if (!hit)
        ms->timed = pl.fused && s->timing;
    ms->plan = pl.after;
    if (items) {
        if (!pl.chain)
            return rtc_fail(RTC_EINVAL, "rtc_cull_items: not a split launch");
        *items = RtcCullItems{P.geoCount, P.geoList,   P.pixMask, P.geoCap,    P.blocksX * 2,        pl.tiles, P.wideItems,
                              P.tileMask, P.maskWords, P.primF,   P.triPadded, pl.superCull ? 1 : 0};
    }
    return 0;
}

extern "C" int rtc_render_rows_async(const RtcDeviceScene *s, const Scene *scene, const RtcCamera *cam,
                                     const RtcRenderDesc *d, void *dColors, float *dAccum,
                                     unsigned long long *dSegments, void *stream)
{
    return render_rows(s, scene, cam, d, dColors, dAccum, dSegments, stream, nullptr);
}

extern "C" int rtc_render_samples_async(const RtcDeviceScene *s, const Scene *scene, const RtcCamera *cam,
                                        const RtcRenderDesc *d, const RtcSampleRange *range, void *dColors,
                                        float *dAccum, unsigned int *dRngState, unsigned long long *dSegments,
                                        void *stream)
{
    if (!range)
        return rtc_fail(RTC_EINVAL, "rtc_render_samples_async: null sample range");
    return render_rows(s, scene, cam, d, dColors, dAccum, dSegments, stream, nullptr, range, dRngState);
}

extern "C" int rtc_render_first_hit_async(const RtcDeviceScene *s, const RtcCamera *cam, const RtcRenderDesc *d,
                                          const RtcHitBuffers *out, void *stream)
{
    if (!s)
        return rtc_fail(RTC_EINVAL, "rtc_render_first_hit_async: null scene");
    if (!out)
        return rtc_fail(RTC_EINVAL, "rtc_render_first_hit_async: null argument");
    return render_rows(s, nullptr, cam, d, nullptr, nullptr, nullptr, stream, nullptr, nullptr, nullptr, out);
}


static int no_refusal() { return 0; }

template <class Own>
static int refuse_query(const char *who, const char *noun, const RtcDeviceScene *s, bool nullArgument,
                        const char *noneAsked, size_t n, int flags, int allowed, const char *allowedNames, Own own)
{
// ... 359 lines not shown
}

extern "C" int rtc_copy_async(void *dst, const void *src, size_t bytes, int blocks, void *stream)
{
    if ((!dst || !src) && bytes)
        return rtc_fail(RTC_EINVAL, "rtc_copy_async: null pointer");
    if (bytes == 0)
        return 0;
    if ((((size_t)dst | (size_t)src) & 15) != 0)
        return rtc_fail(RTC_EINVAL, "rtc_copy_async: pointers must be 16-byte aligned");
    if (blocks <= 0)
        blocks = 32;
    hipLaunchKernelGGL(rtc_copy_kernel, dim3((unsigned)blocks), dim3(256), 0, (hipStream_t)stream,
                       (const unsigned char *)src, (unsigned char *)dst, bytes);
    HIP_TRY(hipGetLastError());
    return 0;
}

template __global__ void rtc_render_sky_rows<4, true>(RenderParams);
template __global__ void rtc_render_sky_rows<4, false>(RenderParams);
template __global__ void rtc_render_sky_rows<1, true>(RenderParams);
template __global__ void rtc_render_sky_rows<1, false>(RenderParams);
template __global__ void rtc_render_chain<true, true, false, true>(RenderParams);
template __global__ void rtc_render_chain<true, false, false, true>(RenderParams);
template __global__ void rtc_render_chain<false, true, false, true>(RenderParams);
template __global__ void rtc_render_chain<false, false, false, true>(RenderParams);
template __global__ void rtc_render_chain<false, false, true, false>(RenderParams);
template __global__ void rtc_render_chain<false, false, false, false>(RenderParams);
template __global__ void rtc_render_kernel<true, true>(RenderParams);
template __global__ void rtc_render_kernel<true, false>(RenderParams);
template __global__ void rtc_render_kernel<false, true>(RenderParams);
template __global__ void rtc_render_kernel<false, false>(RenderParams);
template __global__ void rtc_tile_cull_sph<true>(RenderParams, unsigned long long *, unsigned *, unsigned long long *);
template __global__ void rtc_render_chain<true, true, false, true, true>(RenderParams);
template __global__ void rtc_render_chain<true, false, false, true, true>(RenderParams);
template __global__ void rtc_render_chain<false, true, false, true, true>(RenderParams);
template __global__ void rtc_render_chain<false, false, false, true, true>(RenderParams);
template __global__ void rtc_render_sky_rows<4, true, true>(RenderParams);
template __global__ void rtc_render_sky_rows<1, true, true>(RenderParams);
template __global__ void rtc_render_chain<false, false, false, true, false, true>(RenderParams);
template __global__ void rtc_render_chain<false, false, false, true, true, true>(RenderParams);
template __global__ void rtc_render_chain<false, true, false, true, false, true>(RenderParams);
template __global__ void rtc_render_chain<false, true, false, true, true, true>(RenderParams);
template __global__ void rtc_render_chain<true, false, false, true, false, true>(RenderParams);
template __global__ void rtc_render_chain<true, false, false, true, true, true>(RenderParams);
template __global__ void rtc_render_chain<true, true, false, true, false, true>(RenderParams);
template __global__ void rtc_render_chain<true, true, false, true, true, true>(RenderParams);
template __global__ void rtc_accumulate_samples_resume<true>(RenderParams);
template __global__ void rtc_render_kernel<false, false, true>(RenderParams);
template __global__ void rtc_render_kernel<false, true, true>(RenderParams);
template __global__ void rtc_render_kernel<true, false, true>(RenderParams);
template __global__ void rtc_render_kernel<true, true, true>(RenderParams);
template __global__ void rtc_first_hit<false>(RenderParams, int *, float *, float *, float *);
template __global__ void rtc_first_hit<true>(RenderParams, int *, float *, float *, float *);
template __global__ void rtc_trace_rays<false, true>(TraceRaysArgs);
template __global__ void rtc_trace_rays<true, true>(TraceRaysArgs);
template __global__ void rtc_trace_rays<false, false>(TraceRaysArgs);
template __global__ void rtc_trace_rays<true, false>(TraceRaysArgs);
template __global__ void rtc_tile_cull_draws<true>(RenderParams, unsigned long long *, unsigned *, unsigned long long *,
                                                   DrawCache);
template __global__ void rtc_fill_draws<true>(DrawCache);
template __global__ void rtc_render_chain<false, false, false, false, false, false, true>(RenderParams);
template __global__ void rtc_render_chain<false, false, true, false, false, false, true>(RenderParams);
template __global__ void rtc_trace_paths<false, true>(TracePathsArgs);
template __global__ void rtc_trace_paths<true, true>(TracePathsArgs);
template __global__ void rtc_trace_paths<false, false>(TracePathsArgs);
template __global__ void rtc_trace_paths<true, false>(TracePathsArgs);
template __global__ void rtc_occluded<false, true>(OccludedArgs);
template __global__ void rtc_occluded<true, true>(OccludedArgs);
template __global__ void rtc_occluded<false, false>(OccludedArgs);
template __global__ void rtc_occluded<true, false>(OccludedArgs);
template __global__ void rtc_trace_paths_wave<false, true>(TracePathsArgs);
template __global__ void rtc_trace_paths_wave<true, true>(TracePathsArgs);
template __global__ void rtc_trace_paths_wave<false, false>(TracePathsArgs);
template __global__ void rtc_trace_paths_wave<true, false>(TracePathsArgs);
template __global__ void rtc_render_pixels<false, true>(RenderPixelsArgs);
template __global__ void rtc_render_pixels<true, true>(RenderPixelsArgs);
template __global__ void rtc_render_pixels<false, false>(RenderPixelsArgs);
template __global__ void rtc_render_pixels<true, false>(RenderPixelsArgs);
template __global__ void rtc_render_pixels_wave<false, true>(RenderPixelsArgs);
template __global__ void rtc_render_pixels_wave<true, true>(RenderPixelsArgs);
template __global__ void rtc_render_pixels_wave<false, false>(RenderPixelsArgs);
template __global__ void rtc_render_pixels_wave<true, false>(RenderPixelsArgs);
```

raytracingc_amd/csrc/rtc_scene.hip:

```cpp
#include <hip/hip_runtime.h>

#include <algorithm>
#include <cmath>
#include <cstdlib>
#include <cstring>
#include <vector>

#include "rtc_layout.h"
#include "rtc_internal.h"
#include "rtc_hip_util.h"
#include "rtc_records.h"
#include "rtc_regroup.h"
#include "rtc_staged.h"

static double bounce_hit_share(const Triangle *t, int n, const Sphere *sp = nullptr, int ns = 0)
{
    if (n < 0)
        n = 0;
    if (ns < 0 || !sp)
        ns = 0;
    if (n + ns <= 0)
        return 0.0;
    struct D3 { double x, y, z; };
    const auto sub3 = [](D3 a, D3 b) { return D3{a.x - b.x, a.y - b.y, a.z - b.z}; };
// ... 451 lines not shown
    }
    for (int m = 1; m < kRegroupLanes; m <<= 1)
        for (int a = 0; a < 3; ++a) {
            const RegroupExtent o{__shfl_xor(e[a].mn, m, kRegroupLanes), __shfl_xor(e[a].mx, m, kRegroupLanes)};
            regroup_extent_merge(e[a], o);
        }
    if (px == 0)
        for (int a = 0; a < 3; ++a)
            sExt[slice][a] = e[a];
    __syncthreads();
    for (int a = 0; a < 3; ++a) {
        e[a] = sExt[0][a];
        for (int w = 1; w < kRegroupSlices; ++w)
            regroup_extent_merge(e[a], sExt[w][a]);
    }
    const double *key = cent + (size_t)regroup_axis(e) * n;
    const int p = lo + (int)blockIdx.x * kRegroupLanes + px;
    const bool mine = p < hi;
    const int ip = mine ? in[p] : 0;
    const double kp = mine ? regroup_key(key[ip]) : 0.0;
    int rank = 0;
    for (int base = lo; base < hi; base += kRegroupBlock) {
        const int q = base + tid;
        __syncthreads();
        sKey[tid] = q < hi ? regroup_key(key[in[q]]) : 0.0;
        __syncthreads();
        const int j0 = slice * kRegroupLanes, j1 = min(j0 + kRegroupLanes, hi - base);
        if (mine)
            for (int j = j0; j < j1; ++j)
                rank += regroup_rank(sKey[j], base + j, kp, p);
    }
    sRank[slice][px] = rank;
    __syncthreads();
    if (slice == 0 && mine) {
        for (int w = 1; w < kRegroupSlices; ++w)
            rank += sRank[w][px];
        out[lo + rank] = ip;
    }
}

__global__ __launch_bounds__(kRegroupBlock) void rtc_regroup_index(const int *idx, int *clIndex, int n, int slots)
{
    const int k = (int)(blockIdx.x * kRegroupBlock + threadIdx.x);
    if (k < slots)
        clIndex[k] = k < n ? idx[k] : -1;
}

extern "C" int rtc_bounce_hit_share(const Triangle *tris, int triCount, float *share)
{
    if (!share || triCount < 0 || (triCount > 0 && !tris))
        return rtc_fail(RTC_EINVAL, "rtc_bounce_hit_share: bad argument");
    *share = (float)bounce_hit_share(tris, triCount);
    return 0;
}

extern "C" int rtc_bounce_hit_share_all(const Triangle *tris, int triCount, const Sphere *spheres, int sphereCount,
                                        float *share)
{
    if (!share || triCount < 0 || sphereCount < 0 || (triCount > 0 && !tris) || (sphereCount > 0 && !spheres))
        return rtc_fail(RTC_EINVAL, "rtc_bounce_hit_share_all: bad argument");
    *share = (float)bounce_hit_share(tris, triCount, spheres, sphereCount);
    return 0;
}

extern "C" int rtc_scene_sphere_split(const RtcDeviceScene *s)
{
    if (!s)
        return rtc_fail(RTC_EINVAL, "rtc_scene_sphere_split: null scene");
    return s->sphereSplitGate ? 1 : 0;
}

extern "C" int rtc_scene_chain_wgs(const RtcDeviceScene *s)
{
    if (!s)
        return rtc_fail(RTC_EINVAL, "rtc_scene_chain_wgs: null scene");
    return s->chainWgsFull;
}

extern "C" int rtc_scene_chain_report(const RtcDeviceScene *s, RtcChainReport *out)
{
    if (!s || !out)
        return rtc_fail(RTC_EINVAL, "rtc_scene_chain_report: null argument");
    *out = s->chainReport;
    return 0;
}

void rtc_draws_free(RtcDeviceScene *s)
{
    RtcDeviceScene::Draws &D = s->draws;
    for (void *p : {(void *)D.table, (void *)D.ctr, (void *)D.blockSeed, D.pool, (void *)D.itemDraw})
        if (p)
            (void)hipFree(p);
    const long long blocks = D.blocks;
    D = RtcDeviceScene::Draws{};
    D.blocks = blocks;
    s->plan.drawWidth = s->plan.drawHeight = 0;
    s->plan.itemDrawCap = 0;
}

static int draws_prepare(RtcDeviceScene *s, int width, int height, bool reset, size_t growBytes)
{
    RtcDeviceScene::Draws &D = s->draws;
    const size_t pixels = (size_t)width * (size_t)height;
    if (reset || growBytes || !D.capacity)
        HIP_TRY(hipDeviceSynchronize());
    if (!D.capacity)
        reset = true;
    if (reset) {
        const long long want = D.blocks < 0 ? kDrawCacheDefaultBytes / (long long)kDrawBlockBytes : D.blocks;
        const size_t cap = std::min<size_t>((size_t)want, pixels);
        if (cap == 0 || cap >= 0xffffffffull)
            return rtc_fail(RTC_EINVAL, "draw cache: %zu blocks", cap);
        if (cap > D.capacity) {
            for (void *p : {(void *)D.blockSeed, D.pool})
                if (p)
                    HIP_TRY(hipFree(p));
            D.blockSeed = nullptr, D.pool = nullptr, D.capacity = 0;
            HIP_TRY(hipMalloc(&D.blockSeed, cap * sizeof(unsigned)));
            HIP_TRY(hipMalloc(&D.pool, cap * kDrawBlockBytes));
            D.capacity = cap;
        }
        if (!D.ctr)
            HIP_TRY(hipMalloc(&D.ctr, kDcWords * sizeof(unsigned)));
        if (pixels > D.tablePixels) {
            if (D.table)
                HIP_TRY(hipFree(D.table));
            D.table = nullptr, D.tablePixels = 0;
            HIP_TRY(hipMalloc(&D.table, pixels * sizeof(unsigned)));
            D.tablePixels = pixels;
        }
        HIP_TRY(hipMemset(D.table, 0, pixels * sizeof(unsigned)));
        HIP_TRY(hipMemset(D.ctr, 0, kDcWords * sizeof(unsigned)));
        D.parity = 0;
    }
    if (growBytes) {
        if (D.itemDraw)
            HIP_TRY(hipFree(D.itemDraw));
        D.itemDraw = nullptr;
        HIP_TRY(hipMalloc(&D.itemDraw, growBytes));
    }
    if (reset)
        HIP_TRY(hipDeviceSynchronize());
    return 0;
}

int rtc_draws_prepare(RtcDeviceScene *s, int width, int height, bool reset, size_t growBytes)
{
    const int rc = draws_prepare(s, width, height, reset, growBytes);
    if (rc) {
        (void)hipDeviceSynchronize();
        rtc_draws_free(s);
    }
    return rc;
}

extern "C" int rtc_scene_set_draw_cache(RtcDeviceScene *s, long long blocks)
{
    if (!s)
        return rtc_fail(RTC_EINVAL, "rtc_scene_set_draw_cache: null scene");
    RtcDeviceGuard guard(s->device);
    if (!guard.ok())
        return rtc_fail(RTC_ENODEV, "rtc_scene_set_draw_cache: cannot select the scene's device %d", s->device);
    const RtcDeviceScene::Draws &D = s->draws;
    if (D.table || D.ctr || D.blockSeed || D.pool || D.itemDraw) {
        HIP_TRY(hipDeviceSynchronize());
        rtc_draws_free(s);
// ... 537 lines not shown
```

Measured before the change: 529,600 Mrays/s.

## Add cross-workgroup work stealing to the chain render kernel

Each chain workgroup's item counter moves from LDS to a global per-workgroup counter array, padded to separate cache lines and zeroed by the prep and cull kernels. A workgroup that runs out of its own strided items scans other workgroups' counters with a wave ballot and atomically claims their remaining items. This targets tail imbalance at the end of the persistent kernel. The cost is global atomics on every item fetch instead of LDS atomics, plus a larger counter set. It is enabled by default only for the fast non-HITS, non-GENERAL variants when the plan conditions hold.

```diff
diff --git a/include/rtc.h b/include/rtc.h
--- a/include/rtc.h
+++ b/include/rtc.h
@@ -47,6 +47,8 @@
 #define RTC_F_SPLIT_SPHERES 0x2000
 #define RTC_F_NO_DRAW_CACHE 0x4000
 #define RTC_F_WAVE_PER_RAY  0x20000
+#define RTC_F_STEAL         0x40000
+#define RTC_F_NO_STEAL      0x80000
 #define RTC_F_OVERLAP       0x800
 
 typedef struct RtcStats {
@@ -118,6 +120,7 @@
     int chainPrimF, wgsPerCu, chainDyn, clusterCount, chunkCount, launches;
 } RtcChainReport;
 int rtc_scene_chain_report(const RtcDeviceScene *s, RtcChainReport *out);
+int rtc_scene_chain_steal(const RtcDeviceScene *s, int *stole, int *groups);
 int rtc_scene_set_draw_cache(RtcDeviceScene *s, long long blocks);
 int rtc_scene_draw_cache_reset(RtcDeviceScene *s);
 int rtc_scene_draw_cache_stats(const RtcDeviceScene *s, unsigned long long out[4]);
@@ -194,6 +197,7 @@
                         int maxOps, unsigned long long *footprint, int maxFootprint);
 int rtc_plan_sim_set_spheres(RtcPlanSim *sim, int sphereCount, int gateAllows);
 int rtc_plan_sim_set_draw_cache(RtcPlanSim *sim, int on);
+int rtc_plan_sim_set_steal(RtcPlanSim *sim, int eligible);
 int rtc_plan_sim_set_sample_range(RtcPlanSim *sim, int first, int count, unsigned long long rngBuffer);
 int rtc_plan_sim_set_first_hit(RtcPlanSim *sim, unsigned long long prim, unsigned long long depth,
                                unsigned long long normal, unsigned long long albedo);
diff --git a/raytracingc_amd/__init__.py b/raytracingc_amd/__init__.py
--- a/raytracingc_amd/__init__.py
+++ b/raytracingc_amd/__init__.py
@@ -19,6 +19,8 @@
     RTC_F_HOST_ROWS,
     RTC_F_SPLIT_SPHERES,
     RTC_F_NO_DRAW_CACHE,
+    RTC_F_STEAL,
+    RTC_F_NO_STEAL,
     RTC_F_NO_REORDER,
     RTC_F_NO_TILE_CULL,
     RTC_F_WAVE_PER_RAY,
@@ -135,6 +137,7 @@
     overlap: bool = False
     split_spheres: bool = False
     draw_cache: bool = True
+    steal: "bool | None" = None
 
     def flags(self) -> int:
         return ((RTC_F_HOIST_PRIMARY if self.hoist else 0) | (RTC_F_DEBUG_BOUNCES if self.debug_bounces else 0)
@@ -142,7 +145,8 @@
                 | (0 if self.coop else RTC_F_NO_COOP) | (0 if self.cluster_cull else RTC_F_NO_CLUSTER_CULL)
                 | (RTC_F_CHAIN_INLINE if self.chain_inline else 0) | (RTC_F_OVERLAP if self.overlap else 0)
                 | (RTC_F_HOST_ROWS if self.host_rows else 0) | (RTC_F_SPLIT_SPHERES if self.split_spheres else 0)
-                | (0 if self.draw_cache else RTC_F_NO_DRAW_CACHE))
+                | (0 if self.draw_cache else RTC_F_NO_DRAW_CACHE)
+                | (0 if self.steal is None else RTC_F_STEAL if self.steal else RTC_F_NO_STEAL))
 
     def desc(self) -> RtcRenderDesc:
         return RtcRenderDesc(self.width, self.height, self.spp, self.max_bounce, int(self.triangles_only),
@@ -705,6 +709,10 @@
         out = {k: bool(getattr(r, k)) for k in ("multi", "count", "hits", "general", "spheres", "resume")}
         out.update(chain_prim_f=bool(r.chainPrimF), wgs_per_cu=r.wgsPerCu, chain_dyn=r.chainDyn,
                    cluster_count=r.clusterCount, chunk_count=r.chunkCount, launches=r.launches)
+        if hasattr(lib(), "rtc_scene_chain_steal"):
+            stole, groups = C.c_int(0), C.c_int(0)
+            check(lib().rtc_scene_chain_steal(self._h, C.byref(stole), C.byref(groups)), "rtc_scene_chain_steal")
+            out.update(steal=bool(stole.value), groups=groups.value)
         return out
 
     def set_draw_cache(self, blocks: int = -1):
diff --git a/raytracingc_amd/_abi.py b/raytracingc_amd/_abi.py
--- a/raytracingc_amd/_abi.py
+++ b/raytracingc_amd/_abi.py
@@ -114,6 +114,8 @@
 RTC_F_HOST_ROWS = 0x1000
 RTC_F_SPLIT_SPHERES = 0x2000
 RTC_F_NO_DRAW_CACHE = 0x4000
+RTC_F_STEAL = 0x40000
+RTC_F_NO_STEAL = 0x80000
 RTC_F_WAVE_PER_RAY = 0x20000
 RAY_ORDER_KEYS_PER_GROUP = 4096
 RAY_ORDER_SCAN_GROUPS = 256
@@ -160,7 +162,7 @@
     "rtc_probe_primary_cull",
     "rtc_scene_update_async", "rtc_scene_update", "rtc_plan_sim_update", "rtc_plan_sim_set_update_fault",
     "rtc_scene_records_host", "rtc_probe_scene_records",
-    "rtc_scene_chain_report",
+    "rtc_scene_chain_report", "rtc_scene_chain_steal", "rtc_plan_sim_set_steal",
     "rtc_render_first_hit_async", "rtc_plan_sim_set_first_hit",
     "rtc_trace_rays_async", "rtc_trace_rays", "rtc_plan_sim_trace_rays",
     "rtc_scene_set_draw_cache", "rtc_scene_draw_cache_reset", "rtc_scene_draw_cache_stats", "rtc_probe_draw_cache",
@@ -273,6 +275,9 @@
         L.rtc_probe_scene_records.argtypes = [vp, vp, vp, vp, vp, vp, vp, vp]
     if hasattr(L, "rtc_scene_chain_report"):
         L.rtc_scene_chain_report.argtypes = [vp, C.POINTER(RtcChainReport)]
+    if hasattr(L, "rtc_scene_chain_steal"):
+        L.rtc_scene_chain_steal.argtypes = [vp, C.POINTER(C.c_int), C.POINTER(C.c_int)]
+        L.rtc_plan_sim_set_steal.argtypes = [vp, ip]
     if hasattr(L, "rtc_render_first_hit_async"):
         L.rtc_render_first_hit_async.argtypes = [vp, C.POINTER(RtcCamera), C.POINTER(RtcRenderDesc),
                                                  C.POINTER(RtcHitBuffers), vp]
diff --git a/raytracingc_amd/csrc/rtc_chain.h b/raytracingc_amd/csrc/rtc_chain.h
--- a/raytracingc_amd/csrc/rtc_chain.h
+++ b/raytracingc_amd/csrc/rtc_chain.h
@@ -428,7 +428,8 @@
     return S;
 }
 
-template <bool MULTI, bool COUNT, bool HITS, bool GENERAL, bool SPHERES = false, bool RESUME = false, bool DRAWS = false>
+template <bool MULTI, bool COUNT, bool HITS, bool GENERAL, bool SPHERES = false, bool RESUME = false, bool DRAWS = false,
+          bool STEAL = false>
 __global__ __launch_bounds__(kChainBlock) __attribute__((amdgpu_waves_per_eu(RTC_CHAIN_WAVES))) void rtc_render_chain(
     RenderParams P)
 {
@@ -466,7 +467,14 @@
     ChainWaveLds &W = sWave[threadIdx.x >> 6];
     const RngJump laneJump = rng_jump_by(7u * (unsigned)lane);
     int nextIt = 0;
-    const auto next_item = [&]() { return (int)blockIdx.x + atomicAdd(&sWork, 1) * (int)gridDim.x; };
+    static_assert(!STEAL || (!GENERAL && !HITS && !RESUME && !SPHERES && !MULTI && !COUNT), "stealing: the fast kernels without HITS");
+    int *const workCtr = P.geoCount + kGeoWorkFirst;
+    const auto next_item = [&]() {
+        if constexpr (STEAL)
+            return (int)blockIdx.x + atomicAdd(workCtr + (size_t)blockIdx.x * kWorkStride, 1) * (int)gridDim.x;
+        else
+            return (int)blockIdx.x + atomicAdd(&sWork, 1) * (int)gridDim.x;
+    };
     if (lane == 0)
         nextIt = next_item();
 #ifdef RTC_DIAG_COUNT
@@ -517,8 +525,56 @@
     }
     if (lane == 0)
         nextIt = next_item();
+    unsigned struck = 0;
+    bool stealing = false;
+    const auto steal_item = [&]() -> int {
+        const int G = (int)gridDim.x, x = (int)blockIdx.x & 7, me = (int)blockIdx.x >> 3;
+        const int nX = (G - x + 7) >> 3;
+        for (int base = 0, round = 0; base < nX - 1;) {
+            const int j = base + lane;
+            int v = 0;
+            bool open = false;
+            if (j < nX - 1 && !((struck >> round) & 1u)) {
+                int q = me + 1 + j;
+                q -= q >= nX ? nX : 0;
+                v = x + 8 * q;
+                if (v < nItems) {
+                    const int c = __hip_atomic_load(workCtr + (size_t)v * kWorkStride, __ATOMIC_RELAXED, __HIP_MEMORY_SCOPE_AGENT);
+                    open = (long long)v + (long long)c * G < (long long)nItems;
+                }
+            }
+            const unsigned long long any = __ballot(open);
+            if (!any) {
+                base += 64;
+                ++round;
+                continue;
+            }
+            const int pick = __builtin_amdgcn_readfirstlane((int)__builtin_ctzll(any));
+            const int vs = __builtin_amdgcn_readlane(v, pick);
+            int k = 0;
+            if (lane == 0)
+                k = atomicAdd(workCtr + (size_t)vs * kWorkStride, 1);
+            k = __builtin_amdgcn_readfirstlane(k);
+            const long long claimed = (long long)vs + (long long)k * G;
+            if (claimed < (long long)nItems)
+                return (int)claimed;
+            if (lane == pick)
+                struck |= 1u << round;
+        }
+        return -1;
+    };
     DMARK(dcur, 19);
     for (;;) {
+        if constexpr (STEAL) {
+            if (it >= nItems) {
+                stealing = true;
+                it = steal_item();
+                if (it < 0)
+                    break;
+                vc = record_dwords(it);
+                vm = mask_dwords((unsigned)__builtin_amdgcn_readfirstlane((int)vc));
+            }
+        }
         if (it >= nItems)
             break;
 #ifdef RTC_DIAG
@@ -549,7 +605,7 @@
         if (itNext < nItems)
             vc = record_dwords(itNext);
         bool maskNext = itNext >= nItems;
-        if (lane == 0)
+        if (lane == 0 && !(STEAL && stealing))
             nextIt = next_item();
         const int tile = record_tile(d0);
         int x = (int)(d0 & 0xffffu), r = (int)(d0 >> 16);
diff --git a/raytracingc_amd/csrc/rtc_closest.h b/raytracingc_amd/csrc/rtc_closest.h
--- a/raytracingc_amd/csrc/rtc_closest.h
+++ b/raytracingc_amd/csrc/rtc_closest.h
@@ -7,6 +7,9 @@
     const int t = blockIdx.x * 64 + threadIdx.x;
     if (geoCount && blockIdx.x == 0 && threadIdx.x < kGeoLists)
         geoCount[threadIdx.x * kGeoCountStride] = 0;
+    if (geoCount && blockIdx.x == 0)
+        for (int i = threadIdx.x; i < kWorkGroupsMax; i += 64)
+            geoCount[kGeoWorkFirst + i * kWorkStride] = 0;
     if (t >= triCount)
         return;
     const DevTri T = tris[t];
diff --git a/raytracingc_amd/csrc/rtc_cull.h b/raytracingc_amd/csrc/rtc_cull.h
--- a/raytracingc_amd/csrc/rtc_cull.h
+++ b/raytracingc_amd/csrc/rtc_cull.h
@@ -36,6 +36,9 @@
     const int lane = threadIdx.x & 63, wave = threadIdx.x >> 6;
     if (P.geoCountNext && bx == 0 && by == 0 && threadIdx.x < kGeoLists)
         P.geoCountNext[threadIdx.x * kGeoCountStride] = 0;
+    if (P.geoCountNext && bx == 0 && by == 0)
+        for (int i = threadIdx.x; i < kWorkGroupsMax; i += kBlock)
+            P.geoCountNext[kGeoWorkFirst + i * kWorkStride] = 0;
     __syncthreads();
     const unsigned long long *sup =
         P.superMask ? P.superMask + (size_t)((by / kSuperBlocks) * P.superX + bx / kSuperBlocks) * P.maskWords : nullptr;
diff --git a/raytracingc_amd/csrc/rtc_layout.h b/raytracingc_amd/csrc/rtc_layout.h
--- a/raytracingc_amd/csrc/rtc_layout.h
+++ b/raytracingc_amd/csrc/rtc_layout.h
@@ -181,7 +181,9 @@
 
 constexpr int kGeoLists = 16, kGeoCountStride = 32;
 constexpr int kItemRecDwords = 4;
-constexpr int kGeoRing = 16, kGeoSetInts = kGeoLists * kGeoCountStride;
+constexpr int kWorkStride = 16, kWorkGroupsMax = 1024;
+constexpr int kGeoRing = 16, kGeoWorkFirst = kGeoLists * kGeoCountStride;
+constexpr int kGeoSetInts = kGeoWorkFirst + kWorkGroupsMax * kWorkStride;
 static_assert(kGeoSetInts >= kGeoLists * kGeoCountStride, "a counter set holds every sub-list counter");
 static_assert(kSkySlots == rtcplan::kSlots && kGeoRing == rtcplan::kGeoRing && kGeoLists == rtcplan::kGeoLists &&
                   kGeoCountStride == rtcplan::kGeoCountStride && kItemRecDwords * 4 == rtcplan::kItemRecordBytes,
@@ -259,6 +261,7 @@
     bool timing;
     bool timed;
     RtcChainReport chainReport;
+    int chainStole, chainGroups;
     struct Draws {
         long long blocks;
         unsigned *table;
diff --git a/raytracingc_amd/csrc/rtc_plan.cpp b/raytracingc_amd/csrc/rtc_plan.cpp
--- a/raytracingc_amd/csrc/rtc_plan.cpp
+++ b/raytracingc_amd/csrc/rtc_plan.cpp
@@ -92,6 +92,11 @@
 void set_draw_cache(Request &r, int eligible)
 {
     r.drawCache = eligible & 3;
+}
+
+void set_steal(Request &r, int eligible)
+{
+    r.stealOk = eligible & 3;
 }
 
 void set_sample_range(Request &r, int first, int count, uint64_t rngState)
@@ -218,6 +223,9 @@
                 n.itemDrawCap = p.itemDrawNeed;
             p.itemDrawOffset = (size_t)p.half * (n.itemDrawCap / kSlots);
         }
+        p.steal = ((r.stealOk >> (p.smallShare ? 1 : 0)) & 1) && r.spp > 0 && p.sampleCap == 0 && !r.segments && !r.resume &&
+                  r.sphereCount == 0 && !(r.flags & (RTC_F_HOIST_PRIMARY | RTC_F_NO_STEAL)) &&
+                  ((r.flags & RTC_F_STEAL) || (p.chainOnCs && !p.smallShare && px > kInlineSumPixels));
     }
     const auto bind = [&p](bool on, std::initializer_list<int> bufs) { for (int b : bufs) p.bound |= (unsigned)on << b; };
     bind(true, {kBufPrim, kBufSceneGen});
@@ -233,6 +241,7 @@
     bind(r.segments, {kBufSegSlots, kBufCallerSegments});
     bind(r.resume, {kBufRngState});
     bind(p.draws, {kBufDrawTable, kBufItemDraw});
+    bind(p.chain, {kBufWorkSet, kBufWorkSetNext});
 
     if (p.cs != kStCaller) {
         E.record(kStCaller, kEvCullSync);
@@ -341,7 +350,7 @@
 }
 
 namespace {
-enum When : int { kAlways, kIfMerge, kIfNotMerge, kIfPrepCounts, kIfResumeRead };
+enum When : int { kAlways, kIfMerge, kIfNotMerge, kIfPrepCounts, kIfResumeRead, kIfSteal };
 struct Touch {
     int kernel, buf, access, when;
 };
@@ -382,20 +391,24 @@
     {kKFirstHit, kBufSceneGen, kRead, kAlways},    {kKFirstHit, kBufHit, kWrite, kAlways},
     {kKTileCull, kBufDrawTable, kWrite, kAlways},  {kKTileCull, kBufItemDraw, kWrite, kAlways},
     {kKChain, kBufItemDraw, kRead, kAlways},
+    {kKPrep, kBufWorkSet, kWrite, kIfPrepCounts},  {kKTileCull, kBufWorkSetNext, kWrite, kAlways},
+    {kKChain, kBufWorkSet, kAtomic, kIfSteal},
 };
 }
 
 int kernel_footprint(const Plan &p, const Request &r, int kernel, Footprint *out, int max)
 {
-    const struct { int res; unsigned long long id; } outside[kBufs - kScratchRegions] = {
+    const struct { int res; unsigned long long id, lo; } outside[kBufs - kScratchRegions] = {
         {kResPrim, (unsigned long long)p.half}, {kResGeoSet, p.geoSet}, {kResGeoSet, p.geoSetNext}, {kResSamples, 0},
         {kResSegSlots, 0}, {kResColors, r.key.colors}, {kResAccum, r.key.accum}, {kResCallerSegments, 0},
         {kResRngState, r.rngState}, {kResSceneGen, (unsigned long long)p.gen}, {kResHit, 0},
-        {kResDrawTable, 0}, {kResItemDraw, (unsigned long long)p.half}};
+        {kResDrawTable, 0}, {kResItemDraw, (unsigned long long)p.half}, {kResGeoSet, p.geoSet, 1},
+        {kResGeoSet, p.geoSetNext, 1}};
     int k = 0;
     for (const Touch &t : kTouches) {
         const bool when = t.when == kAlways || (t.when == kIfResumeRead ? p.resumeRead
                                                 : t.when == kIfPrepCounts ? p.prepCounts
+                                                : t.when == kIfSteal      ? p.steal
                                                                           : p.merge == (t.when == kIfMerge));
         if (t.kernel != kernel || !p.binds(t.buf) || !when)
             continue;
@@ -412,7 +425,8 @@
             out[k] = Footprint{kResScratch, t.access, 0, p.slotOffset + p.reg[t.buf].offset,
                                p.slotOffset + p.reg[t.buf].offset + p.reg[t.buf].size};
         else if (k < max)
-            out[k] = Footprint{outside[t.buf - kScratchRegions].res, t.access, outside[t.buf - kScratchRegions].id, 0, 1};
+            out[k] = Footprint{outside[t.buf - kScratchRegions].res, t.access, outside[t.buf - kScratchRegions].id,
+                               outside[t.buf - kScratchRegions].lo, outside[t.buf - kScratchRegions].lo + 1};
         ++k;
     }
     return k;
@@ -575,6 +589,7 @@
     bool hitNext;
     uint64_t hit[4];
     bool drawCache;
+    int stealOk;
 };
 
 namespace {
@@ -645,6 +660,14 @@
     return 0;
 }
 
+extern "C" int rtc_plan_sim_set_steal(RtcPlanSim *s, int eligible)
+{
+    if (!s || eligible < 0 || eligible > 3)
+        return RTC_EINVAL;
+    s->stealOk = eligible;
+    return 0;
+}
+
 extern "C" int rtc_plan_sim_set_sample_range(RtcPlanSim *s, int first, int count, unsigned long long rngBuffer)
 {
     if (!s)
@@ -696,6 +719,7 @@
     }
     if (s->drawCache)
         rtcplan::set_draw_cache(r, 3);
+    rtcplan::set_steal(r, s->stealOk);
     rtcplan::Plan &p = s->last;
     rtcplan::plan_launch(s->st, r, p);
     s->st = p.after;
diff --git a/raytracingc_amd/csrc/rtc_plan.h b/raytracingc_amd/csrc/rtc_plan.h
--- a/raytracingc_amd/csrc/rtc_plan.h
+++ b/raytracingc_amd/csrc/rtc_plan.h
@@ -99,6 +99,7 @@
     bool firstHit;
     uint64_t hit[4];
     int drawCache;
+    int stealOk;
     int height;
 };
 
@@ -114,6 +115,8 @@
 void set_first_hit(Request &r, const uint64_t ids[4]);
 
 void set_draw_cache(Request &r, int eligible);
+
+void set_steal(Request &r, int eligible);
 
 int geometry_error(const RtcRenderDesc &d);
 
@@ -136,6 +139,7 @@
     kBufSceneGen,
     kBufHit,
     kBufDrawTable, kBufItemDraw,
+    kBufWorkSet, kBufWorkSetNext,
     kBufs
 };
 struct Region {
@@ -167,6 +171,7 @@
     unsigned long long geoSet, geoSetNext;
     bool prep, prepCounts;
     bool cullPrio;
+    bool steal;
     bool draws, drawReset, itemDrawGrow;
     size_t itemDrawNeed, itemDrawOffset;
     int nOps;
diff --git a/raytracingc_amd/csrc/rtc_probe.hip b/raytracingc_amd/csrc/rtc_probe.hip
--- a/raytracingc_amd/csrc/rtc_probe.hip
+++ b/raytracingc_amd/csrc/rtc_probe.hip
@@ -369,7 +369,7 @@
         if (const int r = rtc_cull_items(s, scene, cam, d, dColors, &it))
             return r;
         HIP_TRY(hipDeviceSynchronize());
-        int raw[kGeoSetInts];
+        int raw[kGeoWorkFirst];
         HIP_TRY(hipMemcpy(raw, it.geoCount, sizeof raw, hipMemcpyDeviceToHost));
         size_t total = 0;
         for (int l = 0; l < kGeoLists; ++l) {
diff --git a/raytracingc_amd/csrc/rtc_render.hip b/raytracingc_amd/csrc/rtc_render.hip
--- a/raytracingc_amd/csrc/rtc_render.hip
+++ b/raytracingc_amd/csrc/rtc_render.hip
@@ -94,19 +94,20 @@
 }
 
 struct ChainFlags {
-    bool multi, count, hits, general, spheres, resume, draws;
+    bool multi, count, hits, general, spheres, resume, draws, steal;
     constexpr bool operator==(const ChainFlags &o) const
     {
         return multi == o.multi && count == o.count && hits == o.hits && general == o.general && spheres == o.spheres &&
-               resume == o.resume && draws == o.draws;
+               resume == o.resume && draws == o.draws && steal == o.steal;
     }
 };
 
 constexpr ChainFlags chain_flags(bool multi, bool count, bool defer, bool hits, bool spheres, bool resume,
-                                 bool draws = false)
+                                 bool draws = false, bool steal = false)
 {
     const bool general = multi || count || defer || spheres || resume;
-    return ChainFlags{multi, count, hits && !general, general, spheres, resume, draws && !general};
+    return ChainFlags{multi, count, hits && !general, general, spheres, resume, draws && !general,
+                      steal && !general && !hits};
 }
 
 struct ChainVariant {
@@ -123,21 +124,24 @@
     return n;
 }
 
-constexpr int kInMulti = 1, kInCount = 2, kInDefer = 4, kInHits = 8, kInSpheres = 16, kInResume = 32, kInDraws = 64;
+constexpr int kInMulti = 1, kInCount = 2, kInDefer = 4, kInHits = 8, kInSpheres = 16, kInResume = 32, kInDraws = 64,
+              kInSteal = 128;
 template <typename Rule> constexpr bool every_chain_launch(Rule rule)
 {
-    for (int in = 0; in < 128; ++in)
+    for (int in = 0; in < 256; ++in)
         if (!rule(in, chain_flags(in & kInMulti, in & kInCount, in & kInDefer, in & kInHits, in & kInSpheres,
-                                  in & kInResume, in & kInDraws)))
+                                  in & kInResume, in & kInDraws, in & kInSteal)))
             return false;
     return true;
 }
-static_assert(every_chain_launch([](int in, ChainFlags f) { return f.general == ((in & ~(kInHits | kInDraws)) != 0); }),
+static_assert(every_chain_launch([](int in, ChainFlags f) { return f.general == ((in & ~(kInHits | kInDraws | kInSteal)) != 0); }),
               "GENERAL whenever the launch is multi-chunk, counting, deferring, with spheres or a pass");
-static_assert(every_chain_launch([](int in, ChainFlags f) { return f.hits == ((in & ~kInDraws) == kInHits); }),
+static_assert(every_chain_launch([](int in, ChainFlags f) { return f.hits == ((in & ~(kInDraws | kInSteal)) == kInHits); }),
               "HITS only when none of them holds and the scene is hit-heavy");
 static_assert(every_chain_launch([](int in, ChainFlags f) { return f.draws == (!!(in & kInDraws) && !f.general); }),
               "DRAWS only in the two kernels without GENERAL");
+static_assert(every_chain_launch([](int in, ChainFlags f) { return f.steal == (!!(in & kInSteal) && !f.general && !f.hits); }),
+              "STEAL only in the kernels without GENERAL and HITS");
 static_assert(every_chain_launch([](int in, ChainFlags f) {
                   return f.multi == !!(in & kInMulti) && f.count == !!(in & kInCount) &&
                          f.spheres == !!(in & kInSpheres) && f.resume == !!(in & kInResume);
@@ -295,6 +299,14 @@
     return (chain_prim_f_staged(s, s->chainWgsFull) ? 1 : 0) | (chain_prim_f_staged(s, RTC_CHAIN_WGS_SHARE) ? 2 : 0);
 }
 
+static int steal_eligible(const RtcDeviceScene *s)
+{
+    if (s->triCount == 0 || (s->chainWgsFull == RTC_CHAIN_WGS_HIT && RTC_CHAIN_WGS_HIT != RTC_CHAIN_WGS_FULL))
+        return 0;
+    const auto fits = [&](int wgsPerCu) { return chain_prim_f_staged(s, wgsPerCu) && wgsPerCu * s->cuCount <= kWorkGroupsMax; };
+    return (fits(s->chainWgsFull) ? 1 : 0) | (fits(RTC_CHAIN_WGS_SHARE) ? 2 : 0);
+}
+
 static void size_chain_lds(Launch &L)
 {
     const RtcDeviceScene *s = L.s;
@@ -378,19 +390,24 @@
         CHAIN_ROW(true, false, false, true, false, true),    CHAIN_ROW(true, true, false, true, false, true),
         CHAIN_ROW(false, false, false, true, true, true),    CHAIN_ROW(false, true, false, true, true, true),
         CHAIN_ROW(true, false, false, true, true, true),     CHAIN_ROW(true, true, false, true, true, true),
-        CHAIN_ROW(false, false, false, false, false, false, true), CHAIN_ROW(false, false, true, false, false, false, true)};
+        CHAIN_ROW(false, false, false, false, false, false, true), CHAIN_ROW(false, false, true, false, false, false, true),
+        CHAIN_ROW(false, false, false, false, false, false, false, true),
+        CHAIN_ROW(false, false, false, false, false, false, true, true)};
     constexpr int kVariants = (int)(sizeof kChain / sizeof kChain[0]);
     static_assert(every_chain_launch([](int, ChainFlags f) { return chain_variant(kChain, f) < kVariants; }),
                   "every launch selects an instantiated kernel");
     const int variant =
-        chain_variant(kChain, chain_flags(multi, count, defer, hits, P.sphereCount > 0, L.resume, L.pl.draws));
+        chain_variant(kChain, chain_flags(multi, count, defer, hits, P.sphereCount > 0, L.resume, L.pl.draws, L.pl.steal));
     if (kChain[variant].flags.draws != L.pl.draws)
         return rtc_fail(RTC_EINVAL, "rtc_render_chain: the launch was planned with the draw cache but runs a GENERAL kernel");
+    if (kChain[variant].flags.steal != L.pl.steal || (L.pl.steal && cg.x > (unsigned)kWorkGroupsMax))
+        return rtc_fail(RTC_EINVAL, "rtc_render_chain: the launch was planned to steal but runs a kernel that cannot");
     {
         const ChainFlags &f = kChain[variant].flags;
         RtcChainReport &r = const_cast<RtcDeviceScene *>(s)->chainReport;
         r = RtcChainReport{f.multi,      f.count,    f.hits,          f.general,       f.spheres,     f.resume,
                            P.chainPrimF, L.wgsPerCu, (int)L.chainDyn, s->clusterCount, s->chunkCount, r.launches + 1};
+        const_cast<RtcDeviceScene *>(s)->chainStole = f.steal, const_cast<RtcDeviceScene *>(s)->chainGroups = (int)cg.x;
     }
     if (s->timing)
         HIP_TRY(hipEventRecord(s->evHeavy0, os));
@@ -511,6 +528,8 @@
     }
     if (!hit && !items)
         rtcplan::set_draw_cache(rq, draw_cache_eligible(s));
+    if (!hit && !items)
+        rtcplan::set_steal(rq, steal_eligible(s));
     rtcplan::plan_launch(s->plan, rq, pl);
     ms->plan.prepValid[pl.half] = false;
     if (!hit)
@@ -1036,3 +1055,5 @@
 template __global__ void rtc_render_pixels_wave<true, true>(RenderPixelsArgs);
 template __global__ void rtc_render_pixels_wave<false, false>(RenderPixelsArgs);
 template __global__ void rtc_render_pixels_wave<true, false>(RenderPixelsArgs);
+template __global__ void rtc_render_chain<false, false, false, false, false, false, false, true>(RenderParams);
+template __global__ void rtc_render_chain<false, false, false, false, false, false, true, true>(RenderParams);
diff --git a/raytracingc_amd/csrc/rtc_scene.hip b/raytracingc_amd/csrc/rtc_scene.hip
--- a/raytracingc_amd/csrc/rtc_scene.hip
+++ b/raytracingc_amd/csrc/rtc_scene.hip
@@ -557,6 +557,15 @@
     if (!s || !out)
         return rtc_fail(RTC_EINVAL, "rtc_scene_chain_report: null argument");
     *out = s->chainReport;
+    return 0;
+}
+
+extern "C" int rtc_scene_chain_steal(const RtcDeviceScene *s, int *stole, int *groups)
+{
+    if (!s || !stole || !groups)
+        return rtc_fail(RTC_EINVAL, "rtc_scene_chain_steal: null argument");
+    *stole = s->chainStole;
+    *groups = s->chainGroups;
     return 0;
 }
 
```

Result: slower. 434,900 Mrays/s (-17.9%).
